# EnnaDelfen/SUHMO

Hardware: AMD Instinct MI355X
Metric: multigrid V-cycles/s (FAS head solve) + GSRB cell-updates/s; achieved HBM GB/s vs peak (higher is better)
Workload: dtype f64; 1 GPU; SHMIP-A head solve, 4096x4096 cells per GPU (square cells of 24.4 m), single AMR level, 64x64 boxes, 6 MG depths, 4+4 GSRB sweeps per depth, 16 bottom (BASELINE north_star: 4096^2 single-level); partition=none

## Files before the change

### suhmo_amd/csrc/suhmo_amr.hip

```cpp
#include "suhmo_common.h"

namespace {
struct Pair { suhmo_level *C, *F; };

int check_pair(suhmo_level *C, suhmo_level *F)
{
    ARG(C && F);
    const DV &c = C->d[0].v, &f = F->d[0].v;
    if (f.nxg != 2 * c.nxg || f.nyg != 2 * c.nyg || (f.i0 & 1) || (f.j0 & 1) || (f.nx & 1) || (f.ny & 1)) {
        suhmo_set_error("amr: the fine level must be a coarse-aligned patch of the domain refined by 2"); return -1; }
    {
        const int lo[2] = {f.i0 / 2, f.j0 / 2}, hi[2] = {(f.i0 + f.nx) / 2 - 1, (f.j0 + f.ny) / 2 - 1};
        const int clo[2] = {c.i0, c.j0}, chi[2] = {c.i0 + c.nx - 1, c.j0 + c.ny - 1}, dom[2] = {c.nxg, c.nyg};
        for (int d = 0; d < 2; d++) {
            bool ok_lo = (clo[d] == 0) ? lo[d] >= 0 : lo[d] - clo[d] >= 2;
            bool ok_hi = (chi[d] == dom[d] - 1) ? hi[d] <= chi[d] : chi[d] - hi[d] >= 2;
            if (d == 1) {
                if (f.rk[0]) ok_lo = lo[1] == clo[1] && c.rk[0]; else if (c.rk[0]) ok_lo = lo[1] - clo[1] >= 1;
                if (f.rk[1]) ok_hi = hi[1] == chi[1] && c.rk[1]; else if (c.rk[1]) ok_hi = chi[1] - hi[1] >= 1;
            }
            if (!ok_lo || !ok_hi) { suhmo_set_error("amr: the fine patch is not properly nested in its coarse level (2 cells)"); return -1; }
        }
    }
    if (C->device != F->device) { suhmo_set_error("amr2: both levels on one device"); return -1; }
// ... 155 lines not shown
    const int co = cidx(vc, I + vf.i0 / 2 - vc.i0, J + vf.j0 / 2 - vc.j0), fo = cidx(vf, 2 * I, 2 * J);
    if (J < ncy) { double sm = 0.0; sm = sm + bxf[fo]; sm = sm + bxf[fo + vf.P]; bxc[co] = sm / 2.0; }
    if (I < ncx) { double sm = 0.0; sm = sm + byf[fo]; sm = sm + byf[fo + 1]; byc[co] = sm / 2.0; }
}
}

int suhmo_grad_cc(suhmo_level *L, int depth, hipStream_t st);
int suhmo_re_bcoef_unfused(suhmo_level *L, int depth, hipStream_t st);

extern "C" int suhmo_amr2_cf_interp(suhmo_level_t *C, suhmo_level_t *F, int field_f, int field_c, suhmo_stream_t s)
{
    int rc = check_pair(C, F); if (rc) return rc;
    ARG(field_f >= 0 && field_f < SUHMO_F_COUNT && field_c >= 0 && field_c < SUHMO_F_COUNT);
    HIPCHK(hipSetDevice(F->device));
    const DV &vf = F->d[0].v, &vc = C->d[0].v;
    double *pf = suhmo_field(F, 0, field_f), *pc = suhmo_field(C, 0, field_c);
    if (!pf || !pc) { suhmo_set_error("field allocation failed"); return -2; }
    if (field_c == SUHMO_F_PHI && (rc = suhmo_ensure_phi_halo(C, 0, 1, (hipStream_t)s))) return rc;
    int n = 2 * vf.ny + 2 * vf.nx;
    hipLaunchKernelGGL(k_cf_interp, dim3((n + 255) / 256), dim3(256), 0, (hipStream_t)s, vf, pf, vc, pc);
    HIPCHK(hipGetLastError());
    return 0;
}

extern "C" int suhmo_amr2_average(suhmo_level_t *C, suhmo_level_t *F, int field_f, int field_c, suhmo_stream_t s)
{
    int rc = check_pair(C, F); if (rc) return rc;
    ARG(field_f >= 0 && field_f < SUHMO_F_COUNT && field_c >= 0 && field_c < SUHMO_F_COUNT);
    HIPCHK(hipSetDevice(F->device));
    const DV &vf = F->d[0].v, &vc = C->d[0].v;
    double *pf = suhmo_field(F, 0, field_f), *pc = suhmo_field(C, 0, field_c);
    if (!pf || !pc) { suhmo_set_error("field allocation failed"); return -2; }
    if (field_c == SUHMO_F_PHI) C->d[0].phi_fresh = 0;
    hipLaunchKernelGGL(k_amr_average, dim3((vf.nx / 2 + 63) / 64, (vf.ny / 2 + 3) / 4), dim3(64, 4), 0, (hipStream_t)s, vf, pf, vc, pc);
    HIPCHK(hipGetLastError());
    return 0;
}

extern "C" int suhmo_amr2_fine_update_operator(suhmo_level_t *C, suhmo_level_t *F, suhmo_stream_t s)
{
    int rc = check_pair(C, F); if (rc) return rc;
    HIPCHK(hipSetDevice(F->device));
    hipStream_t st = (hipStream_t)s;
    if ((rc = suhmo_grad_cc(F, 0, st))) return rc;
    if ((rc = suhmo_grad_cc(C, 0, st))) return rc;
    if ((rc = suhmo_amr2_cf_interp(C, F, SUHMO_F_GRADX, SUHMO_F_GRADX, s))) return rc;
    if ((rc = suhmo_amr2_cf_interp(C, F, SUHMO_F_GRADY, SUHMO_F_GRADY, s))) return rc;
    return suhmo_re_bcoef_unfused(F, 0, st);
}

extern "C" int suhmo_amr2_reflux(suhmo_level_t *C, suhmo_level_t *F, int field_c, suhmo_stream_t s)
{
    int rc = check_pair(C, F); if (rc) return rc;
    ARG(field_c >= 0 && field_c < SUHMO_F_COUNT && field_c != SUHMO_F_PHI && field_c != SUHMO_F_BX && field_c != SUHMO_F_BY);
    HIPCHK(hipSetDevice(F->device));
    const DV &vf = F->d[0].v, &vc = C->d[0].v;
    double *p = suhmo_field(C, 0, field_c);
    if (!p) { suhmo_set_error("field allocation failed"); return -2; }
    if ((rc = suhmo_amr2_cf_interp(C, F, SUHMO_F_PHI, SUHMO_F_PHI, s))) return rc;
    int n = vf.ny + vf.nx;
    hipLaunchKernelGGL(k_amr_reflux, dim3((n + 255) / 256), dim3(256), 0, (hipStream_t)s, vf, F->d[0].fp, vc, C->d[0].fp, p);
    HIPCHK(hipGetLastError());
    return 0;
}
extern "C" int suhmo_amr2_pwl_fill(suhmo_level_t *C, suhmo_level_t *F, int field_f, int field_c, suhmo_stream_t s)
{
    int rc = check_pair(C, F); if (rc) return rc;
    ARG(field_f >= 0 && field_f < SUHMO_F_COUNT && field_c >= 0 && field_c < SUHMO_F_COUNT);
    ARG(field_f != SUHMO_F_BX && field_f != SUHMO_F_BY && field_f != SUHMO_F_QWX && field_f != SUHMO_F_QWY && field_f != SUHMO_F_DCX && field_f != SUHMO_F_DCY);
    HIPCHK(hipSetDevice(F->device));
    const DV &vf = F->d[0].v, &vc = C->d[0].v;
    double *pf = suhmo_field(F, 0, field_f), *pc = suhmo_field(C, 0, field_c);
    if (!pf || !pc) { suhmo_set_error("field allocation failed"); return -2; }
    if (field_f == SUHMO_F_PHI) F->d[0].phi_fresh = 0;
    int n = 2 * (vf.nx + 2) + 2 * vf.ny;
    hipLaunchKernelGGL(k_pwl_fill, dim3((n + 255) / 256), dim3(256), 0, (hipStream_t)s, vf, pf, vc, pc);
    HIPCHK(hipGetLastError());
    return 0;
}
extern "C" int suhmo_amr2_prolong_pc(suhmo_level_t *C, suhmo_level_t *F, int field_c, suhmo_stream_t s)
{
    int rc = check_pair(C, F); if (rc) return rc;
    ARG(field_c >= 0 && field_c < SUHMO_F_COUNT && field_c != SUHMO_F_BX && field_c != SUHMO_F_BY);
    HIPCHK(hipSetDevice(F->device));
    Depth &DC = C->d[0], &DF = F->d[0];
    double *corr = suhmo_field(C, 0, field_c);
    if (!corr) { suhmo_set_error("field allocation failed"); return -2; }
    DF.phi_fresh = 0;
    hipLaunchKernelGGL(k_amr_prolong_pc, dim3((DF.v.nx + 63) / 64, (DF.v.ny + 3) / 4), dim3(64, 4), 0, (hipStream_t)s, DF.v, DF.fp.f[SUHMO_F_PHI], DC.v, corr);
    HIPCHK(hipGetLastError());
    return 0;
}
extern "C" int suhmo_amr2_finer_operator_changed(suhmo_level_t *C, suhmo_level_t *F, suhmo_stream_t s)
{
    int rc = check_pair(C, F); if (rc) return rc;
    HIPCHK(hipSetDevice(F->device));
    for (int f : {SUHMO_F_ACOEF, SUHMO_F_B, SUHMO_F_PI, SUHMO_F_ZB, SUHMO_F_MASK})
        if ((rc = suhmo_amr2_average(C, F, f, f, s))) return rc;
    const DV &vf = F->d[0].v, &vc = C->d[0].v;
    hipLaunchKernelGGL(k_amr_average_faces, dim3((vf.nx / 2 + 1 + 63) / 64, (vf.ny / 2 + 1 + 3) / 4), dim3(64, 4), 0, (hipStream_t)s, vf,
                       F->d[0].fp.f[SUHMO_F_BX], F->d[0].fp.f[SUHMO_F_BY], vc, C->d[0].fp.f[SUHMO_F_BX], C->d[0].fp.f[SUHMO_F_BY]);
    HIPCHK(hipGetLastError());
    C->coarse_mask_ok = 0;
    suhmo_level_drop_graphs(C);
    return 0;
}

extern "C" int suhmo_amr2_prolong2(suhmo_level_t *C, suhmo_level_t *F, int field_c, suhmo_stream_t s)
{
    int rc = check_pair(C, F); if (rc) return rc;
    ARG(field_c >= 0 && field_c < SUHMO_F_COUNT && field_c != SUHMO_F_BX && field_c != SUHMO_F_BY);
    HIPCHK(hipSetDevice(F->device));
    Depth &DC = C->d[0], &DF = F->d[0];
    double *corr = suhmo_field(C, 0, field_c);
    if (!corr) { suhmo_set_error("field allocation failed"); return -2; }
    if ((rc = suhmo_level_exchange(C, 0, field_c, s))) return rc;
    if ((rc = suhmo_level_fill_ghosts(C, 0, field_c, 0, s))) return rc;
    DF.phi_fresh = 0;
    hipLaunchKernelGGL(k_amr_prolong2, dim3((DF.v.nx + 63) / 64, (DF.v.ny + 3) / 4), dim3(64, 4), 0, (hipStream_t)s, DF.v, DF.fp.f[SUHMO_F_PHI], DC.v, corr);
    HIPCHK(hipGetLastError());
    return 0;
}
extern "C" int suhmo_amr2_set_covered(suhmo_level_t *C, suhmo_level_t *F, int field_c, double value, suhmo_stream_t s)
{
    int rc = check_pair(C, F); if (rc) return rc;
    ARG(field_c >= 0 && field_c < SUHMO_F_COUNT);
    HIPCHK(hipSetDevice(F->device));
    const DV &vf = F->d[0].v, &vc = C->d[0].v;
    double *p = suhmo_field(C, 0, field_c);
    if (!p) { suhmo_set_error("field allocation failed"); return -2; }
    if (field_c == SUHMO_F_PHI) C->d[0].phi_fresh = 0;
    hipLaunchKernelGGL(k_amr_set_covered, dim3((vf.nx / 2 + 63) / 64, (vf.ny / 2 + 3) / 4), dim3(64, 4), 0, (hipStream_t)s, vf, vc, p, value);
    HIPCHK(hipGetLastError());
    return 0;
}

int suhmo_apply_and_residual(suhmo_level *L, int depth, hipStream_t st);
namespace {
int cf_phi(suhmo_level_t **lv, int l, suhmo_stream_t s)
{
    if (l == 0) return 0;
    if (lv[l]) return suhmo_amr2_cf_interp(lv[l - 1], lv[l], SUHMO_F_PHI, SUHMO_F_PHI, s);
    if (lv[l - 1]) return suhmo_ensure_phi_halo(lv[l - 1], 0, 1, (hipStream_t)s);
    return 0;
}
int composite_residual(suhmo_level_t **lv, int l, suhmo_stream_t s)
{
    suhmo_level *C = lv[l - 1], *F = lv[l];
    if (!C) return 0;
    hipStream_t st = (hipStream_t)s;
    int rc;
    if ((rc = cf_phi(lv, l - 1, s))) return rc;
    if ((rc = suhmo_apply_and_residual(C, 0, st))) return rc;
    double *res = suhmo_field(C, 0, SUHMO_F_RES);
    if ((rc = cf_phi(lv, l, s))) return rc;
    if (F) {
        const DV &vf = F->d[0].v, &vc = C->d[0].v;
        int n = vf.ny + vf.nx;
        hipLaunchKernelGGL(k_amr_reflux, dim3((n + 255) / 256), dim3(256), 0, st, vf, F->d[0].fp, vc, C->d[0].fp, res, 1);
        HIPCHK(hipGetLastError());
    }
    return 0;
}
int vcycle_amr(suhmo_level_t **lv, int l, const suhmo_solver_params_t *sp, suhmo_stream_t s)
// ... 131 lines not shown
```

### suhmo_amd/csrc/suhmo_bcoef.hip

```cpp
#include "suhmo_hier.h"
#include "suhmo_level_int.h"
#include "suhmo_batch.h"
#include <algorithm>
#include <cmath>
#include <initializer_list>
#include <type_traits>
__device__ __forceinline__ void d_gradcc_val(const DV &v, const FP &fp, int hasMask, int i, int j, double &gx, double &gy)
{
    const double *__restrict__ phi = fp.f[SUHMO_F_PHI];
    int idx = cidx(v, i, j);
    double c = phi[idx];
    double e = phiE(v, phi, idx, i, c, false), w = phiW(v, phi, idx, i, c, false);
    double n = phiN(v, phi, idx, j, c, false), s = phiS(v, phi, idx, j, c, false);
    double gW = v.fdx * (c - w), gE = v.fdx * (e - c), gS = v.fdy * (c - s), gN = v.fdy * (n - c);
    if (hasMask) {
        const double *__restrict__ m = fp.f[SUHMO_F_MASK];
        bool mc = m[idx] < 1e-6;
        if (mc || m[idx - 1] < 1e-6) gW = 0.0;
        if (mc || m[idx + 1] < 1e-6) gE = 0.0;
        if (mc || m[idx - v.P] < 1e-6) gS = 0.0;
        if (mc || m[idx + v.P] < 1e-6) gN = 0.0;
    }
    gx = 0.5 * (gW + gE);
    gy = 0.5 * (gS + gN);
// ... 122 lines not shown
    if (i > v.nx || j > v.ny) return;
    int idx = cidx(v, i, j);
    const double *__restrict__ Re = fp.f[SUHMO_F_RE], *__restrict__ B = fp.f[SUHMO_F_B], *__restrict__ m = fp.f[SUHMO_F_MASK];
    if (j < v.ny)
        fp.f[SUHMO_F_BX][idx] = bcoef_face(ph, Re[idx], Re[idx - 1], B[idx], B[idx - 1], m[idx], m[idx - 1], i + v.i0 == 0 || i + v.i0 == v.nxg);
    if (i < v.nx) {
        int jg = j + v.j0;
        fp.f[SUHMO_F_BY][idx] = bcoef_face(ph, Re[idx], Re[idx - v.P], B[idx], B[idx - v.P], m[idx], m[idx - v.P], jg == 0 || jg == v.nyg);
    }
}
template <class T> __global__ __launch_bounds__(256) void k_bcoef_faces(T t) { d_bcoef_faces(t.view(), t.fields(), t.phys()); }
__global__ __launch_bounds__(256) void k_re_bcoef(OnBoxes t)
{
    const DV &v = t.view();
    const FP &fp = t.fields();
    const suhmo_phys_t &ph = t.phys();
    const int i = (int)(blockIdx.x * blockDim.x + threadIdx.x) - 1, j = (int)(blockIdx.y * blockDim.y + threadIdx.y) - 1;
    if (i > v.nx || j > v.ny) return;
    const bool xo = (i < 0 || i >= v.nx), yo = (j < 0 || j >= v.ny);
    if (xo && yo) return;
    const int idx = cidx(v, i, j);
    const double Rc = d_re_val(fp, ph, idx);
    fp.f[SUHMO_F_RE][idx] = Rc;
    if (i < 0 || j < 0) return;
    const double *__restrict__ B = fp.f[SUHMO_F_B], *__restrict__ m = fp.f[SUHMO_F_MASK];
    if (j < v.ny)
        fp.f[SUHMO_F_BX][idx] = bcoef_face(ph, Rc, d_re_val(fp, ph, idx - 1), B[idx], B[idx - 1], m[idx], m[idx - 1], i + v.i0 == 0 || i + v.i0 == v.nxg);
    if (i < v.nx) {
        const int jg = j + v.j0;
        fp.f[SUHMO_F_BY][idx] = bcoef_face(ph, Rc, d_re_val(fp, ph, idx - v.P), B[idx], B[idx - v.P], m[idx], m[idx - v.P], jg == 0 || jg == v.nyg);
    }
}

template <bool INTERIOR, int BT_X, int BT_Y>
__device__ __forceinline__ void bcoef_tile(const DV &v, const FP &fp, const suhmo_phys_t &ph, int hasMask, double *sphi, double *sB, double *sM,
                                           unsigned *negflag, unsigned epoch)
{
    constexpr int PW = BT_X + 4, PH = BT_Y + 4;
    constexpr int RW = BT_X + 2, RH = BT_Y + 2;
    constexpr int TX = BT_X + 2, TY = 256 / TX;
    constexpr int NK = RH / TY;
    static_assert(TX * TY == 256 && RH % TY == 0, "tile shape");
    double *sre = sphi;
    const int i0 = blockIdx.x * BT_X, j0 = blockIdx.y * BT_Y;
    const int tx = threadIdx.x, ty = threadIdx.y;
    const double *__restrict__ phi = fp.f[SUHMO_F_PHI], *__restrict__ Bf = fp.f[SUHMO_F_B], *__restrict__ mk = fp.f[SUHMO_F_MASK];
    double *__restrict__ bxo = fp.f[SUHMO_F_BX], *__restrict__ byo = fp.f[SUHMO_F_BY];
    const bool halo_lo = v.ext[0], halo_hi = v.ext[1], selfper_y = v.per[1] && !halo_lo && !halo_hi;
    auto xin = [&](int i) { return INTERIOR || (i >= 0 && i < v.nx) || v.per[0]; };
    auto yin = [&](int j) { return INTERIOR || (j >= 0 && j < v.ny) || selfper_y || (j < 0 && halo_lo && j >= -v.gy) || (j >= v.ny && halo_hi && j < v.ny + v.gy); };
    auto wrapx = [&](int i) { return (!INTERIOR && v.per[0]) ? (i < 0 ? i + v.nx : (i >= v.nx ? i - v.nx : i)) : i; };
    auto wrapy = [&](int j) { return (!INTERIOR && selfper_y) ? (j < 0 ? j + v.ny : (j >= v.ny ? j - v.ny : j)) : j; };

    for (int lj = ty; lj < PH; lj += TY) {
        const int j = j0 - 2 + lj;
        const bool yi = yin(j);
        for (int li = tx; li < PW; li += TX) {
            const int i = i0 - 2 + li;
            const bool xi = xin(i);
            double val = 0.0;
            if (xi && yi) val = phi[cidx(v, wrapx(i), wrapy(j))];
            else if (yi && (i == -1 || i == v.nx)) {
                int ic = i < 0 ? 0 : v.nx - 1, idx = cidx(v, ic, wrapy(j));
                double c = phi[idx];
                val = i < 0 ? phiW(v, phi, idx, ic, c, false) : phiE(v, phi, idx, ic, c, false);
            } else if (xi && (j == -1 || j == v.ny)) {
                int jc = j < 0 ? 0 : v.ny - 1, idx = cidx(v, wrapx(i), jc);
                double c = phi[idx];
                val = j < 0 ? phiS(v, phi, idx, jc, c, false) : phiN(v, phi, idx, jc, c, false);
            }
            sphi[lj * PW + li] = val;
        }
    }
    const int i = i0 - 1 + tx;
    const bool xi = xin(i);
    double Br[NK];
    bool hasB[NK];
    bool neg = false;
#pragma unroll
    for (int k = 0; k < NK; k++) {
        const int lj = ty + TY * k, j = j0 - 1 + lj;
        hasB[k] = INTERIOR || (i >= -1 && i <= v.nx && j >= -v.gy && j <= v.ny + v.gy - 1 && !((i < 0 || i >= v.nx) && (j < 0 || j >= v.ny)));
        double b = 0.0, m = 0.0;
        if (hasB[k]) { int idx = cidx(v, i, j); b = Bf[idx]; m = mk[idx]; }
        neg = neg || (m < 0.0 && i >= 0 && i < v.nx && j >= 0 && j < v.ny);
        Br[k] = b;
        sB[lj * RW + tx] = b; sM[lj * RW + tx] = m;
    }
    if (negflag && neg) *negflag = epoch;
    __syncthreads();
    auto gradcc = [&](int p, int gi, int gj, double &gx, double &gy) {
        double c = sphi[p], w = sphi[p - 1], e = sphi[p + 1], s = sphi[p - PW], n = sphi[p + PW];
        double gW = v.fdx * (c - w), gE = v.fdx * (e - c), gS = v.fdy * (c - s), gN = v.fdy * (n - c);
        if (hasMask) {
            int idx = cidx(v, wrapx(gi), wrapy(gj));
            bool mc = mk[idx] < 1e-6;
            if (mc || mk[idx - 1] < 1e-6) gW = 0.0;
            if (mc || mk[idx + 1] < 1e-6) gE = 0.0;
            if (mc || mk[idx - v.P] < 1e-6) gS = 0.0;
            if (mc || mk[idx + v.P] < 1e-6) gN = 0.0;
        }
        gx = 0.5 * (gW + gE); gy = 0.5 * (gS + gN);
    };
    double rer[NK];
#pragma unroll
    for (int k = 0; k < NK; k++) {
        const int lj = ty + TY * k, j = j0 - 1 + lj;
        const bool yi = yin(j);
        const int p = (lj + 1) * PW + (tx + 1);
        double gx = 0.0, gy = 0.0;
        if (xi && yi) {
            gradcc(p, i, j, gx, gy);
        } else if (xi != yi) {
            int d = 0, di = 0, dj = 0;
            if (!xi && (i == -1 || i == v.nx)) { di = i < 0 ? 1 : -1; d = di; }
            else if (!yi && (j == -1 || j == v.ny)) { dj = j < 0 ? 1 : -1; d = dj * PW; }
            if (d != 0) {
                double g1x, g1y, g2x, g2y;
                gradcc(p + d, i + di, j + dj, g1x, g1y);
                gradcc(p + 2 * d, i + 2 * di, j + 2 * dj, g2x, g2y);
                gx = 2.0 * g1x - g2x; gy = 2.0 * g1y - g2y;
            }
        }
        double re = 0.0;
        if (hasB[k]) {
            double B = Br[k];
            double sg = sqrt(gx * gx + gy * gy);
            double discr = 1.0 + 4.0 * ph.omega * (B * B * B * ph.grav * sg) / (12.0 * ph.nu * ph.nu);
            re = (-1.0 + sqrt(discr)) / (2.0 * ph.omega);
        }
        rer[k] = re;
    }
    __syncthreads();
#pragma unroll
    for (int k = 0; k < NK; k++) sre[(ty + TY * k) * RW + tx] = rer[k];
    __syncthreads();
    const int nxt = (!INTERIOR && i0 + BT_X >= v.nx) ? v.nx - i0 + 1 : BT_X, nyt = (!INTERIOR && j0 + BT_Y >= v.ny) ? v.ny - j0 + 1 : BT_Y;
    const int fx = tx - 1;
    if (fx >= 0 && fx < nxt) {
        for (int fy = ty; fy < nyt; fy += TY) {
            const int j = j0 + fy, idx = cidx(v, i, j), r = (fy + 1) * RW + tx;
            if (INTERIOR || j < v.ny)
                bxo[idx] = bcoef_face(ph, sre[r], sre[r - 1], sB[r], sB[r - 1], sM[r], sM[r - 1], !INTERIOR && (i == 0 || i == v.nx));
            if (INTERIOR || i < v.nx) {
                int jg = j + v.j0;
                byo[idx] = bcoef_face(ph, sre[r], sre[r - RW], sB[r], sB[r - RW], sM[r], sM[r - RW], !INTERIOR && (jg == 0 || jg == v.nyg));
            }
        }
    }
}
struct MaskHalo { const double *m[SUHMO_MAXDEPTH]; int nx[SUHMO_MAXDEPTH], ny[SUHMO_MAXDEPTH], P[SUHMO_MAXDEPTH], gy[SUHMO_MAXDEPTH]; int nd, lo, hi; };
__global__ __launch_bounds__(256) void k_mask_halo_report(MaskHalo h, unsigned *negflag, unsigned epoch)
{
    const int d = blockIdx.z, i = blockIdx.x * blockDim.x + threadIdx.x;
    if (d >= h.nd || i >= h.nx[d]) return;
    const int g = h.gy[d];
    bool neg = false;
    for (int r = blockIdx.y; r < 2 * g; r += gridDim.y) {
        const bool top = r >= g;
        if (top ? !h.hi : !h.lo) continue;
        const int j = top ? h.ny[d] + (r - g) : -1 - r;
        neg = neg || h.m[d][(long)(j + g) * h.P[d] + SUHMO_XOFF + i] < 0.0;
    }
    if (neg) *negflag = epoch;
}
template <int BT_X, int BT_Y>
__device__ __forceinline__ void d_bcoef_fused(const DV &v, const FP &fp, const suhmo_phys_t &ph, int hasMask, unsigned *negflag, unsigned epoch)
{
    __shared__ double sphi[(BT_X + 4) * (BT_Y + 4)], sB[(BT_X + 2) * (BT_Y + 2)], sM[(BT_X + 2) * (BT_Y + 2)];
    const int i0 = blockIdx.x * BT_X, j0 = blockIdx.y * BT_Y;
    const bool interior = i0 - 2 >= 0 && i0 + BT_X + 1 <= v.nx - 1 && j0 - 2 >= 0 && j0 + BT_Y + 1 <= v.ny - 1;
    if (interior) bcoef_tile<true, BT_X, BT_Y>(v, fp, ph, hasMask, sphi, sB, sM, negflag, epoch);
    else bcoef_tile<false, BT_X, BT_Y>(v, fp, ph, hasMask, sphi, sB, sM, negflag, epoch);
}
template <class T, int BT_X, int BT_Y>
__global__ __launch_bounds__(256) void k_bcoef_fused(T t, unsigned *negflag, unsigned epoch)
{
    const suhmo_phys_t ph = t.phys();
    if (std::is_same<T, OnMembers>::value) { negflag = nullptr; epoch = 0u; }
    d_bcoef_fused<BT_X, BT_Y>(t.view(), t.fields(), ph, ph.use_mask_gradients, negflag, epoch);
}
template <class T> int launch_bcoef_fused(const T &t, bool wide, unsigned *flag, unsigned epoch, hipStream_t st)
{
    if constexpr (std::is_same<T, OnLevel>::value)
        if (wide) return launch_grid(k_bcoef_fused<T, 126, 14>, t, dim3((t.nx() + 125) / 126, (t.ny() + 13) / 14), dim3(128, 2), st, flag, epoch);
    return launch_grid(k_bcoef_fused<T, 62, 14>, t, dim3((t.nx() + 61) / 62, (t.ny() + 13) / 14), dim3(64, 4), st, flag, epoch);
}
template int launch_bcoef_fused(const OnMembers &, bool, unsigned *, unsigned, hipStream_t);
template <class T> int launch_re(const T &t, hipStream_t st) { return launch_over(k_re<T>, t, GHOSTED, st); }
template <class T> int launch_bcoef_faces(const T &t, hipStream_t st) { return launch_over(k_bcoef_faces<T>, t, FACES, st); }
template <class T> int launch_grad_cc(const T &t, hipStream_t st)
{
    int rc = launch_over(k_gradcc<T>, t, CELLS, st);
    return rc ? rc : launch_over(k_grad_ghosts<T>, t, PERIMETER, st);
}
template int launch_re(const OnLevel &, hipStream_t);
template int launch_re(const OnBoxes &, hipStream_t);
template int launch_re(const OnMembers &, hipStream_t);
template int launch_bcoef_faces(const OnLevel &, hipStream_t);
template int launch_bcoef_faces(const OnBoxes &, hipStream_t);
template int launch_bcoef_faces(const OnMembers &, hipStream_t);
template int launch_grad_cc(const OnMembers &, hipStream_t);

extern "C" int suhmo_level_update_operator(suhmo_level_t *L, int depth, suhmo_stream_t s)
{
    SUHMO_TIME("VCAMRNonLinearPoissonOp::UpdateOperator");
    ARG(L); ARG(depth >= 0 && depth < L->ndepth);
    HIPCHK(hipSetDevice(L->device));
    hipStream_t st = (hipStream_t)s;
    Depth &D = L->d[depth];
    bool fused = L->bcoef_fused && D.v.nx >= 4 && D.v.ny >= 4 && (!(D.v.ext[0] || D.v.ext[1]) || (D.v.gy >= 2 && D.v.ny >= 2))
                 && L->desc.nx_global == 0;
    int rc = suhmo_ensure_phi_halo(L, depth, fused ? 2 : 1, st); if (rc) return rc;
    if (fused) {
        const bool wide = L->bcoef_tile_x == 126 && D.v.nx >= 256;
        unsigned *flag = nullptr;
        if (depth == 0) { L->maskflag_epoch = 0; L->mask_reported = 0; }
        if (depth == 0 && L->skip_mask) {
            flag = (unsigned *)(L->scratch + L->scratch_elems - 1);
            if (++L->mask_epoch == 0) L->mask_epoch = 1;
            L->mask_reported = 1;
        }
        if ((rc = launch_bcoef_fused(on_level(L, depth), wide, flag, L->mask_epoch, st))) return rc;
        if (flag && (D.v.ext[0] || D.v.ext[1])) {
            MaskHalo h;
            h.nd = 0; h.lo = D.v.ext[0]; h.hi = D.v.ext[1];
            const int last = L->coarse_mask_ok ? (L->agg ? L->agg_depth : L->ndepth) : 1;
            int gmax = 1;
            for (int k = 0; k < last && k < SUHMO_MAXDEPTH; k++) {
                const Depth &Dk = L->d[k];
                h.m[k] = Dk.fp.f[SUHMO_F_MASK]; h.nx[k] = Dk.v.nx; h.ny[k] = Dk.v.ny; h.P[k] = Dk.v.P; h.gy[k] = Dk.v.gy;
                if (Dk.v.gy > gmax) gmax = Dk.v.gy;
                h.nd = k + 1;
            }
            hipLaunchKernelGGL(k_mask_halo_report, dim3((D.v.nx + 255) / 256, 2 * gmax, h.nd), dim3(256), 0, st, h, flag, L->mask_epoch);
        }
    } else {
        if (depth == 0) { L->maskflag_epoch = 0; L->mask_reported = 0; }
        if (!suhmo_field(L, depth, SUHMO_F_GRADX) || !suhmo_field(L, depth, SUHMO_F_GRADY) || !suhmo_field(L, depth, SUHMO_F_RE)) return -2;
        const OnLevel t = on_level(L, depth);
        if ((rc = launch_over(k_gradcc<OnLevel>, t, CELLS, st))) return rc;
        rc = suhmo_exchange_fields(L, depth, {SUHMO_F_GRADX, SUHMO_F_GRADY}, st); if (rc) return rc;
        if ((rc = launch_over(k_grad_ghosts<OnLevel>, t, PERIMETER, st)) || (rc = launch_re(t, st)) || (rc = launch_bcoef_faces(t, st))) return rc;
    }
    HIPCHK(hipGetLastError());
    if (depth == 0 && L->faces_deferred) return 0;
    rc = suhmo_exchange_fields(L, depth, {SUHMO_F_BX, SUHMO_F_BY}, st); if (rc) return rc;
    return 0;
}

int suhmo_grad_cc(suhmo_level *L, int depth, hipStream_t st)
{
    if (!suhmo_field(L, depth, SUHMO_F_GRADX) || !suhmo_field(L, depth, SUHMO_F_GRADY) || !suhmo_field(L, depth, SUHMO_F_RE)) return -2;
    int rc = suhmo_ensure_phi_halo(L, depth, 1, st); if (rc) return rc;
    if ((rc = launch_over(k_gradcc<OnLevel>, on_level(L, depth), CELLS, st))) return rc;
    rc = suhmo_exchange_fields(L, depth, {SUHMO_F_GRADX, SUHMO_F_GRADY}, st); if (rc) return rc;
    return launch_over(k_grad_ghosts<OnLevel>, on_level(L, depth), PERIMETER, st);
}
int suhmo_grad_cc_list(suhmo_level *L, int depth, const int2 *d_cells, int n, hipStream_t st)
{
    Depth &D = L->d[depth];
    if (!suhmo_field(L, depth, SUHMO_F_GRADX) || !suhmo_field(L, depth, SUHMO_F_GRADY) || !suhmo_field(L, depth, SUHMO_F_RE)) return -2;
    int rc = suhmo_ensure_phi_halo(L, depth, 1, st); if (rc) return rc;
    if (n) hipLaunchKernelGGL(k_gradcc_list, dim3((n + 255) / 256), dim3(256), 0, st, D.v, D.fp, L->ph.use_mask_gradients, d_cells, n);
    HIPCHK(hipGetLastError());
    return 0;
}
int suhmo_re_bcoef_unfused(suhmo_level *L, int depth, hipStream_t st)
{
// ... 260 lines not shown
{
    static const int fields[5] = {SUHMO_F_ACOEF, SUHMO_F_B, SUHMO_F_PI, SUHMO_F_ZB, SUHMO_F_MASK};
    int nblocks = 0;
    for (int q = 0; q < 5; q++) a.f[q] = L->d[0].fp.f[fields[q]];
    for (int dep = 1; dep < L->ndepth; dep++) {
        const Depth &C = L->d[dep];
        AvgDepth &o = a.d[dep - 1];
        o.nx = C.v.nx; o.ny = C.v.ny; o.P = C.v.P; o.gy = C.v.gy;
        for (int q = 0; q < 5; q++) o.c[q] = C.fp.f[fields[q]];
        o.boff = nblocks; o.nbx = (C.v.nx + 63) / 64;
        nblocks += 5 * o.nbx * ((C.v.ny + 3) / 4);
    }
    return nblocks;
}
template <class T, class A> static int launch_average_cells_all(const T &t, A av, int nblocks, const DV &v1, int nd, hipStream_t st)
{
    int rc = launch_grid(k_average_cells_all<T, A>, t, dim3(nblocks), BLK2D, st, av, nd);
    return rc ? rc : launch_grid(k_coef_ghosts_all<T, A>, t, dim3((2 * v1.ny + 2 * v1.nx + 255) / 256, 4 * (nd - 1)), dim3(256), st, av);
}
int suhmo_build_mg_coefficients(suhmo_level *L, bool with_faces, hipStream_t st)
{
    const int nd = L->ndepth;
    if (nd > 1) {
        AvgAll a;
        const int nblocks = fill_avg_all(L, a);
        int rc = launch_average_cells_all(on_level(L, 0), a, nblocks, L->d[1].v, nd, st); if (rc) return rc;
    }
    for (int dep = 1; dep < nd; dep++) {
        int rc;
        if (with_faces && (rc = suhmo_level_average_operator(L, dep, (suhmo_stream_t)st))) return rc;
        if (L->agg && dep >= L->agg_depth) continue;
        rc = suhmo_exchange_fields(L, dep, {SUHMO_F_ACOEF, SUHMO_F_B, SUHMO_F_PI, SUHMO_F_ZB, SUHMO_F_MASK}, st); if (rc) return rc;
    }
    L->coarse_mask_ok = 1;
    return suhmo_agg_gather_static(L, with_faces, st);
}
extern "C" int suhmo_level_build_mg_coefficients(suhmo_level_t *L, suhmo_stream_t s)
{
    ARG(L);
    HIPCHK(hipSetDevice(L->device));
    return suhmo_build_mg_coefficients(L, true, (hipStream_t)s);
}

int suhmo_multi_grad_cc(const suhmo_multi &m, hipStream_t st)
{
    return m.merged ? launch_over(k_gradcc_ghosts, m.on(), CELLS, st) : launch_grad_cc(m.on(), st);
}

int suhmo_levels_grad_cc(const suhmo_lvboxes &lv, int hasMask, hipStream_t st)
{
    int nz = 0;
    for (int q = 0; q < lv.n; q++) nz += lv.nbox[q];
    if (nz <= 0) return 0;
    hipLaunchKernelGGL(k_gradcc_ghosts_lv, dim3((lv.maxnx + 63) / 64, (lv.maxny + 3) / 4, nz), BLK2D, 0, st, lv, hasMask);
    HIPCHK(hipGetLastError());
    return 0;
}

int suhmo_multi_re_bcoef(const suhmo_multi &m, hipStream_t st)
{
    const OnBoxes t = m.on();
    if (m.merged) return launch_over(k_re_bcoef, t, GHOSTED, st);
    int rc = launch_re(t, st);
    return rc ? rc : launch_bcoef_faces(t, st);
}

// ... 37 lines not shown
```

### suhmo_amd/csrc/suhmo_common.h

```cpp
#pragma once
#include <hip/hip_runtime.h>
#include <cstdio>
#include <cstdlib>
#include <cstring>
#include <utility>
#include <string>
#include <vector>
#include "../../include/suhmo_hip.h"

#define SUHMO_XOFF 16
#define SUHMO_MAXDEPTH 16

struct DV {
    int nx, ny;
    int P;
    int gy;
    int rows;
    int j0, nyg;
    double dx, dy;
    double rdx, rdy;
    double fdx, fdy;
    double alpha, beta;
    int bct[2][2];
    double two_v[2][2];
// ... 64 lines not shown
{
    return aterm * c
           - v.beta * (bxE * (e - c) * v.rdx - bxW * (c - w) * v.rdx
                       + byN * (n - c) * v.rdy - byS * (c - s) * v.rdy)
           + nl;
}

__device__ __forceinline__ double lambda_cell(const DV &v, double aterm, double bxE, double bxW,
                                              double byN, double byS)
{
    double lam = aterm;
    lam = lam + v.rdx * v.beta * (bxE + bxW);
    lam = lam + v.rdy * v.beta * (byN + byS);
    return lam;
}

struct Depth {
    DV v;
    FP fp;
    size_t elems;
    int nbox;
    int prolong_pending;
    int rhs_pending;
    double *phi_alt;
    int phi_fresh;
};

struct VGraph {
    int key[4]; hipGraphExec_t exec;
    double *p0[SUHMO_MAXDEPTH], *a0[SUHMO_MAXDEPTH];
    double *p1[SUHMO_MAXDEPTH], *a1[SUHMO_MAXDEPTH];
    double *rhs;
    int rout_req, rout_done, rout_np; const double *rout_rhs;
};
struct ProfEv { hipEvent_t a, b; long cells; int restricts; };

struct suhmo_level {
    int ndepth;
    int batch_owned;
    int stub;
    Depth d[SUHMO_MAXDEPTH];
    suhmo_level_desc_t desc;
    std::vector<int> boxes;
    suhmo_phys_t ph;
    int device;
    double *scratch;
    double *hscratch;
    double *hscratch_dev;
    unsigned long long hseq;
    int poll_readback;
    size_t scratch_elems;
    suhmo_exchange_fn ex;
    suhmo_allreduce_max_fn ar;
    suhmo_allreduce_fn ar2;
    int (*ard)(void *user, double *dev_values, int n, int op, suhmo_stream_t s);
    void *user;
    int (*ex_begin)(void *user);
    int (*ex_end)(void *user, suhmo_level *L, suhmo_stream_t s);
    long graph_max_cells;
    std::vector<VGraph> vgraphs; int vgraph_seen[4]; hipStream_t gstream;
    long vgraph_replays;
    suhmo_level *gap; double gap_dt;
    void *rccl;
    int faces_deferred;
    void *ipc; int ipc_owner;
    long agg_min_cells;
    int agg_depth, agg_world, agg_rank;
    suhmo_level *agg;
    int agg_static_stale;
    suhmo_allgather_fn ag; void *ag_user;
    double *agg_send, *agg_recv; size_t agg_cap; long agg_gathers;
    int resout_req, resout_armed, resout_done; const double *resout_rhs; long resout_count;
    int resout_np;
    long frhs_stream, frhs_tile;
    int prof_on;
    std::vector<ProfEv> prof;
    int gsrb_variant;
    long fused_min_cells;
    int bcoef_fused;
    int bcoef_tile_x;
    int fused_nt;
    int fused_restrict;
    int fused_hc;
    int fas_rhs_fused;
    int strips_rhs_local;
    int skip_mask;
    int mask_reported;
    int coarse_mask_ok;
    unsigned mask_epoch, maskflag_epoch;
    int overlap_halo;
    hipStream_t xstream; hipEvent_t xev[2]; long overlapped;
    int tile_strips;
    int tile_chunks;
    int resid_in_relax;
    int fas_rhs_in_relax;
    long tile_max_cells;
    int tile_restrict;
    int tile_order;
    int bottom_solver; long bottom_one_launch_max_cells;
    unsigned long long *bottom_ctr; long bottom_host_iters, bottom_host_solves;
    int gsrb_tile, tile_t, tile_s;
};

void suhmo_set_error(const char *fmt, ...);
struct SuhmoTimer { const char *name; double t0; int mode; explicit SuhmoTimer(const char *n); ~SuhmoTimer(); };
#define SUHMO_TIME(label) SuhmoTimer suhmo_tm_(label)
#define HIPCHK(x) do { hipError_t e_ = (x); if (e_ != hipSuccess) { \
    suhmo_set_error("%s:%d %s -> %s", __FILE__, __LINE__, #x, hipGetErrorString(e_)); return -2; } } while (0)
#define ARG(cond) do { if (!(cond)) { suhmo_set_error("%s:%d bad argument: %s", __FILE__, __LINE__, #cond); return -1; } } while (0)

double *suhmo_field(suhmo_level *L, int depth, int field);
int suhmo_level_create_(suhmo_level_t **out, const suhmo_level_desc_t *desc, bool stub);
void suhmo_level_share_transport(suhmo_level *dst, const suhmo_level *src);
int suhmo_level_materialize_(suhmo_level *L);
void suhmo_fp_changed();
unsigned long suhmo_fp_epoch();
struct SwapGuard {
    double **a, **b; bool armed;
    SwapGuard() : a(nullptr), b(nullptr), armed(false) {}
    void arm(double **a_, double **b_) { a = a_; b = b_; std::swap(*a, *b); armed = true; suhmo_fp_changed(); }
    void back() { if (armed) { std::swap(*a, *b); armed = false; suhmo_fp_changed(); } }
    ~SwapGuard() { back(); }
};
int suhmo_average_operator_all(suhmo_level *L, int nd, hipStream_t st);
int suhmo_restrict_both(suhmo_level *L, int depth, hipStream_t st);
bool suhmo_gsrb_can_fuse_prolong(suhmo_level *L, int depth, int sweeps);
int suhmo_level_residual_and_norm(suhmo_level *L, double *out, hipStream_t st);
int suhmo_level_norm_from_partials(suhmo_level *L, int np, double *out, hipStream_t st);
bool suhmo_gsrb_can_fuse_rhs(suhmo_level *L, int depth, int sweeps, bool rhs_local = false);
int suhmo_launch_gsrb(suhmo_level *L, int depth, int sweeps, int tail, hipStream_t st, int *restricted = nullptr);
void suhmo_level_drop_graphs(suhmo_level *L);
int suhmo_ensure_phi_halo(suhmo_level *L, int depth, int need, hipStream_t st);
int suhmo_fas_coarse_rhs(suhmo_level *L, int depth, hipStream_t st, int hcomp = 0);
struct HostSlot { double *val; unsigned long long *flag; unsigned long long seq; };
HostSlot suhmo_host_slot(suhmo_level *L);
int suhmo_readback(suhmo_level *L, hipStream_t st, double *out, double *out2 = nullptr);
// ... 53 lines not shown
```

### suhmo_amd/csrc/suhmo_fas.hip

```cpp
#include "suhmo_common.h"
#include <cstdlib>

static int eff_depths(const suhmo_level *L, const suhmo_solver_params_t *sp)
{
    int nd = L->ndepth;
    if (sp->max_depth >= 0 && sp->max_depth + 1 < nd) nd = sp->max_depth + 1;
    return nd;
}

static int relax(suhmo_level *L, int dep, int sweeps, int tail, suhmo_stream_t s, bool observable = false, int *restricted = nullptr)
{
    L->resout_armed = observable && dep == 0 && L->resout_req && L->resid_in_relax;
    int rc = suhmo_launch_gsrb(L, dep, sweeps, tail, (hipStream_t)s, restricted);
    L->resout_armed = 0;
    if (rc) return rc;
    if (sweeps > 0 && observable) return suhmo_level_fill_ghosts(L, dep, SUHMO_F_PHI, 1, s);
    return 0;
}

static int rows_after_prolong(int dep, int num_smooth)
{
    int tail_post = 2;
    for (int d = 1; d <= dep; d++) tail_post = (2 * num_smooth + tail_post + 1) / 2;
    return 2 * num_smooth + tail_post;
// ... 52 lines not shown
    } else {
        if ((rc = suhmo_prolong_with_halo(L, dep, (hipStream_t)s))) return rc;
    }
    return relax(L, dep, S, tail_post, s, dep == 0);
}

static int vcycle_body(suhmo_level *L, const suhmo_solver_params_t *sp, int nd, suhmo_stream_t s)
{
    int rc;
    if (sp->bcoeff_otf) {
        L->faces_deferred = 1;
        rc = suhmo_level_update_operator(L, 0, s);
        if (rc) { L->faces_deferred = 0; return rc; }
        if (L->mask_reported) L->maskflag_epoch = L->mask_epoch;
        if ((rc = suhmo_average_operator_all(L, nd, (hipStream_t)s))) return rc;
    } else L->maskflag_epoch = 0;
    rc = fas_cycle(L, 0, sp, nd, s);
    L->maskflag_epoch = 0;
    return rc;
}

void suhmo_level_drop_graphs(suhmo_level *L)
{
    if (getenv("SUHMO_GRAPH_DEBUG")) { int ok = 0; for (VGraph &g : L->vgraphs) ok += g.exec != nullptr; fprintf(stderr,
        "[suhmo] level %dx%d: %zu V-cycle graphs, %d executable\n", L->d[0].v.nx, L->d[0].v.ny, L->vgraphs.size(), ok); }
    for (VGraph &g : L->vgraphs) if (g.exec) (void)hipGraphExecDestroy(g.exec);
    L->vgraphs.clear();
    if (L->gstream) { (void)hipStreamDestroy(L->gstream); L->gstream = nullptr; }
}
static int vcycle_graph(suhmo_level *L, const suhmo_solver_params_t *sp, int nd, suhmo_stream_t s, bool &done)
{
    done = false;
    const int key[4] = {sp->num_smooth, sp->num_bottom, sp->bcoeff_otf, nd};
    auto at_start = [&](const VGraph &g) {
        if (memcmp(g.key, key, sizeof(key))) return false;
        for (int d = 0; d < L->ndepth; d++) if (L->d[d].fp.f[SUHMO_F_PHI] != g.p0[d] || L->d[d].phi_alt != g.a0[d]) return false;
        if (g.rout_req != (L->resid_in_relax ? L->resout_req : 0) || g.rout_rhs != L->resout_rhs) return false;
        return L->d[0].fp.f[SUHMO_F_RHS] == g.rhs;
    };
    for (const VGraph &g : L->vgraphs)
        if (at_start(g)) {
            if (!g.exec) return 0;
            HIPCHK(hipGraphLaunch(g.exec, (hipStream_t)s)); L->vgraph_replays++;
            for (int d = 0; d < L->ndepth; d++) { L->d[d].fp.f[SUHMO_F_PHI] = g.p1[d]; L->d[d].phi_alt = g.a1[d]; } suhmo_fp_changed();
            if (g.rout_done) { L->resout_done = 1; L->resout_count++; L->resout_np = g.rout_np; }
            done = true;
            return 0;
        }
    for (int k = 0; k < 4; k++) if (L->vgraph_seen[k] != key[k]) { memcpy(L->vgraph_seen, key, sizeof(key)); return 0; }
    if (L->vgraphs.size() >= 16) return 0;
    if (!L->gstream) HIPCHK(hipStreamCreateWithFlags(&L->gstream, hipStreamNonBlocking));
    VGraph g; memcpy(g.key, key, sizeof(key)); g.exec = nullptr;
    for (int d = 0; d < SUHMO_MAXDEPTH; d++) { g.p0[d] = g.a0[d] = g.p1[d] = g.a1[d] = nullptr; }
    for (int d = 0; d < L->ndepth; d++) { g.p0[d] = L->d[d].fp.f[SUHMO_F_PHI]; g.a0[d] = L->d[d].phi_alt; }
    g.rhs = L->d[0].fp.f[SUHMO_F_RHS];
    g.rout_req = L->resid_in_relax ? L->resout_req : 0; g.rout_rhs = L->resout_rhs; g.rout_done = 0;
    const int rout_before = L->resout_done; const long rout_count = L->resout_count;
    HIPCHK(hipStreamSynchronize((hipStream_t)s));
    hipGraph_t graph = nullptr;
    hipError_t e = hipStreamBeginCapture(L->gstream, hipStreamCaptureModeThreadLocal);
    int rc = 0;
    if (e == hipSuccess) {
        rc = vcycle_body(L, sp, nd, (suhmo_stream_t)L->gstream);
        e = hipStreamEndCapture(L->gstream, &graph);
    }
    g.rout_done = L->resout_count != rout_count;
    g.rout_np = L->resout_np;
    L->resout_done = rout_before; L->resout_count = rout_count;
    bool clean = true;
    for (int d = 0; d < L->ndepth; d++) {
        clean = clean && !L->d[d].prolong_pending && !L->d[d].rhs_pending;
        g.p1[d] = L->d[d].fp.f[SUHMO_F_PHI]; g.a1[d] = L->d[d].phi_alt;
        L->d[d].prolong_pending = 0; L->d[d].rhs_pending = 0;
        L->d[d].fp.f[SUHMO_F_PHI] = g.p0[d]; L->d[d].phi_alt = g.a0[d];
    }
    if (e == hipSuccess && rc == 0 && clean && graph && hipGraphInstantiate(&g.exec, graph, nullptr, nullptr, 0) != hipSuccess) g.exec = nullptr;
    if (!(e == hipSuccess && rc == 0 && clean)) g.exec = nullptr;
    if (graph) (void)hipGraphDestroy(graph);
    (void)hipGetLastError();
    L->vgraphs.push_back(g);
    if (!g.exec) return 0;
    HIPCHK(hipGraphLaunch(g.exec, (hipStream_t)s)); L->vgraph_replays++;
    for (int d = 0; d < L->ndepth; d++) { L->d[d].fp.f[SUHMO_F_PHI] = g.p1[d]; L->d[d].phi_alt = g.a1[d]; } suhmo_fp_changed();
    if (g.rout_done) { L->resout_done = 1; L->resout_count++; L->resout_np = g.rout_np; }
    done = true;
    return 0;
}

extern "C" int suhmo_level_vcycle(suhmo_level_t *L, const suhmo_solver_params_t *sp, suhmo_stream_t s)
{
    SUHMO_TIME("AMRFASMultiGrid::VCycle");
    ARG(L && sp);
    HIPCHK(hipSetDevice(L->device));
    int nd = eff_depths(L, sp);
    const Depth &D = L->d[0];
    const bool ext = D.v.ext[0] || D.v.ext[1];
    const bool host_bottom = L->bottom_solver && !suhmo_bottom_one_launch(L, nd - 1);
    if (L->graph_max_cells > 0 && !L->ex && !ext && !L->prof_on && !host_bottom && (long)D.v.nx * D.v.ny <= L->graph_max_cells) {
        bool done = false;
        int rc = vcycle_graph(L, sp, nd, s, done);
        if (rc || done) return rc;
    }
    return vcycle_body(L, sp, nd, s);
}

extern "C" int suhmo_level_solve(suhmo_level_t *L, const suhmo_solver_params_t *sp, int *iters, double *hist, suhmo_stream_t s)
{
    SUHMO_TIME("AMRFASMultiGrid::solve");
    ARG(L && sp);
    HIPCHK(hipSetDevice(L->device));
    bool have_res = false;
    int np = 0;
    auto residual = [&](double *rnorm) {
        if (!have_res) return suhmo_level_residual_and_norm(L, rnorm, (hipStream_t)s);
        if (np > 0) return suhmo_level_norm_from_partials(L, np, rnorm, (hipStream_t)s);
        return suhmo_level_norm(L, 0, SUHMO_F_RES, 0, rnorm, s);
    };
    auto cycle = [&] {
        L->resout_req = 1 | 4; L->resout_rhs = nullptr; L->resout_done = 0; L->resout_np = 0;
        int rc = suhmo_level_vcycle(L, sp, s);
        have_res = L->resout_done != 0;
        np = have_res ? L->resout_np : 0;
        L->resout_req = 0; L->resout_done = 0; L->resout_np = 0;
        return rc;
    };
    int rc = suhmo_solve_no_init(sp, iters, hist, residual, cycle);
    if (rc) return rc;
    return suhmo_level_fill_ghosts(L, 0, SUHMO_F_PHI, 0, s);
}
```

### suhmo_amd/csrc/suhmo_gsrb.hip

```cpp
#include "suhmo_hier.h"
#include "suhmo_batch.h"
#include <type_traits>

template <bool HAS_ALPHA>
__device__ __forceinline__ void d_gsrb_pass_simple(const DV &v, const FP &fp, suhmo_phys_t ph, int pass, int jlo, int jhi,
                                                   const FP *__restrict__ ft = nullptr, const int2 *__restrict__ push = nullptr)
{
    int j = jlo + (int)(blockIdx.y * blockDim.y + threadIdx.y);
    int t = blockIdx.x * blockDim.x + threadIdx.x;
    if (j > jhi) return;
    int i = 2 * t + ((j + v.j0 + pass) & 1);
    if (i >= v.nx) return;
    double *__restrict__ phi = fp.f[SUHMO_F_PHI];
    int idx = cidx(v, i, j);
    double c = phi[idx];
    double e = phiE(v, phi, idx, i, c, false), w = phiW(v, phi, idx, i, c, false);
    double n = phiN(v, phi, idx, j, c, false), s = phiS(v, phi, idx, j, c, false);
    double bxW = fp.f[SUHMO_F_BX][idx], bxE = fp.f[SUHMO_F_BX][idx + 1];
    double byS = fp.f[SUHMO_F_BY][idx], byN = fp.f[SUHMO_F_BY][idx + v.P];
    double nl, dnl;
    nl_terms(ph, c, fp.f[SUHMO_F_B][idx], fp.f[SUHMO_F_PI][idx], fp.f[SUHMO_F_ZB][idx],
             fp.f[SUHMO_F_MASK][idx], nl, dnl);
    double aterm = HAS_ALPHA ? v.alpha * fp.f[SUHMO_F_ACOEF][idx] : v.alpha;
    double lofphi = lofphi_cell(v, aterm, c, e, w, n, s, bxE, bxW, byN, byS, nl);
// ... 187 lines not shown
template <int G, int T, int S>
static void launch_box(const suhmo_multi &m, const suhmo_phys_t &ph, bool has_alpha, const void *halo, const int *hbase, int fsrc, int fdst, int npass, int bc_ghosts, hipStream_t st)
{
    const dim3 grd(((m.maxnx + T - 1) / T) * ((m.maxny + T - 1) / T), m.nbox);
    if (has_alpha) hipLaunchKernelGGL((k_gsrb_box_m<true, G, T, S>), grd, dim3(BoxGeom<G, T, S>::NT), 0, st, m.dv, m.fp, (const int2 *)halo, hbase, ph, fsrc, fdst, npass, bc_ghosts);
    else hipLaunchKernelGGL((k_gsrb_box_m<false, G, T, S>), grd, dim3(BoxGeom<G, T, S>::NT), 0, st, m.dv, m.fp, (const int2 *)halo, hbase, ph, fsrc, fdst, npass, bc_ghosts);
}
int suhmo_multi_gsrb_box(const suhmo_multi &m, const suhmo_phys_t &ph, bool has_alpha, const void *halo, const int *hbase, int fsrc, int fdst, int npass, int bc_ghosts, hipStream_t st)
{
    if (m.nbox <= 0) return 0;
    if (npass < 1 || npass > 2 * SUHMO_BOX_HALO) { suhmo_set_error("internal: %d colour passes in one box launch", npass); return -4; }
    if (npass > 4) launch_box<8, 16, 1>(m, ph, has_alpha, halo, hbase, fsrc, fdst, npass, bc_ghosts, st);
    else launch_box<4, 16, 1>(m, ph, has_alpha, halo, hbase, fsrc, fdst, npass, bc_ghosts, st);
    HIPCHK(hipGetLastError());
    return 0;
}

struct FusedGeom {
    int W;
    int Hc;
    int nstrips, nchunks, ntiles;
    int ylo, yhi;
    int jbeg, jend;
    int wrap_y;
    const unsigned *negflag; unsigned mask_epoch;
    int nchl, chunk0, chunk1, edges;
    const double *pc, *pco; int Pc, gyc;
    double *rres, *rphi; int rP, rgy;
    const double *fres; double *frhs, *flphi, *fphiold;
    const double *ortrue; double *ores, *olphi;
    double *onorm;
};

struct RowCoef {
    double rhs[2], B[2], Pi[2], zb[2], mask[2], a[2], byS[2], byN[2];
    double bx0, bx1, bx2;
};
#define CP2(d, s, f) d.f[0] = s.f[0]; d.f[1] = s.f[1]
template <bool HAS_ALPHA>
__device__ __forceinline__ void copy_coef(RowCoef &d, const RowCoef &s)
{
    CP2(d, s, rhs); CP2(d, s, B); CP2(d, s, Pi); CP2(d, s, zb); CP2(d, s, mask);
    if (HAS_ALPHA) { CP2(d, s, a); }
    CP2(d, s, byS); CP2(d, s, byN);
    d.bx0 = s.bx0; d.bx1 = s.bx1; d.bx2 = s.bx2;
}

template <int K, bool HAS_ALPHA, int NT, int RM = 0, bool FRHS = false>
__global__ __launch_bounds__(NT) void k_gsrb_fused(DV v, FP fp, const double *__restrict__ pin,
                                                   double *__restrict__ pout, suhmo_phys_t ph, FusedGeom g)
{
    constexpr bool ROUT = RM == 2, RR = RM != 0;
    static_assert(!(FRHS && (RR || HAS_ALPHA)), "the right-hand side is formed in the plain launch of an alpha = 0 operator");
    constexpr int LW = 2 * NT, R = 2 * K + 3 + (RR ? 1 : 0);
    constexpr int HX = 2 * K + (RR ? 2 : 0), EY = RR ? 1 : 0;
    __shared__ double lds[R * LW];

    int b = blockIdx.x, q = g.ntiles / 8, rem = g.ntiles % 8, xcd = b % 8;
    int tile = xcd * q + (xcd < rem ? xcd : rem) + b / 8;
    int strip = tile / g.nchl, chunk = tile % g.nchl;
    chunk = g.edges ? (chunk < g.chunk0 ? chunk : g.chunk1 + (chunk - g.chunk0)) : g.chunk0 + chunk;

    const int t = threadIdx.x;
    const int c0 = strip * g.W;
    const int xl = 2 * t;
    const int i0 = c0 - HX + xl;
    const bool in_row = xl < g.W + 2 * HX;
    int im = i0;
    if (v.per[0]) { if (im < 0) im += v.nx; else if (im >= v.nx) im -= v.nx; }
    const bool cval = in_row && im >= 0 && im < v.nx;
    const int cend = (c0 + g.W < v.nx) ? c0 + g.W : v.nx;
    const bool own = cval && i0 >= c0 && i0 < cend;

    const int jA = g.jbeg + chunk * g.Hc;
    const int jB = (jA + g.Hc < g.jend) ? jA + g.Hc : g.jend;
    const int jmin = (jA - EY - 2 * K > g.ylo) ? jA - EY - 2 * K : g.ylo;
    const int jmax = (jB - 1 + EY + 2 * K < g.yhi) ? jB - 1 + EY + 2 * K : g.yhi;

    const double *__restrict__ f_rhs = fp.f[SUHMO_F_RHS], *__restrict__ f_B = fp.f[SUHMO_F_B];
    const double *__restrict__ f_Pi = fp.f[SUHMO_F_PI], *__restrict__ f_zb = fp.f[SUHMO_F_ZB];
    const double *__restrict__ f_mask = fp.f[SUHMO_F_MASK], *__restrict__ f_a = fp.f[SUHMO_F_ACOEF];
    const double *__restrict__ f_bx = fp.f[SUHMO_F_BX], *__restrict__ f_by = fp.f[SUHMO_F_BY];

    auto wrapj = [&](int j) { if (g.wrap_y) { if (j < 0) j += v.ny; else if (j >= v.ny) j -= v.ny; } return j; };
    auto ld2 = [&](const double *__restrict__ p, int idx) { return *reinterpret_cast<const double2 *>(p + idx); };

    RowCoef cf0, cf1, cf2, cf3, cf4, cf5;
    double racc = 0.0, raccp = 0.0;
    double nmax = 0.0;
    const bool xbc = !v.per[0] && (c0 - HX <= 0 || c0 + g.W + HX >= v.nx);
    const bool ybc = !v.per[1] && (jmin <= 0 || jmax >= v.ny - 1);
    double2 pnext = make_double2(0.0, 0.0);
    double2 pprev = make_double2(0.0, 0.0);
    const bool usemask = !g.negflag || *g.negflag == g.mask_epoch;

    int sr = 0;
    auto ring = [](int x) { return x < 0 ? x + R : x; };
    for (int r = jmin - 1; r <= jB - 1 + 2 * K + EY; r++) {
        bool lphi = cval && (r + 1 >= jmin) && (r + 1 <= jmax);
        if (lphi) {
            const int jr = wrapj(r + 1);
            pnext = ld2(pin, cidx(v, im, jr));
            if (g.pc) {
                const int ic = ((jr >> 1) + g.gyc) * g.Pc + SUHMO_XOFF + (im >> 1);
                const double corr = 1.0 * g.pc[ic] + (-1.0) * g.pco[ic];
                pnext.x = pnext.x + corr; pnext.y = pnext.y + corr;
            }
        }
        bool lcf = cval && (r >= jmin) && (r <= jmax);
        if (lcf) {
            int idx = cidx(v, im, wrapj(r));
#define LD2(dst, p, ix) { double2 t_ = ld2(p, ix); dst[0] = t_.x; dst[1] = t_.y; }
            LD2(cf0.rhs, (FRHS ? g.fres : f_rhs), idx); LD2(cf0.B, f_B, idx); LD2(cf0.Pi, f_Pi, idx);
            LD2(cf0.zb, f_zb, idx);
            if (usemask) { LD2(cf0.mask, f_mask, idx); } else { cf0.mask[0] = 1.0; cf0.mask[1] = 1.0; }
            if (HAS_ALPHA) LD2(cf0.a, f_a, idx);
            LD2(cf0.byS, f_by, idx); LD2(cf0.byN, f_by, idx + v.P);
            double2 bxp = ld2(f_bx, idx);
            cf0.bx0 = bxp.x; cf0.bx1 = bxp.y; cf0.bx2 = f_bx[idx + 2];
        }
        __syncthreads();

        if constexpr (FRHS) {
            const int jf = r - 1;
            if (cval && jf >= jmin && jf <= jmax) {
                const int s0 = ring(sr - 1), sN = sr;
                const double *row = lds + s0 * LW;
                double lo[2], cc[2];
#pragma unroll
                for (int a = 0; a < 2; a++) {
                    const int x = xl + a, i = im + a;
                    double c = row[x];
                    double w = row[(a == 0 && xl == 0) ? 0 : x - 1], e = row[(a == 1 && xl == LW - 2) ? LW - 1 : x + 1];
                    double n = lds[sN * LW + x], s = a ? pprev.y : pprev.x;
                    if (xbc) {
                        if (i == 0) w = (v.bct[0][0] == 0) ? v.two_v[0][0] - c : c + v.neu[0][0];
                        if (i == v.nx - 1) e = (v.bct[0][1] == 0) ? v.two_v[0][1] - c : c + v.neu[0][1];
                    }
                    if (ybc) {
                        if (jf == 0 && !v.ext[0]) s = (v.bct[1][0] == 0) ? v.two_v[1][0] - c : c + v.neu[1][0];
                        if (jf == v.ny - 1 && !v.ext[1]) n = (v.bct[1][1] == 0) ? v.two_v[1][1] - c : c + v.neu[1][1];
                    }
                    double nl, dnl;
                    nl_terms(ph, c, cf1.B[a], cf1.Pi[a], cf1.zb[a], cf1.mask[a], nl, dnl);
                    const double bxW = a ? cf1.bx1 : cf1.bx0, bxE = a ? cf1.bx2 : cf1.bx1;
                    lo[a] = lofphi_cell(v, v.alpha, c, e, w, n, s, bxE, bxW, cf1.byN[a], cf1.byS[a], nl);
                    cc[a] = c;
                }
                cf1.rhs[0] = 1.0 * cf1.rhs[0] + 1.0 * lo[0]; cf1.rhs[1] = 1.0 * cf1.rhs[1] + 1.0 * lo[1];
                const bool lo_end = v.ext[0] && chunk == 0, hi_end = v.ext[1] && chunk == g.nchunks - 1;
                const int jP0 = lo_end ? jmin : jA, jP1 = hi_end ? jmax + 1 : jB;
                const int jR0 = lo_end ? jmin + 1 : jA, jR1 = hi_end ? jmax : jB;
                if (own && jf >= jP0 && jf < jP1) {
                    const int idx = cidx(v, i0, jf);
                    if (jf >= jR0 && jf < jR1) {
                        *reinterpret_cast<double2 *>(g.flphi + idx) = make_double2(lo[0], lo[1]);
                        *reinterpret_cast<double2 *>(g.frhs + idx) = make_double2(cf1.rhs[0], cf1.rhs[1]);
                    }
                    *reinterpret_cast<double2 *>(g.fphiold + idx) = make_double2(cc[0], cc[1]);
                }
                pprev = make_double2(cc[0], cc[1]);
            }
            __syncthreads();
        }

        auto advance_a = [&](const int m, const RowCoef &q, auto a_tag) {
            constexpr int a = decltype(a_tag)::value;
            const int j = r - m;
            const int x = xl + a, i = im + a;
            const int s0 = ring(sr - m), sN = ring(sr - m + 1), sS = ring(sr - m - 1);
            const double *row = lds + s0 * LW;
            double c = row[x];
            double w = row[(a == 0 && xl == 0) ? 0 : x - 1], e = row[(a == 1 && xl == LW - 2) ? LW - 1 : x + 1];
            double n = lds[sN * LW + x], s = lds[sS * LW + x];
            if (xbc) {
                if (i == 0) w = (v.bct[0][0] == 0) ? v.two_v[0][0] - c : c + v.neu[0][0];
                if (i == v.nx - 1) e = (v.bct[0][1] == 0) ? v.two_v[0][1] - c : c + v.neu[0][1];
            }
            if (ybc) {
                if (j == 0 && !v.ext[0]) s = (v.bct[1][0] == 0) ? v.two_v[1][0] - c : c + v.neu[1][0];
                if (j == v.ny - 1 && !v.ext[1]) n = (v.bct[1][1] == 0) ? v.two_v[1][1] - c : c + v.neu[1][1];
            }
            double nl, dnl;
            nl_terms(ph, c, q.B[a], q.Pi[a], q.zb[a], q.mask[a], nl, dnl);
            const double bxW = a ? q.bx1 : q.bx0, bxE = a ? q.bx2 : q.bx1;
            double aterm = HAS_ALPHA ? v.alpha * q.a[a] : v.alpha;
            double lofphi = lofphi_cell(v, aterm, c, e, w, n, s, bxE, bxW, q.byN[a], q.byS[a], nl);
            double lam = lambda_cell(v, aterm, bxE, bxW, q.byN[a], q.byS[a]);
            double denom = 1.0e-16 + lam + dnl;
            lds[s0 * LW + x] = c + (q.rhs[a] - lofphi) / denom;
        };
        auto advance = [&](const int m, const RowCoef &q) {
            const int j = r - m;
            if (j >= jmin && j <= jmax) {
                const int a = (j + v.j0 + ((m - 1) & 1)) & 1;
                if (a) { if (cval) advance_a(m, q, std::integral_constant<int, 1>()); }
                else   { if (cval) advance_a(m, q, std::integral_constant<int, 0>()); }
            }
        };
        advance(1, cf1);
        __syncthreads();
        advance(2, cf2);
        if constexpr (K >= 2) {
            __syncthreads();
            advance(3, cf3);
            __syncthreads();
            advance(4, cf4);
        }

        if constexpr (RR) {
            const int jr = r - 2 * K - 1;
            if (own && jr >= jA && jr < jB && jr >= 0 && jr < v.ny) {
                const RowCoef &q = (K >= 2) ? cf5 : cf3;
                const int s0 = ring(sr - (2 * K + 1)), sN = ring(sr - 2 * K), sS = ring(sr - (2 * K + 2));
                const double *row = lds + s0 * LW;
                double acc = (jr & 1) ? racc : 0.0, accp = (jr & 1) ? raccp : 0.0;
                double lo2[2] = {0.0, 0.0};
#pragma unroll
                for (int a = 0; a < 2; a++) {
                    const int x = xl + a, i = im + a;
                    double c = row[x], w = row[x - 1], e = row[x + 1];
                    double n = lds[sN * LW + x], s = lds[sS * LW + x];
                    if (xbc) {
                        if (i == 0) w = (v.bct[0][0] == 0) ? v.two_v[0][0] - c : c + v.neu[0][0];
                        if (i == v.nx - 1) e = (v.bct[0][1] == 0) ? v.two_v[0][1] - c : c + v.neu[0][1];
                    }
                    if (ybc) {
                        if (jr == 0 && !v.ext[0]) s = (v.bct[1][0] == 0) ? v.two_v[1][0] - c : c + v.neu[1][0];
                        if (jr == v.ny - 1 && !v.ext[1]) n = (v.bct[1][1] == 0) ? v.two_v[1][1] - c : c + v.neu[1][1];
                    }
                    double nl, dnl;
                    nl_terms(ph, c, q.B[a], q.Pi[a], q.zb[a], q.mask[a], nl, dnl);
                    const double bxW = a ? q.bx1 : q.bx0, bxE = a ? q.bx2 : q.bx1;
                    double aterm = HAS_ALPHA ? v.alpha * q.a[a] : v.alpha;
                    double lofphi = lofphi_cell(v, aterm, c, e, w, n, s, bxE, bxW, q.byN[a], q.byS[a], nl);
                    if constexpr (ROUT) lo2[a] = lofphi;
                    else {
                        acc = acc + (q.rhs[a] - lofphi) / 4.0;
                        accp = accp + c / 4.0;
                    }
                }
                if constexpr (ROUT) {
                    const int idx = cidx(v, i0, jr);
                    const double2 rt = *reinterpret_cast<const double2 *>(g.ortrue + idx);
                    const double r0 = -1.0 * lo2[0] + 1.0 * rt.x, r1 = -1.0 * lo2[1] + 1.0 * rt.y;
                    *reinterpret_cast<double2 *>(g.ores + idx) = make_double2(r0, r1);
                    if (g.olphi) *reinterpret_cast<double2 *>(g.olphi + idx) = make_double2(lo2[0], lo2[1]);
                    nmax = fmax(nmax, fmax(fabs(r0), fabs(r1)));
                } else if (jr & 1) {
                    const int ic = ((jr >> 1) + g.rgy) * g.rP + SUHMO_XOFF + (i0 >> 1);
                    g.rres[ic] = acc; g.rphi[ic] = accp;
                } else { racc = acc; raccp = accp; }
            }
        }
        {
            const int jo = r - 2 * K;
            if (own && jo >= jA && jo < jB) {
                const int so = ring(sr - 2 * K);
                double2 o = make_double2(lds[so * LW + xl], lds[so * LW + xl + 1]);
                *reinterpret_cast<double2 *>(pout + cidx(v, i0, jo)) = o;
            }
        }
        sr = sr + 1 == R ? 0 : sr + 1;
        if (in_row) { lds[sr * LW + xl] = pnext.x; lds[sr * LW + xl + 1] = pnext.y; }
        if constexpr (RR && K >= 2) copy_coef<HAS_ALPHA>(cf5, cf4);
        if constexpr (K >= 2) { copy_coef<HAS_ALPHA>(cf4, cf3); copy_coef<HAS_ALPHA>(cf3, cf2); }
        else if constexpr (RR) copy_coef<HAS_ALPHA>(cf3, cf2);
        copy_coef<HAS_ALPHA>(cf2, cf1);
        copy_coef<HAS_ALPHA>(cf1, cf0);
    }
    if constexpr (ROUT) {
        if (g.onorm) {
            static_assert(!ROUT || NT == 64, "one wave per workgroup");
#pragma unroll
            for (int o = 32; o > 0; o >>= 1) nmax = fmax(nmax, __shfl_xor(nmax, o));
            if (t == 0) g.onorm[strip * g.nchunks + chunk] = nmax;
        }
    }
}

static bool fused_ok(const suhmo_level *L, const Depth &D, int K)
{
    const DV &v = D.v;
    if (v.nx % 2 || v.nx < 64 || v.ny < 4 * K + 4) return false;
    if (v.cfx[0] || v.cfx[1] || L->desc.nx_global > 0) return false;
    if ((v.ext[0] || v.ext[1]) && (v.gy < 2 * K || v.ny < 2 * K)) return false;
    if (v.per[1] && !(v.ext[0] || v.ext[1]) && v.ny < 4 * K) return false;
    return true;
}

template <int K, int NT, int RM = 0>
static int launch_fused(suhmo_level *L, int depth, int ext_rows, hipStream_t st, int part = 0)
{
    constexpr bool RST = RM == 1, RR = RM != 0;
    Depth &D = L->d[depth];
    const DV &v = D.v;
    if (!D.phi_alt) {
        HIPCHK(hipMalloc(&D.phi_alt, D.elems * sizeof(double)));
        HIPCHK(hipMemsetAsync(D.phi_alt, 0, D.elems * sizeof(double), st));
    }
    FusedGeom g;
    constexpr int HX = 2 * K + (RR ? 2 : 0), EY = RR ? 1 : 0;
    const int maxW = 2 * NT - 2 * HX;
    g.nstrips = (v.nx + maxW - 1) / maxW;
    g.W = 2 * ((v.nx + 2 * g.nstrips - 1) / (2 * g.nstrips));
    g.nstrips = (v.nx + g.W - 1) / g.W;
    {
        static int slots_k[3] = {0, 0, 0};
        if (!slots_k[K]) {
            int nb = 0, ncu = 0, dev = 0;
            HIPCHK(hipGetDevice(&dev));
            HIPCHK(hipDeviceGetAttribute(&ncu, hipDeviceAttributeMultiprocessorCount, dev));
            HIPCHK(hipOccupancyMaxActiveBlocksPerMultiprocessor(&nb, (k_gsrb_fused<K, false, NT, RM>), NT, 0));
            slots_k[K] = (nb > 0 ? nb : 1) * (ncu > 0 ? ncu : 256);
        }
        g.jbeg = v.ext[0] ? -ext_rows : 0;
        g.jend = v.ny + (v.ext[1] ? ext_rows : 0);
        const int nrows = g.jend - g.jbeg;
        int nch = slots_k[K] / g.nstrips;
        if (nch < 1) nch = 1;
        g.Hc = (nrows + nch - 1) / nch;
        if (g.Hc < 8 * K) g.Hc = 8 * K;
        if ((long)v.nx * v.ny < 2000000L) g.Hc = 6;
        if (L->fused_hc > 0) g.Hc = L->fused_hc;
        if (RST) g.Hc += g.Hc & 1;
        if (g.Hc > nrows) g.Hc = nrows;
        g.nchunks = (nrows + g.Hc - 1) / g.Hc;
    }
    g.nchl = g.nchunks; g.chunk0 = 0; g.chunk1 = g.nchunks; g.edges = 0;
    if (part) {
        int c0 = 0, c1 = g.nchunks;
        if (v.ext[0]) while (c0 < g.nchunks && g.jbeg + c0 * g.Hc - 2 * K - EY < 0) c0++;
        if (v.ext[1]) while (c1 > c0 && std::min(g.jbeg + c1 * g.Hc, g.jend) - 1 + 2 * K + EY > v.ny - 1) c1--;
        const bool ok = c1 > c0 && c1 - c0 < g.nchunks;
        if (!ok) { if (part == 1) return 1; }
        else if (part == 1) { g.chunk0 = c0; g.chunk1 = c1; g.nchl = c1 - c0; }
        else { g.edges = 1; g.chunk0 = c0; g.chunk1 = c1; g.nchl = g.nchunks - (c1 - c0); }
    }
    g.ntiles = g.nstrips * g.nchl;
    bool selfper = v.per[1] && !(v.ext[0] || v.ext[1]);
    g.wrap_y = selfper;
    g.ylo = v.ext[0] ? g.jbeg - 2 * K - EY : (selfper ? -2 * K - EY : 0);
    g.yhi = v.ext[1] ? g.jend - 1 + 2 * K + EY : (selfper ? v.ny - 1 + 2 * K + EY : v.ny - 1);
    const double *pin = D.fp.f[SUHMO_F_PHI];
    g.pc = g.pco = nullptr; g.Pc = g.gyc = 0;
    if (D.prolong_pending) {
        Depth &C = L->d[depth + 1];
        g.pc = C.fp.f[SUHMO_F_PHI]; g.pco = C.fp.f[SUHMO_F_PHIOLD]; g.Pc = C.v.P; g.gyc = C.v.gy;
        if (part != 1) D.prolong_pending = 0;
    }
    g.negflag = nullptr; g.mask_epoch = 0;
    if (L->skip_mask && L->maskflag_epoch && L->maskflag_epoch == L->mask_epoch && (depth == 0 || L->coarse_mask_ok)
        && (L->desc.nx_global == 0)) {
        g.negflag = (const unsigned *)(L->scratch + L->scratch_elems - 1); g.mask_epoch = L->mask_epoch;
    }
    g.rres = g.rphi = nullptr; g.rP = g.rgy = 0;
    if (RST) {
        Depth &C = L->d[depth + 1];
        g.rres = C.fp.f[SUHMO_F_RES]; g.rphi = C.fp.f[SUHMO_F_PHI]; g.rP = C.v.P; g.rgy = C.v.gy;
        C.phi_fresh = 0;
    }
    g.fres = nullptr; g.frhs = g.flphi = g.fphiold = nullptr;
    g.ortrue = nullptr; g.ores = g.olphi = nullptr;
    if (RM == 2) {
        if (v.alpha != 0.0) { suhmo_set_error("internal: residual output on a launch that cannot form it"); return -4; }
        g.ortrue = L->resout_rhs ? L->resout_rhs : D.fp.f[SUHMO_F_RHS];
        g.ores = D.fp.f[SUHMO_F_RES];
        if (L->resout_req & 2) { g.olphi = suhmo_field(L, depth, SUHMO_F_LPHI); if (!g.olphi) return -2; }
        g.onorm = nullptr;
        if ((L->resout_req & 4) && (size_t)g.nstrips * g.nchunks + 4 < L->scratch_elems) { g.onorm = L->scratch + 2; L->resout_np = g.nstrips * g.nchunks; }
        else L->resout_np = 0;
    }
    if (D.rhs_pending) {
        if constexpr (K == 2 && NT == 64 && !RR) {
            if (part || v.alpha != 0.0) { suhmo_set_error("internal: rhs_pending on a launch that cannot form it"); return -4; }
            g.fres = D.fp.f[SUHMO_F_RES]; g.frhs = D.fp.f[SUHMO_F_RHS]; g.flphi = suhmo_field(L, depth, SUHMO_F_LPHI); g.fphiold = suhmo_field(L, depth, SUHMO_F_PHIOLD);
            if (!g.flphi || !g.fphiold) return -2;
            D.rhs_pending = 0; L->frhs_stream++;
            hipLaunchKernelGGL((k_gsrb_fused<2, false, 64, false, true>), dim3(g.ntiles), dim3(NT), 0, st, v, D.fp, pin, D.phi_alt, L->ph, g);
            { std::swap(D.fp.f[SUHMO_F_PHI], D.phi_alt); suhmo_fp_changed(); }
            return 0;
        } else { suhmo_set_error("internal: rhs_pending on a launch that cannot form it"); return -4; }
    }
    if (v.alpha != 0.0)
        hipLaunchKernelGGL((k_gsrb_fused<K, true, NT, false>), dim3(g.ntiles), dim3(NT), 0, st, v, D.fp, pin, D.phi_alt, L->ph, g);
    else
        hipLaunchKernelGGL((k_gsrb_fused<K, false, NT, RM>), dim3(g.ntiles), dim3(NT), 0, st, v, D.fp, pin, D.phi_alt, L->ph, g);
    if (part != 1) { std::swap(D.fp.f[SUHMO_F_PHI], D.phi_alt); suhmo_fp_changed(); }
    return 0;
}

struct TileGeom {
    int ntx, nty;
    const double *pc, *pco; int Pc, gyc;
    double *rres, *rphi; int rP, rgy;
    int frhs;
    int jbeg, jend;
    int chunks;
    int order;
};
struct PairCoef { double rhs0, rhs1, B0, B1, Pi0, Pi1, zb0, zb1, a0, a1, byS0, byS1, byN0, byN1, bx0, bx1, bx2; int mneg; };

template <int T, bool RST> struct TileShape { static constexpr int TX = T, TY = (RST && T == 32) ? 28 : T; };
template <int S, int T, bool RST> struct TileThreads { static constexpr int NT = 256; };
template <int S, int T, bool HAS_ALPHA, bool RST = false, bool CHUNKED = false>
__device__ __forceinline__ void d_gsrb_tile(const DV &v, const FP &fp, const double *__restrict__ pin, double *__restrict__ pout,
                                            const suhmo_phys_t &ph, const TileGeom &g)
{
    constexpr int TX = TileShape<T, RST>::TX, TY = TileShape<T, RST>::TY;
    constexpr int HX = 2 * S + (RST ? 2 : 0), HY = 2 * S + (RST ? 1 : 0);
    constexpr int LX = TX + 2 * HX, LY = TY + 2 * HY, NP = LX / 2, NPAIR = NP * LY;
    constexpr int NT = TileThreads<S, T, RST>::NT, NK = (NPAIR + NT - 1) / NT;
    constexpr int PAD = LX + 2;
    __shared__ double lds_raw[LY * LX + 2 * PAD];
    double *const lds = lds_raw + PAD;
    __shared__ double lq[RST ? TY * TX : 1];
    int tl = blockIdx.x;
    if (g.order) {
        const int nt = g.ntx * g.nty, q8 = nt / 8, rem = nt % 8, xcd = tl % 8;
// ... 619 lines not shown
```

### suhmo_amd/csrc/suhmo_hier.h

```cpp
#pragma once
#include "suhmo_target.h"
constexpr int SUHMO_BOX_HALO = 8;
struct suhmo_multi { const DV *dv; const FP *fp; int nbox, maxnx, maxny; double *red;
                     int merged;
                     const void *push; const int *pbase;
                     suhmo_phys_t ph;
                     OnBoxes on() const { return OnBoxes{dv, fp, ph, nbox, maxnx, maxny}; } };
template <class T> int launch_colour_pass(const T &t, bool has_alpha, int pass, int lo, int hi, const void *push, const int *pbase, hipStream_t st);
int suhmo_multi_gsrb_box(const suhmo_multi &m, const suhmo_phys_t &ph, bool has_alpha, const void *halo, const int *hbase, int fsrc, int fdst, int npass,
    int bc_ghosts, hipStream_t st);
template <class T> int launch_fill_ghosts(const T &t, int field, int homog, hipStream_t st);
template <class T> int launch_axby(const T &t, int fd, int fx, int fy, double a, double b, hipStream_t st);
template <class T> int launch_restrict(const T &f, const T &c, bool also_phi, bool has_alpha, hipStream_t st);
template <class T> int launch_prolong(const T &f, const T &c, int lo, int hi, int lo_c, int hi_c, hipStream_t st);
int launch_apply_boxes(const OnBoxes &t, bool has_alpha, int mode, hipStream_t st);
int suhmo_apply_and_residual(suhmo_level *L, int depth, hipStream_t st);
int launch_fas_enter(const OnBoxes &t, hipStream_t st);
int launch_fas_leave(const OnBoxes &t, hipStream_t st);
int launch_copy(const OnBoxes &t, int fd, int fs, hipStream_t st);
int launch_copy_between(const OnBoxes &dst, const OnBoxes &src, const int *fd, const int *fs, int n, hipStream_t st);
template <class T> int launch_grad_cc(const T &t, hipStream_t st);
template <class T> int launch_re(const T &t, hipStream_t st);
template <class T> int launch_bcoef_faces(const T &t, hipStream_t st);
template <class T> int launch_coef_ghosts(const T &t, int field, hipStream_t st);
template <class T> int launch_bcoef_fused(const T &t, bool wide, unsigned *flag, unsigned epoch, hipStream_t st);
int suhmo_multi_grad_cc(const suhmo_multi &m, hipStream_t st);
int suhmo_multi_re_bcoef(const suhmo_multi &m, hipStream_t st);
int suhmo_multi_norm_max(const suhmo_multi &m, suhmo_level *slot, int field, double *out, hipStream_t st);
int suhmo_level_norm_max_partials(suhmo_level *L, int field, const double **partials, int *np, hipStream_t st);
int suhmo_multi_norm_max_partials(const suhmo_multi &m, int field, const double **partials, int *np, hipStream_t st);
int suhmo_norm_max_of_lists(suhmo_level *slot, const double *const *partials, const int *np, int cnt, double *out, hipStream_t st);
constexpr int SUHMO_LVMAX = 7;
struct suhmo_lvboxes { const DV *dv[SUHMO_LVMAX]; const FP *fp[SUHMO_LVMAX]; int nbox[SUHMO_LVMAX], mode[SUHMO_LVMAX]; int n, maxnx, maxny; };
int suhmo_levels_apply(const suhmo_lvboxes &lv, const suhmo_phys_t &ph, bool has_alpha, hipStream_t st);
int suhmo_levels_norm_max_cover_partials(const suhmo_lvboxes &lv, int field, double *partial, int *np, hipStream_t st);
int suhmo_level_norm_max_cover_partials(suhmo_level *L, int field, const double **partials, int *np, hipStream_t st);
int suhmo_levels_grad_cc(const suhmo_lvboxes &lv, int hasMask, hipStream_t st);
```

### suhmo_amd/csrc/suhmo_hier.hip

```cpp
#include "suhmo_hier_int.h"
#include <string>

int suhmo_grad_cc(suhmo_level *L, int depth, hipStream_t st);
int suhmo_apply_and_residual_rects(suhmo_level *L, int depth, const int4 *d_rects, int n, int maxw, int maxh, hipStream_t st);
int suhmo_grad_cc_list(suhmo_level *L, int depth, const int2 *d_cells, int n, hipStream_t st);

using namespace hier;
namespace {
inline const suhmo_phys_t &phys_of(suhmo_hier *H, int l) { return H->lev[l].box[0]->ph; }
inline bool has_alpha(suhmo_hier *H, int l) { return H->lev[l].box[0]->d[0].v.alpha != 0.0; }
int hier_gsrb(suhmo_hier *H, int l, int sweeps, suhmo_stream_t s, bool may_swap = false)
{
    SUHMO_TIME("AMRNonLinearPoissonOp::relaxNF");
    if (l == 0) { H->phi_shadow_fresh = false; H->phi_ver[0]++; H->base_full_ver++; return suhmo_level_gsrb(base_of(H), 0, sweeps, s); }
    int rc;
    suhmo_multi m;
    if ((rc = multi_of(H, l, HST(s), m))) return rc;
    HLev &Vf = H->lev[l];
    if (sweeps > 0 && H->fused_relax && Vf.halo_ok && !Vf.part) {
        if ((rc = ensure_field(H, l, SUHMO_F_PHI2)) || (rc = multi_of(H, l, HST(s), m))) return rc;
        if (Vf.self_wrap < 0) {
            Vf.self_wrap = 0;
            for (suhmo_level *L : Vf.box) { const DV &v = L->d[0].v; if ((v.per[0] && !v.cfx[0]) || (v.per[1] && !v.ext[0])) Vf.self_wrap = 1; }
        }
// ... 19 lines not shown
    const bool push = H->push_ghosts && !V.part;
    for (int it = 0; it < sweeps; it++)
        for (int pass = 0; pass < 2; pass++) {
            if ((rc = launch_colour_pass(m.on(), has_alpha(H, l), pass, 0, 0, push ? m.push : nullptr, m.pbase, HST(s)))) return rc;
            H->phi_ver[l]++;
            if (!push && (rc = hier_ff(H, l, SUHMO_F_PHI, -1, false, HST(s), V.part ? pass : -1))) return rc;
        }
    if (sweeps > 0 && (rc = launch_fill_ghosts(m.on(), SUHMO_F_PHI, 1, HST(s)))) return rc;
    if (sweeps > 0 && push) H->ff_seen[l] = H->phi_ver[l];
    return 0;
}
int hier_level_residual(suhmo_hier *H, int l, suhmo_stream_t s)
{
    if (l == 0) return suhmo_level_residual(base_of(H), 0, s);
    int rc;
    suhmo_multi m;
    if ((rc = hier_ff(H, l, SUHMO_F_PHI, -1, false, HST(s))) || (rc = multi_of(H, l, HST(s), m))) return rc;
    return launch_apply_boxes(m.on(), has_alpha(H, l), 1, HST(s));
}
int hier_axby(suhmo_hier *H, int l, int dst, int x, int y, double a, double b, suhmo_stream_t s)
{
    if (l == 0) return suhmo_level_axby(base_of(H), 0, dst, x, y, a, b, s);
    int rc;
    suhmo_multi m;
    if ((rc = ensure_field(H, l, dst)) || (rc = ensure_field(H, l, x)) || (rc = ensure_field(H, l, y)) || (rc = multi_of(H, l, HST(s), m))) return rc;
    return launch_axby(m.on(), dst, x, y, a, b, HST(s));
}
int hier_copy(suhmo_hier *H, int l, int dst, int src, suhmo_stream_t s)
{
    int rc;
    if ((rc = ensure_field(H, l, dst)) || (rc = ensure_field(H, l, src))) return rc;
    if (dst == SUHMO_F_PHI) { for (suhmo_level *L : H->lev[l].box) L->d[0].phi_fresh = 0; H->phi_ver[l]++; }
    if (dst == SUHMO_F_PHI && l == 0) H->phi_shadow_fresh = false;
    if (l == 0) H->base_full_ver++;
    if (l == 0) {
        suhmo_level *L = base_of(H);
        HIPCHK(hipMemcpyAsync(L->d[0].fp.f[dst], L->d[0].fp.f[src], L->d[0].elems * sizeof(double), hipMemcpyDeviceToDevice, HST(s)));
        return 0;
    }
    suhmo_multi m;
    if ((rc = multi_of(H, l, HST(s), m))) return rc;
    return launch_copy(m.on(), dst, src, HST(s));
}
int cf_phi(suhmo_hier *H, int l, suhmo_stream_t s)
{
    if (l == 0) return 0;
    if (H->cf_seen[l][0] == H->phi_ver[l] && H->cf_seen[l][1] == H->phi_ver[l - 1]) return 0;
    if (H->merged_launches && !H->lev[l].part && H->ff_seen[l] != H->phi_ver[l]) {
        int rc = hier_cf_ff(H, l, SUHMO_F_PHI, SUHMO_F_PHI, -1, -1, false, HST(s));
        if (!rc) { H->cf_seen[l][0] = H->phi_ver[l]; H->cf_seen[l][1] = H->phi_ver[l - 1]; H->ff_seen[l] = H->phi_ver[l]; }
        return rc;
    }
    int rc = hier_cf(H, l, SUHMO_F_PHI, SUHMO_F_PHI, HST(s));
    if (!rc) { H->cf_seen[l][0] = H->phi_ver[l]; H->cf_seen[l][1] = H->phi_ver[l - 1]; }
    return rc;
}

inline bool levels_mergeable(const suhmo_hier *H) { return H->merged_launches && !H->part && !dist_base(H) && H->nlev <= SUHMO_LVMAX + 1; }
int levels_boxes(suhmo_hier *H, int llo, int lhi, int mode_top, int mode_rest, suhmo_stream_t s, suhmo_lvboxes &lv)
{
    memset(&lv, 0, sizeof(lv));
    int rc;
    for (int l = lhi; l >= std::max(1, llo); l--) {
        suhmo_multi m;
        if ((rc = multi_of(H, l, HST(s), m))) return rc;
        const int q = lv.n++;
// ... 442 lines not shown
    ARG(H);
    H->ag = fn; H->ag_user = user;
    if (H->gap) { H->gap->ag = fn; H->gap->ag_user = user; }
    return 0;
}
int suhmo_rccl_allgather_hook(void *user, const double *send, long count, double *recv, suhmo_stream_t s);
extern "C" int suhmo_hier_attach_rccl(suhmo_hier_t *H)
{
    ARG(H);
    suhmo_level *B = base_of(H);
    if (!B->rccl) { suhmo_set_error("hier: attach the base strip first (suhmo_level_attach_rccl on suhmo_hier_box(H, 0, 0))"); return -1; }
    return suhmo_hier_set_allgather(H, suhmo_rccl_allgather_hook, B->rccl);
}
extern "C" long suhmo_hier_gathers(const suhmo_hier_t *H) { return H ? H->gathers + (H->gap ? H->gap->gathers : 0) : -1; }
extern "C" int suhmo_hier_num_levels(const suhmo_hier_t *H) { return H ? H->nlev : -1; }
extern "C" int suhmo_hier_num_boxes(const suhmo_hier_t *H, int l) { return (H && l >= 0 && l < H->nlev) ? (int)H->lev[l].box.size() : -1; }
extern "C" suhmo_level_t *suhmo_hier_box(suhmo_hier_t *H, int l, int k)
{
    if (!H || l < 0 || l >= H->nlev || k < 0 || k >= (int)H->lev[l].box.size()) return nullptr;
    return H->lev[l].box[k];
}
extern "C" int suhmo_hier_box_owner(const suhmo_hier_t *H, int l, int k, int *held)
{
    if (!H || l < 0 || l >= H->nlev || k < 0 || k >= (int)H->lev[l].box.size()) return -2;
    const HLev &V = H->lev[l];
    if (held) *held = V.part ? (int)V.held[k] : 1;
    return V.part ? V.owner[k] : -1;
}
extern "C" int suhmo_hier_exchange(suhmo_hier_t *H, int l, int field, int corners, suhmo_stream_t s)
{
    int rc = check_hier(H); if (rc) return rc;
    ARG(l >= 0 && l < H->nlev && field >= 0 && field < SUHMO_F_COUNT);
    HIPCHK(hipSetDevice(H->device));
    return hier_ff(H, l, field, -1, corners != 0, HST(s));
}
extern "C" int suhmo_hier_cf_interp(suhmo_hier_t *H, int l, int field_f, int field_c, suhmo_stream_t s)
{
    int rc = check_hier(H); if (rc) return rc;
    ARG(l >= 1 && l < H->nlev && field_f >= 0 && field_f < SUHMO_F_COUNT && field_c >= 0 && field_c < SUHMO_F_COUNT);
    HIPCHK(hipSetDevice(H->device));
    return hier_cf(H, l, field_f, field_c, HST(s));
}
extern "C" int suhmo_hier_pwl_fill(suhmo_hier_t *H, int l, int field_f, int field_c, suhmo_stream_t s)
{
    int rc = check_hier(H); if (rc) return rc;
    ARG(l >= 1 && l < H->nlev && field_f >= 0 && field_f < SUHMO_F_COUNT && field_c >= 0 && field_c < SUHMO_F_COUNT);
    HIPCHK(hipSetDevice(H->device));
    return hier_pwl(H, l, field_f, field_c, HST(s));
}
extern "C" int suhmo_hier_average(suhmo_hier_t *H, int l, int field_f, int field_c, suhmo_stream_t s)
{
    int rc = check_hier(H); if (rc) return rc;
    ARG(l >= 1 && l < H->nlev && field_f >= 0 && field_f < SUHMO_F_COUNT && field_c >= 0 && field_c < SUHMO_F_COUNT);
    HIPCHK(hipSetDevice(H->device));
    return hier_avg(H, l, field_f, field_c, 0, 0.0, HST(s));
}
extern "C" int suhmo_hier_gsrb(suhmo_hier_t *H, int l, int sweeps, suhmo_stream_t s)
{
    int rc = check_hier(H); if (rc) return rc;
    ARG(l >= 0 && l < H->nlev && sweeps >= 0);
    HIPCHK(hipSetDevice(H->device));
    return hier_gsrb(H, l, sweeps, s);
}
extern "C" int suhmo_hier_update_operator(suhmo_hier_t *H, int l, suhmo_stream_t s)
{
    int rc = check_hier(H); if (rc) return rc;
// ... 90 lines not shown
```

### suhmo_amd/csrc/suhmo_hier_fill.hip

```cpp
#include "suhmo_hier_int.h"

using namespace hier;
namespace {
__device__ __forceinline__ double *fptr(const FP *tab, const FP &base, int use_base, int b, int field)
{
    return use_base ? base.f[field] : tab[b].f[field];
}
__device__ __forceinline__ void d_ff(const CopyEnt &c, const FP *__restrict__ tab, int f0, int f1)
{
    tab[c.d.b].f[f0][c.d.off] = tab[c.s.b].f[f0][c.s.off];
    if (f1 >= 0) tab[c.d.b].f[f1][c.d.off] = tab[c.s.b].f[f1][c.s.off];
}
__global__ void k_ff(const CopyEnt *__restrict__ e, int n, const FP *__restrict__ tab, int f0, int f1)
{
    int t = blockIdx.x * blockDim.x + threadIdx.x;
    if (t >= n) return;
    d_ff(e[t], tab, f0, f1);
}
__device__ __forceinline__ void d_cf(const CfEnt &q, const FP *__restrict__ ftab, int ff0, const FP *__restrict__ ctab, const FP &cbase,
                                     int use_base, int fc0, int ff1, int fc1)
{
    const double c_s = 8.0 / 15.0, c_b = 2.0 / 3.0, c_a = -0.2;
    const double xt = q.xsign ? 0.25 : -0.25;
  for (int pass = 0; pass < (ff1 >= 0 ? 2 : 1); pass++) {
// ... 516 lines not shown
    if (ff1 >= 0 && ((rc = ensure_field(H, l, ff1)) || (rc = ensure_field(H, l - 1, fc1)) || (rc = refresh_tables(H, l, st)))) return rc;
    { const int fl[2] = {fc, fc1};
      if (l == 1 && (rc = refresh_base(H, fl, ff1 >= 0 ? 2 : 1, st))) return rc; }
    if ((rc = coarse_args(H, l - 1, st, ca))) return rc;
    const DevVec<CopyEnt> &list = corners ? V.ff_all : V.ff_side;
    const int nbcf = (int)g1(V.cf.n).x, nbff = (int)g1(list.n).x;
    if (nbcf + nbff > 0)
        hipLaunchKernelGGL(k_cf_ff, dim3(nbcf + nbff), dim3(256), 0, st, V.cf.d, (int)V.cf.n, nbcf, list.d, (int)list.n, V.d_fp, ff, ca.tab, ca.base, ca.use_base, fc, ff1, fc1);
    HIPCHK(hipGetLastError());
    return 0;
}
int hier_pwl(suhmo_hier *H, int l, int ff, int fc, hipStream_t st)
{
    if (l == 0) return 0;
    HLev &V = H->lev[l];
    int rc;
    CoarseArgs ca;
    if ((rc = ensure_field(H, l, ff)) || (rc = ensure_field(H, l - 1, fc)) || (rc = refresh_tables(H, l, st))) return rc;
    if (l == 1 && (rc = refresh_base1(H, fc, st))) return rc;
    if (l > 1 && V.part && (rc = sync1(H, l - 1, V.sy_cread, fc, st))) return rc;
    if ((rc = coarse_args(H, l - 1, st, ca))) return rc;
    if (V.pwl.n) hipLaunchKernelGGL(k_pwl, g1(V.pwl.n), dim3(256), 0, st, V.pwl.d, (int)V.pwl.n, V.d_fp, ff, ca.tab, ca.base, ca.use_base, fc);
    HIPCHK(hipGetLastError());
    return 0;
}
int hier_avg(suhmo_hier *H, int l, int ff, int fc, int mode, double val, hipStream_t st)
{
    HLev &V = H->lev[l];
    int rc;
    CoarseArgs ca;
    if ((rc = ensure_field(H, l, ff)) || (rc = ensure_field(H, l - 1, fc)) || (rc = refresh_tables(H, l, st)) || (rc = coarse_args(H, l - 1, st, ca))) return rc;
    if (fc == SUHMO_F_PHI) { for (suhmo_level *L : H->lev[l - 1].box) L->d[0].phi_fresh = 0; H->phi_ver[l - 1]++; }
    if (fc == SUHMO_F_PHI && l == 1) H->phi_shadow_fresh = false;
    if (mode == 1) {
        if (V.avg_cov.n) {
            dim3 grd((V.cov_w + 63) / 64, (V.cov_h + 3) / 4, (unsigned)V.avg_cov.n);
            hipLaunchKernelGGL(k_avg, grd, dim3(64, 4), 0, st, V.avg_cov.d, V.d_fp, V.d_dv, ff, ca.tab, ca.dv, ca.dst, ca.ddv, ca.use_base, fc, mode, val);
        }
        HIPCHK(hipGetLastError());
        return 0;
    }
    if (V.avg.n) {
        dim3 grd((V.avg_w + 63) / 64, (V.avg_h + 3) / 4, (unsigned)V.avg.n);
        hipLaunchKernelGGL(k_avg, grd, dim3(64, 4), 0, st, V.avg.d, V.d_fp, V.d_dv, ff, ca.tab, ca.dv, ca.dst, ca.ddv, ca.use_base, fc, mode, val);
    }
    HIPCHK(hipGetLastError());
    if (V.part && V.put_stride) {
        SUHMO_TIME("hier: averages onto coarse cells other ranks hold");
        if (!H->ag) { suhmo_set_error("hier: level %d is partitioned over the ranks and no all-gather is attached", l); return -1; }
        if ((rc = part_staging(H, (size_t)V.put_stride, st))) return rc;
        if (V.avg_put.n) {
            dim3 grd((V.put_w + 63) / 64, (V.put_h + 3) / 4, (unsigned)V.avg_put.n);
            hipLaunchKernelGGL(k_avg_put, grd, dim3(64, 4), 0, st, V.avg_put.d, V.d_fp, V.d_dv, ff, H->ps);
        }
        HIPCHK(hipGetLastError());
        if ((rc = H->ag(H->ag_user, H->ps, V.put_stride, H->pr, (suhmo_stream_t)st))) return rc;
        H->part_gathers++;
        H->part_bytes += 8L * V.put_mine;
        if (V.avg_get.n) {
            dim3 grd((V.get_w + 63) / 64, (V.get_h + 3) / 4, (unsigned)V.avg_get.n);
            hipLaunchKernelGGL(k_put_unpack, grd, dim3(64, 4), 0, st, V.avg_get.d, ca.tab, ca.dv, ca.dst, ca.ddv, ca.use_base, fc, H->pr, V.put_stride);
        }
        HIPCHK(hipGetLastError());
    }
    return 0;
}
// ... 40 lines not shown
        if ((rc = multi_of(H, l - 1, st, mc))) return rc;
        const int cgx = (mc.maxnx + 2 + 63) / 64, cgy = (mc.maxny + 2 + 3) / 4;
        hipLaunchKernelGGL(k_prolong2_fused, dim3(nk + cgx * cgy * mc.nbox), dim3(256), (size_t)V.win_max * sizeof(double), st, V.wing.d, V.wstart.d, V.d_win, k0,
                           ca.tab, ca.dv, ca.base, ca.bdv, ca.use_base, (int)SUHMO_F_PHI, (const double *)nullptr, V.d_fp, V.d_dv, (int)SUHMO_F_PHIOLD, nk, cgx, cgy);
        HIPCHK(hipGetLastError());
        return 0;
    }
    if (H->fused_prolong && V.win_max <= 6144) {
        hipLaunchKernelGGL(k_prolong2_fused, dim3(nk), dim3(256), (size_t)V.win_max * sizeof(double), st, V.wing.d, V.wstart.d, V.d_win, k0,
                           ca.tab, ca.dv, ca.base, ca.bdv, ca.use_base, field_c, minus_saved ? V.winold : nullptr, V.d_fp, V.d_dv, -1, nk, 1, 1);
        HIPCHK(hipGetLastError());
        return 0;
    }
    if (V.wing.n) {
        dim3 grd((V.wing_w + 63) / 64, (V.wing_h + 3) / 4, (unsigned)V.wing.n);
        hipLaunchKernelGGL(k_win_gather, grd, dim3(64, 4), 0, st, V.wing.d, V.winbuf, ca.tab, ca.dv, ca.base, ca.bdv, ca.use_base, field_c, V.d_win, V.d_wing_box,
                           minus_saved ? V.winold : nullptr);
    }
    int maxp = 0, maxx = 0, maxy = 0;
    for (const Win &w : V.win) maxp = std::max(maxp, 2 * (w.nx - 2) + 2 * (w.ny - 2));
    for (suhmo_level *L : V.box) { maxx = std::max(maxx, L->d[0].v.nx); maxy = std::max(maxy, L->d[0].v.ny); }
    hipLaunchKernelGGL(k_win_bc, dim3((maxp + 255) / 256, nk), dim3(256), 0, st, V.d_win + k0, nk, V.winbuf, ca.bdv);
    hipLaunchKernelGGL(k_prolong2_win, dim3((maxx + 63) / 64, (maxy + 3) / 4, nk), dim3(64, 4), 0, st, V.d_win + k0, V.winbuf, V.d_fp + k0, V.d_dv + k0);
    HIPCHK(hipGetLastError());
    return 0;
}
int hier_reflux(suhmo_hier *H, int l, int field_c, hipStream_t st, int residual)
{
    SUHMO_TIME("VCAMRNonLinearPoissonOp::reflux");
    HLev &V = H->lev[l];
    int rc;
    CoarseArgs ca;
    if ((rc = ensure_field(H, l - 1, field_c)) || (rc = refresh_tables(H, l, st))) return rc;
    { const int fl[3] = {SUHMO_F_PHI, SUHMO_F_BX, SUHMO_F_BY};
      if (l == 1) { if ((rc = refresh_base(H, fl, 3, st))) return rc; }
      else if (V.part && (rc = sync_run(H, l - 1, V.sy_cread, fl, 3, st))) return rc;
      if (V.part && (rc = sync_run(H, l, V.sy_fface, fl, 3, st))) return rc; }
    if ((rc = coarse_args(H, l - 1, st, ca))) return rc;
    const DV &vc = H->lev[l - 1].box[0]->d[0].v;
    if (V.targets.n)
        hipLaunchKernelGGL(k_reflux, g1(V.targets.n), dim3(256), 0, st, V.targets.d, (int)V.targets.n, V.faces.d, V.d_fp, V.d_dv, ca.tab, ca.base, ca.dst,
                           ca.use_base, field_c, vc.dx, vc.dy, vc.beta, residual);
    HIPCHK(hipGetLastError());
    return 0;
}

int ghosts_levels(suhmo_hier *H, int llo, int lhi, suhmo_stream_t s)
{
    LvGhosts g;
    memset(&g, 0, sizeof(g));
    int rc, nb = 0;
    for (int l = std::max(1, llo); l <= lhi; l++) {
        HLev &V = H->lev[l];
        const bool cf_ok = H->cf_seen[l][0] == H->phi_ver[l] && H->cf_seen[l][1] == H->phi_ver[l - 1], ff_ok = H->ff_seen[l] == H->phi_ver[l];
        if (cf_ok && ff_ok) continue;
        if ((rc = ensure_field(H, l, SUHMO_F_PHI)) || (rc = ensure_field(H, l - 1, SUHMO_F_PHI)) || (rc = refresh_tables(H, l, HST(s)))) return rc;
        if (l - 1 >= 1 && (rc = refresh_tables(H, l - 1, HST(s)))) return rc;
        const int q = g.n++;
        g.cf[q] = V.cf.d; g.ncf[q] = (int)V.cf.n; g.nbcf[q] = (int)g1(V.cf.n).x;
        g.ff[q] = V.ff_side.d; g.nff[q] = (int)V.ff_side.n;
        g.nb[q] = g.nbcf[q] + (int)g1(V.ff_side.n).x;
        g.ftab[q] = V.d_fp; g.ctab[q] = l - 1 >= 1 ? H->lev[l - 1].d_fp : nullptr; g.use_base[q] = l - 1 == 0;
        nb += g.nb[q];
        H->cf_seen[l][0] = H->phi_ver[l]; H->cf_seen[l][1] = H->phi_ver[l - 1]; H->ff_seen[l] = H->phi_ver[l];
    }
    if (nb > 0) {
// ... 60 lines not shown
```

### suhmo_amd/csrc/suhmo_level.hip

```cpp
#include "suhmo_hier.h"
#include "suhmo_level_int.h"
#include <algorithm>
#include <cstdarg>
#include <cmath>
#include <initializer_list>

static thread_local char g_err[512] = "";
void suhmo_set_error(const char *fmt, ...)
{
    va_list ap; va_start(ap, fmt); vsnprintf(g_err, sizeof(g_err), fmt, ap); va_end(ap);
}
extern "C" const char *suhmo_last_error(void) { return g_err; }
#include <atomic>
#include <chrono>
#include <map>
#include <mutex>
namespace {
std::atomic<int> g_timer_mode{-1};
std::mutex g_timer_mu;
struct TimerRec { long count = 0; double total = 0.0; };
std::map<std::string, TimerRec> g_timers;
inline double now_s() { return std::chrono::duration<double>(std::chrono::steady_clock::now().time_since_epoch()).count(); }
inline int timer_mode()
{
// ... 112 lines not shown
    ARG(desc->i0 >= 0 && (desc->nx_global == 0 ? desc->i0 == 0 : desc->i0 + desc->nx <= desc->nx_global));
    ARG(desc->i0 % 2 == 0);
    ARG(desc->patch_ny == 0 || (desc->nx_global > 0 && desc->patch_j0 <= desc->j0 && desc->j0 + desc->ny <= desc->patch_j0 + desc->patch_ny));
    ARG((long)(desc->nx + 64) * (long)(desc->ny + 2 * (desc->halo_rows < 1 ? 1 : desc->halo_rows)) < (1L << 31));
    int ndev = 0;
    HIPCHK(hipGetDeviceCount(&ndev));
    if (ndev <= 0) { suhmo_set_error("no HIP device: the product path has no CPU fallback"); return -3; }
    ARG(desc->device >= 0 && desc->device < ndev);
    HIPCHK(hipSetDevice(desc->device));
    suhmo_level *L = new suhmo_level();
    L->desc = *desc; L->ph = desc->phys; L->device = desc->device; L->batch_owned = 0;
    L->ex = nullptr; L->ar = nullptr; L->ar2 = nullptr; L->ard = nullptr; L->user = nullptr; L->ex_begin = nullptr; L->ex_end = nullptr; L->rccl = nullptr;
        L->ipc = nullptr; L->ipc_owner = 0; L->faces_deferred = 0; L->gap = nullptr; L->gap_dt = 0.0; L->prof_on = 0; L->gsrb_variant = -1; L->fused_hc = 0;
    L->bcoef_fused = 1;
    L->bcoef_tile_x = 62;
    L->fused_nt = 64;
    L->fused_restrict = 1;
    L->gsrb_tile = 1; L->tile_t = 0; L->tile_s = 4;
    L->tile_max_cells = 3000000;
    L->fas_rhs_in_relax = 3;
    L->tile_chunks = 1;
    L->tile_order = 2; L->tile_restrict = 0;
    L->tile_strips = 1;
    L->overlap_halo = 1; L->xstream = nullptr; L->xev[0] = L->xev[1] = nullptr; L->overlapped = 0;
    L->strips_rhs_local = 1;
    L->fas_rhs_fused = 1;
    L->agg_min_cells = 100000; L->agg_depth = 0; L->agg_world = 1; L->agg_rank = 0; L->agg = nullptr; L->ag = nullptr; L->ag_user = nullptr;
    L->agg_send = L->agg_recv = nullptr; L->agg_cap = 0; L->agg_gathers = 0; L->agg_static_stale = 0;
    L->frhs_stream = L->frhs_tile = 0;
    L->resout_np = 0;
    L->resout_req = L->resout_armed = L->resout_done = 0; L->resout_rhs = nullptr; L->resout_count = 0; L->resid_in_relax = 1;
    L->graph_max_cells = 1500000; L->gstream = nullptr; L->vgraph_replays = 0; memset(L->vgraph_seen, 0, sizeof(L->vgraph_seen));
    L->fused_min_cells = 1000000;
    L->skip_mask = 1; L->poll_readback = 1;
    L->bottom_solver = 0; L->bottom_one_launch_max_cells = 16384;
    L->bottom_ctr = nullptr; L->bottom_host_iters = L->bottom_host_solves = 0;
    {
        struct IntKnob { const char *env; int suhmo_level::*field; };
        struct LongKnob { const char *env; long suhmo_level::*field; };
        static const IntKnob ints[] = {
            {"SUHMO_GSRB_VARIANT", &suhmo_level::gsrb_variant}, {"SUHMO_FUSED_HC", &suhmo_level::fused_hc}, {"SUHMO_BCOEF_FUSED", &suhmo_level::bcoef_fused},
            {"SUHMO_BCOEF_TILE_X", &suhmo_level::bcoef_tile_x}, {"SUHMO_FUSED_NT", &suhmo_level::fused_nt}, {"SUHMO_OVERLAP_HALO", &suhmo_level::overlap_halo},
            {"SUHMO_STRIPS_RHS_LOCAL", &suhmo_level::strips_rhs_local}, {"SUHMO_FAS_RHS_FUSED", &suhmo_level::fas_rhs_fused},
            {"SUHMO_RESID_IN_RELAX", &suhmo_level::resid_in_relax}, {"SUHMO_TILE_STRIPS", &suhmo_level::tile_strips}, {"SUHMO_TILE_CHUNKS", &suhmo_level::tile_chunks},
            {"SUHMO_TILE_RESTRICT", &suhmo_level::tile_restrict}, {"SUHMO_TILE_ORDER", &suhmo_level::tile_order}, {"SUHMO_FAS_RHS_IN_RELAX", &suhmo_level::fas_rhs_in_relax},
            {"SUHMO_TILE_S", &suhmo_level::tile_s}, {"SUHMO_GSRB_TILE", &suhmo_level::gsrb_tile}, {"SUHMO_TILE_T", &suhmo_level::tile_t},
            {"SUHMO_FUSED_RESTRICT", &suhmo_level::fused_restrict}, {"SUHMO_SKIP_MASK", &suhmo_level::skip_mask}, {"SUHMO_POLL_READBACK", &suhmo_level::poll_readback}};
        static const LongKnob longs[] = {
            {"SUHMO_AGG_MIN_CELLS", &suhmo_level::agg_min_cells}, {"SUHMO_TILE_MAX_CELLS", &suhmo_level::tile_max_cells},
            {"SUHMO_GRAPH_MAX_CELLS", &suhmo_level::graph_max_cells}, {"SUHMO_FUSED_MIN_CELLS", &suhmo_level::fused_min_cells},
            {"SUHMO_BOTTOM_ONE_LAUNCH_MAX_CELLS", &suhmo_level::bottom_one_launch_max_cells}};
        for (const IntKnob &k : ints) if (const char *e = getenv(k.env)) L->*(k.field) = atoi(e);
        for (const LongKnob &k : longs) if (const char *e = getenv(k.env)) L->*(k.field) = atol(e);
        L->fas_rhs_fused = L->fas_rhs_fused != 0;
        if (L->tile_order < 0 || L->tile_order > 2) L->tile_order = 0;
        if (L->tile_t != 16 && L->tile_t != 32) L->tile_t = 0;
    }
    if (desc->boxes && desc->nbox > 0) {
        L->boxes.assign(desc->boxes, desc->boxes + 4 * (size_t)desc->nbox);
    } else {
        int mb = desc->max_box > 0 ? desc->max_box : 64;
        for (int bj = 0; bj * mb < desc->ny; bj++)
            for (int bi = 0; bi * mb < desc->nx; bi++) {
                int lo0 = desc->i0 + bi * mb, lo1 = desc->j0 + bj * mb;
                int hi0 = std::min(lo0 + mb, desc->i0 + desc->nx) - 1, hi1 = std::min(lo1 + mb, desc->j0 + desc->ny) - 1;
                int b[4] = {lo0, lo1, hi0, hi1};
                L->boxes.insert(L->boxes.end(), b, b + 4);
            }
    }
    L->desc.boxes = nullptr;
    L->desc.nbox = (int)(L->boxes.size() / 4);
    {
        long cells = 0;
        for (size_t k = 0; k < L->boxes.size(); k += 4) {
            const int *b = &L->boxes[k];
            if (b[0] < desc->i0 || b[2] >= desc->i0 + desc->nx || b[1] < desc->j0 || b[3] >= desc->j0 + desc->ny || b[0] > b[2] || b[1] > b[3]) {
                suhmo_set_error("box %zu outside the strip", k / 4); delete L; return -1;
            }
            cells += (long)(b[2] - b[0] + 1) * (b[3] - b[1] + 1);
        }
        if (cells != (long)desc->nx * desc->ny) { suhmo_set_error("boxes do not tile the level"); delete L; return -1; }
    }
    L->ndepth = 1;
    for (int dep = 1; dep < SUHMO_MAXDEPTH; dep++) {
        if (!boxes_coarsenable(L->boxes, (1 << dep) * 2)) break;
        if ((desc->j0 % (1 << dep)) || (desc->ny_global % (1 << dep))) break;
        if ((desc->i0 % (2 << dep)) || (desc->nx_global % (1 << dep))) break;
        L->ndepth = dep + 1;
    }
    for (int dep = 0; dep < L->ndepth; dep++) {
        Depth &D = L->d[dep];
        make_dv(D.v, L->desc, dep);
        D.elems = (size_t)D.v.P * (size_t)(D.v.rows + 1);
        D.nbox = L->desc.nbox;
        memset(&D.fp, 0, sizeof(D.fp));
        D.phi_alt = nullptr; D.prolong_pending = 0; D.rhs_pending = 0; D.phi_fresh = 0;
    }
    L->scratch = nullptr; L->scratch_elems = 0; L->hscratch = nullptr; L->hscratch_dev = nullptr; L->hseq = 0;
    L->mask_epoch = 0; L->maskflag_epoch = 0; L->mask_reported = 0; L->coarse_mask_ok = 0;
    L->stub = 1;
    if (!stub) { int rc = level_storage(L); if (rc) { suhmo_level_destroy(L); return rc; } }
    *out = L;
    return 0;
}
static int level_storage(suhmo_level *L)
{
    static const int eager[] = {SUHMO_F_PHI, SUHMO_F_RHS, SUHMO_F_ACOEF, SUHMO_F_B, SUHMO_F_PI, SUHMO_F_ZB,
                                SUHMO_F_MASK, SUHMO_F_BX, SUHMO_F_BY, SUHMO_F_RES, SUHMO_F_LPHI};
    HIPCHK(hipSetDevice(L->device));
    L->stub = 0;
    for (int dep = 0; dep < L->ndepth; dep++) {
        for (int f : eager) {
            if (dep == 0 && f == SUHMO_F_LPHI) continue;
            if (!suhmo_field(L, dep, f)) { suhmo_set_error("hipMalloc failed (depth %d field %d)", dep, f); return -2; }
        }
        if (dep > 0) { suhmo_field(L, dep, SUHMO_F_PHIOLD); suhmo_field(L, dep, SUHMO_F_CORR); }
    }
    L->scratch_elems = 16384;
    HIPCHK(hipMalloc(&L->scratch, L->scratch_elems * sizeof(double)));
    HIPCHK(hipMemset(L->scratch, 0, L->scratch_elems * sizeof(double)));
    HIPCHK(hipHostMalloc(&L->hscratch, 64 * sizeof(double), hipHostMallocMapped | hipHostMallocCoherent));
    memset(L->hscratch, 0, 64 * sizeof(double));
    if (L->poll_readback && hipHostGetDevicePointer((void **)&L->hscratch_dev, L->hscratch, 0) != hipSuccess) { L->hscratch_dev = nullptr; L->poll_readback = 0; (void)hipGetLastError(); }
    return 0;
}

extern "C" int suhmo_level_destroy(suhmo_level_t *L)
{
    if (!L) return 0;
    if (L->batch_owned) { suhmo_set_error("this level is a member of a batch: suhmo_batch_destroy frees it"); return -1; }
    (void)hipSetDevice(L->device);
    (void)hipDeviceSynchronize();
    if (L->rccl) (void)suhmo_level_detach_rccl(L);
    if (L->gap) { (void)suhmo_level_destroy(L->gap); L->gap = nullptr; }
    suhmo_ipc_release(L);
    suhmo_agg_release(L);
    suhmo_level_drop_graphs(L);
    for (int dep = 0; dep < L->ndepth; dep++)
        for (int f = 0; f < SUHMO_F_COUNT; f++)
            if (L->d[dep].fp.f[f]) (void)hipFree(L->d[dep].fp.f[f]);
    for (int dep = 0; dep < L->ndepth; dep++)
        if (L->d[dep].phi_alt) (void)hipFree(L->d[dep].phi_alt);
    for (auto &pe : L->prof) { (void)hipEventDestroy(pe.a); (void)hipEventDestroy(pe.b); }
    if (L->xstream) { (void)hipStreamDestroy(L->xstream); (void)hipEventDestroy(L->xev[0]); (void)hipEventDestroy(L->xev[1]); }
    if (L->scratch) (void)hipFree(L->scratch);
    if (L->bottom_ctr) (void)hipFree(L->bottom_ctr);
    if (L->hscratch) (void)hipHostFree(L->hscratch);
    delete L;
    return 0;
}

static int remake_views(suhmo_level *L)
{
    for (int dep = 0; dep < L->ndepth; dep++) make_dv(L->d[dep].v, L->desc, dep);
    suhmo_level_drop_graphs(L);
    return 0;
}
extern "C" int suhmo_level_set_alpha_beta(suhmo_level_t *L, double alpha, double beta)
{
    ARG(L);
    L->desc.alpha = alpha; L->desc.beta = beta;
    if (L->agg) { int rc = suhmo_level_set_alpha_beta(L->agg, alpha, beta); if (rc) return rc; }
    return remake_views(L);
}
extern "C" int suhmo_level_set_bc(suhmo_level_t *L, const suhmo_bc_t *bc)
{
    ARG(L && bc);
    for (int d = 0; d < 2; d++)
        if ((bc->periodic[d] != 0) != (L->desc.bc.periodic[d] != 0)) { suhmo_set_error("setBC cannot change the periodicity of the domain"); return -1; }
    for (int d = 0; d < 2; d++) for (int s = 0; s < 2; s++) ARG(bc->type[d][s] == 0 || bc->type[d][s] == 1);
    L->desc.bc = *bc;
    if (L->agg) { int rc = suhmo_level_set_bc(L->agg, bc); if (rc) return rc; }
    return remake_views(L);
}

static long *option_slot_long(suhmo_level *L, const char *key)
{
    if (!strcmp(key, "fused_min_cells")) return &L->fused_min_cells;
    if (!strcmp(key, "tile_max_cells")) return &L->tile_max_cells;
    if (!strcmp(key, "graph_max_cells")) return &L->graph_max_cells;
    if (!strcmp(key, "agg_min_cells")) return &L->agg_min_cells;
    return nullptr;
}
static int *option_slot_int(suhmo_level *L, const char *key)
{
    static const struct { const char *k; int suhmo_level::*m; } tab[] = {
        {"gsrb_variant", &suhmo_level::gsrb_variant}, {"fused_hc", &suhmo_level::fused_hc}, {"bcoef_fused", &suhmo_level::bcoef_fused}, {"bcoef_tile_x", &suhmo_level::bcoef_tile_x},
        {"fused_nt", &suhmo_level::fused_nt}, {"fused_restrict", &suhmo_level::fused_restrict}, {"strips_rhs_local", &suhmo_level::strips_rhs_local},
        {"tile_strips", &suhmo_level::tile_strips}, {"overlap_halo", &suhmo_level::overlap_halo}, {"skip_mask", &suhmo_level::skip_mask}, {"tile_chunks",
            &suhmo_level::tile_chunks}, {"tile_order", &suhmo_level::tile_order}, {"tile_restrict", &suhmo_level::tile_restrict}, {"fas_rhs_in_relax",
            &suhmo_level::fas_rhs_in_relax}, {"resid_in_relax", &suhmo_level::resid_in_relax}, {"fas_rhs_fused", &suhmo_level::fas_rhs_fused},
        {"tile_s", &suhmo_level::tile_s}, {"gsrb_tile", &suhmo_level::gsrb_tile}, {"tile_t", &suhmo_level::tile_t}, {"poll_readback", &suhmo_level::poll_readback}};
    for (const auto &e : tab) if (!strcmp(key, e.k)) return &(L->*(e.m));
    return nullptr;
}
extern "C" int suhmo_level_set_option(suhmo_level_t *L, const char *key, long value)
{
    ARG(L && key);
    if (!strcmp(key, "bottom_solver")) {
        if (value != 0 && value != 1) { suhmo_set_error("bottom_solver: 0 (bottom relaxes only) or 1 (RelaxSolver)"); return -1; }
        return suhmo_bottom_configure(L, (int)value, L->bottom_one_launch_max_cells);
    }
    if (!strcmp(key, "bottom_one_launch_max_cells")) {
        if (value < 0) { suhmo_set_error("bottom_one_launch_max_cells: >= 0"); return -1; }
        return suhmo_bottom_configure(L, L->bottom_solver, value);
    }
    if (long *p = option_slot_long(L, key)) {
        *p = value; suhmo_level_drop_graphs(L);
        if (!strcmp(key, "agg_min_cells")) return suhmo_agg_setup(L);
        return 0;
    }
    if (int *p = option_slot_int(L, key)) {
        if (!strcmp(key, "tile_t") && value != 0 && value != 16 && value != 32) { suhmo_set_error("tile_t: 0 (by size), 16 or 32"); return -1; }
        if (!strcmp(key, "fused_nt") && value != 64 && value != 256) { suhmo_set_error("fused_nt: 64 or 256"); return -1; }
        if (!strcmp(key, "poll_readback") && value && !L->hscratch_dev) { suhmo_set_error("poll_readback: no device address of the host slot"); return -1; }
        *p = (int)value; suhmo_level_drop_graphs(L); return 0;
    }
    suhmo_set_error("unknown option '%s'", key);
    return -1;
}
extern "C" int suhmo_level_get_option(const suhmo_level_t *L, const char *key, long *value)
{
    ARG(L && key && value);
    if (long *p = option_slot_long(const_cast<suhmo_level *>(L), key)) { *value = *p; return 0; }
    if (int *p = option_slot_int(const_cast<suhmo_level *>(L), key)) { *value = *p; return 0; }
    if (!strcmp(key, "overlapped_launches")) { *value = L->overlapped; return 0; }
    if (!strcmp(key, "agg_gathers")) { *value = L->agg_gathers; return 0; }
    if (!strcmp(key, "rhs_in_streaming_launches")) { *value = L->frhs_stream; return 0; }
    if (!strcmp(key, "rhs_in_tile_launches")) { *value = L->frhs_tile; return 0; }
    if (!strcmp(key, "residual_in_relax_launches")) { *value = L->resout_count; return 0; }
    if (!strcmp(key, "vcycle_graph_replays")) { *value = L->vgraph_replays; return 0; }
    if (!strcmp(key, "bottom_solver")) { *value = L->bottom_solver; return 0; }
    if (!strcmp(key, "bottom_one_launch_max_cells")) { *value = L->bottom_one_launch_max_cells; return 0; }
    if (!strcmp(key, "bottom_solver_iterations")) { *value = suhmo_bottom_counter(L, 0); return 0; }
    if (!strcmp(key, "bottom_solves_one_launch")) { *value = suhmo_bottom_counter(L, 1); return 0; }
    if (!strcmp(key, "bottom_solves_host_loop")) { *value = suhmo_bottom_counter(L, 2); return 0; }
    suhmo_set_error("unknown option '%s'", key);
    return -1;
}

extern "C" int suhmo_level_num_depths(const suhmo_level_t *L) { return L ? L->ndepth : -1; }
extern "C" int suhmo_level_synchronize(suhmo_level_t *L, suhmo_stream_t s)
{
    ARG(L);
    HIPCHK(hipStreamSynchronize((hipStream_t)s));
    return 0;
}
extern "C" int suhmo_level_set_hooks(suhmo_level_t *L, suhmo_exchange_fn ex, suhmo_allreduce_max_fn ar, void *user)
{
    ARG(L);
    L->ex = ex; L->ar = ar; L->ar2 = nullptr; L->ard = nullptr; L->user = user; L->ex_begin = nullptr; L->ex_end = nullptr;
    return 0;
}
void suhmo_level_share_transport(suhmo_level *dst, const suhmo_level *src)
{
    dst->ex = src->ex; dst->ar = src->ar; dst->ar2 = src->ar2; dst->ard = src->ard; dst->user = src->user;
    dst->ex_begin = src->ex_begin; dst->ex_end = src->ex_end; dst->ipc = src->ipc;
}
extern "C" int suhmo_level_set_allgather(suhmo_level_t *L, suhmo_allgather_fn fn, void *user)
{
    ARG(L);
    HIPCHK(hipSetDevice(L->device));
    L->ag = fn; L->ag_user = user;
    return suhmo_agg_setup(L);
}
extern "C" int suhmo_level_agglomerated_depth(const suhmo_level_t *L) { return L ? L->agg_depth : -1; }
extern "C" int suhmo_level_set_reduce_hook(suhmo_level_t *L, suhmo_allreduce_fn fn)
{
    ARG(L);
    L->ar2 = fn;
    return 0;
}

extern "C" int suhmo_level_exchange(suhmo_level_t *L, int depth, int field, suhmo_stream_t s)
{
    ARG(L); ARG(depth >= 0 && depth < L->ndepth); ARG(field >= 0 && field < SUHMO_F_COUNT);
    const DV &v = L->d[depth].v;
    if (L->ex && (v.ext[0] || v.ext[1])) {
        if (!suhmo_field(L, depth, field)) return -2;
        int rc = L->ex(L->user, L, depth, &field, 1, s);
        if (!rc && field == SUHMO_F_PHI) L->d[depth].phi_fresh = suhmo_halo_rows(v);
        return rc;
    }
    return 0;
}
extern "C" int suhmo_level_halo_info(const suhmo_level_t *L, int depth, int *halo_rows, int *ext_lo, int *ext_hi, int *nx, int *ny)
{
    ARG(L); ARG(depth >= 0 && depth < L->ndepth);
    const DV &v = L->d[depth].v;
    if (halo_rows) *halo_rows = v.gy;
    if (ext_lo) *ext_lo = v.ext[0];
    if (ext_hi) *ext_hi = v.ext[1];
    if (nx) *nx = v.nx;
    if (ny) *ny = v.ny;
    return 0;
}


extern "C" int suhmo_level_field_view(suhmo_level_t *L, int depth, int field, double **base, long *pitch, long *origin)
{
    CHECK_DF(L, depth, field);
    double *p = suhmo_field(L, depth, field);
    if (!p) { suhmo_set_error("field allocation failed"); return -2; }
    if (base) *base = p;
    if (pitch) *pitch = L->d[depth].v.P;
    if (origin) *origin = cidx(L->d[depth].v, 0, 0);
    return 0;
}

static int copy2d(suhmo_level *L, int depth, int field, double *host, long hpitch, int i0, int j0, int ni, int nj,
                  bool to_canvas, bool on_device, hipStream_t st)
{
    if (ni <= 0 || nj <= 0) return 0;
    double *p = suhmo_field(L, depth, field);
    if (!p) { suhmo_set_error("field allocation failed"); return -2; }
    const DV &v = L->d[depth].v;
    double *c = p + cidx(v, i0, j0);
    hipMemcpyKind kind = to_canvas ? (on_device ? hipMemcpyDeviceToDevice : hipMemcpyHostToDevice)
                                   : (on_device ? hipMemcpyDeviceToDevice : hipMemcpyDeviceToHost);
    if (to_canvas)
        HIPCHK(hipMemcpy2DAsync(c, (size_t)v.P * 8, host, (size_t)hpitch * 8, (size_t)ni * 8, nj, kind, st));
    else
        HIPCHK(hipMemcpy2DAsync(host, (size_t)hpitch * 8, c, (size_t)v.P * 8, (size_t)ni * 8, nj, kind, st));
    return 0;
}

static int field_io(suhmo_level *L, int depth, int field, double *buf, int ghosted, int on_device, bool set, hipStream_t st)
{
    const DV &v = L->d[depth].v;
    int rc;
    if (is_xface(field)) rc = copy2d(L, depth, field, buf, v.nx + 1, 0, 0, v.nx + 1, v.ny, set, on_device, st);
    else if (is_yface(field)) rc = copy2d(L, depth, field, buf, v.nx, 0, 0, v.nx, v.ny + 1, set, on_device, st);
    else if (ghosted) rc = copy2d(L, depth, field, buf, v.nx + 2, -1, -1, v.nx + 2, v.ny + 2, set, on_device, st);
    else rc = copy2d(L, depth, field, buf, v.nx, 0, 0, v.nx, v.ny, set, on_device, st);
    if (rc) return rc;
    if (!on_device) HIPCHK(hipStreamSynchronize(st));
    return 0;
}

extern "C" int suhmo_level_set_field(suhmo_level_t *L, int depth, int field, const double *src, int ghosted,
                                     int on_device, suhmo_stream_t s)
{
    CHECK_DF(L, depth, field); ARG(src);
    HIPCHK(hipSetDevice(L->device));
    if (field == SUHMO_F_PHI) phi_changed(L, depth);
    if (field == SUHMO_F_MASK) { L->coarse_mask_ok = 0; L->maskflag_epoch = 0; }
    return field_io(L, depth, field, (double *)src, ghosted, on_device, true, (hipStream_t)s);
}
extern "C" int suhmo_level_get_field(suhmo_level_t *L, int depth, int field, double *dst, int ghosted,
                                     int on_device, suhmo_stream_t s)
{
    CHECK_DF(L, depth, field); ARG(dst);
    HIPCHK(hipSetDevice(L->device));
    return field_io(L, depth, field, dst, ghosted, on_device, false, (hipStream_t)s);
}

static void box_region(const suhmo_level *L, int depth, int field, int ibox, int r[4])
{
    const int *b = &L->boxes[4 * (size_t)ibox];
    int c = 1 << depth;
    r[0] = b[0] / c - L->d[depth].v.i0; r[1] = b[1] / c - L->d[depth].v.j0;
    r[2] = (b[2] + 1) / c - 1 - L->d[depth].v.i0; r[3] = (b[3] + 1) / c - 1 - L->d[depth].v.j0;
    if (is_xface(field)) r[2] += 1;
    if (is_yface(field)) r[3] += 1;
}

extern "C" int suhmo_level_put_box(suhmo_level_t *L, int depth, int field, int ibox, const double *fab,
                                   int flo0, int flo1, int fhi0, int fhi1, int with_domain_ghosts, suhmo_stream_t s)
{
    CHECK_DF(L, depth, field); ARG(fab); ARG(ibox >= 0 && ibox < L->desc.nbox);
    HIPCHK(hipSetDevice(L->device));
    hipStream_t st = (hipStream_t)s;
    const DV &v = L->d[depth].v;
    if (field == SUHMO_F_PHI) phi_changed(L, depth);
    if (field == SUHMO_F_MASK) { L->coarse_mask_ok = 0; L->maskflag_epoch = 0; }
    int r[4]; box_region(L, depth, field, ibox, r);
    int j0 = v.j0;
    flo0 -= v.i0; fhi0 -= v.i0;
    const bool patch = L->desc.nx_global > 0;
    long fp = fhi0 - flo0 + 1;
    ARG(flo0 <= r[0] && fhi0 >= r[2] && flo1 - j0 <= r[1] && fhi1 - j0 >= r[3]);
    double *h = (double *)fab;
    int rc = copy2d(L, depth, field, h + (long)(r[1] + j0 - flo1) * fp + (r[0] - flo0), fp, r[0], r[1],
                    r[2] - r[0] + 1, r[3] - r[1] + 1, true, false, st);
    if (rc) return rc;
    if (with_domain_ghosts && !is_face(field)) {
        if (r[0] == 0 && flo0 <= -1)
            rc |= copy2d(L, depth, field, h + (long)(r[1] + j0 - flo1) * fp + (-1 - flo0), fp, -1, r[1], 1, r[3] - r[1] + 1, true, false, st);
        if (r[2] == v.nx - 1 && fhi0 >= v.nx)
            rc |= copy2d(L, depth, field, h + (long)(r[1] + j0 - flo1) * fp + (v.nx - flo0), fp, v.nx, r[1], 1, r[3] - r[1] + 1, true, false, st);
        if (r[1] + j0 == 0 && flo1 <= -1)
            rc |= copy2d(L, depth, field, h + (long)(-1 - flo1) * fp + (r[0] - flo0), fp, r[0], -1 - j0, r[2] - r[0] + 1, 1, true, false, st);
        else if (patch && r[1] == 0 && flo1 <= j0 - 1)
            rc |= copy2d(L, depth, field, h + (long)(j0 - 1 - flo1) * fp + (r[0] - flo0), fp, r[0], -1, r[2] - r[0] + 1, 1, true, false, st);
        if (r[3] + j0 == v.nyg - 1 && fhi1 >= v.nyg)
            rc |= copy2d(L, depth, field, h + (long)(v.nyg - flo1) * fp + (r[0] - flo0), fp, r[0], v.nyg - j0, r[2] - r[0] + 1, 1, true, false, st);
        else if (patch && r[3] == v.ny - 1 && fhi1 >= j0 + v.ny)
            rc |= copy2d(L, depth, field, h + (long)(j0 + v.ny - flo1) * fp + (r[0] - flo0), fp, r[0], v.ny, r[2] - r[0] + 1, 1, true, false, st);
        if (rc) return rc;
    }
    HIPCHK(hipStreamSynchronize(st));
    return 0;
}

extern "C" int suhmo_level_get_box(suhmo_level_t *L, int depth, int field, int ibox, double *fab,
                                   int flo0, int flo1, int fhi0, int fhi1, suhmo_stream_t s)
{
    CHECK_DF(L, depth, field); ARG(fab); ARG(ibox >= 0 && ibox < L->desc.nbox);
// ... 12 lines not shown
    return 0;
}

__global__ void k_pack_rows(DV v, const double *__restrict__ p, int jstart, int rows, double *__restrict__ buf)
{
    int i = blockIdx.x * blockDim.x + threadIdx.x, r = blockIdx.y * blockDim.y + threadIdx.y;
    if (i > v.nx || r >= rows) return;
    buf[(size_t)r * (v.nx + 1) + i] = p[cidx(v, i, jstart + r)];
}
__global__ void k_unpack_rows(DV v, double *__restrict__ p, int jstart, int rows, const double *__restrict__ buf)
{
    int i = blockIdx.x * blockDim.x + threadIdx.x, r = blockIdx.y * blockDim.y + threadIdx.y;
    if (i > v.nx || r >= rows) return;
    p[cidx(v, i, jstart + r)] = buf[(size_t)r * (v.nx + 1) + i];
}
extern "C" int suhmo_level_pack_rows(suhmo_level_t *L, int depth, int field, int side, int rows, double *dev_buf, suhmo_stream_t s)
{
    CHECK_DF(L, depth, field); ARG(dev_buf); ARG(side == 0 || side == 1);
    const DV &v = L->d[depth].v;
    ARG(rows >= 1 && rows <= v.gy && rows <= v.ny);
    HIPCHK(hipSetDevice(L->device));
    int jstart = side == 0 ? 0 : v.ny - rows;
    if (field == SUHMO_F_BY && side == 0) jstart = 1;
    hipLaunchKernelGGL(k_pack_rows, grid2d(v.nx + 1, rows), BLK2D, 0, (hipStream_t)s, v, suhmo_field(L, depth, field), jstart, rows, dev_buf);
    HIPCHK(hipGetLastError());
    return 0;
}
extern "C" int suhmo_level_unpack_rows(suhmo_level_t *L, int depth, int field, int side, int rows, const double *dev_buf, suhmo_stream_t s)
{
    CHECK_DF(L, depth, field); ARG(dev_buf); ARG(side == 0 || side == 1);
    const DV &v = L->d[depth].v;
    ARG(rows >= 1 && rows <= v.gy);
    HIPCHK(hipSetDevice(L->device));
    int jstart = side == 0 ? -rows : v.ny;
    if (field == SUHMO_F_BY && side == 1) jstart = v.ny + 1;
    hipLaunchKernelGGL(k_unpack_rows, grid2d(v.nx + 1, rows), BLK2D, 0, (hipStream_t)s, v, suhmo_field(L, depth, field), jstart, rows, dev_buf);
    HIPCHK(hipGetLastError());
    return 0;
}

extern "C" int suhmo_level_profile_enable(suhmo_level_t *L, int on) { ARG(L); L->prof_on = on; return 0; }
extern "C" int suhmo_level_profile_reset(suhmo_level_t *L)
{
    ARG(L);
    for (auto &pe : L->prof) { (void)hipEventDestroy(pe.a); (void)hipEventDestroy(pe.b); }
    L->prof.clear();
    return 0;
}
static int profile_read_kind(suhmo_level_t *L, suhmo_stream_t s, int kind, double *ms_total, long *launches, long *cells);
extern "C" int suhmo_level_profile_read(suhmo_level_t *L, suhmo_stream_t s, double *ms_total, long *launches, long *cells)
{ return profile_read_kind(L, s, 0, ms_total, launches, cells); }
extern "C" int suhmo_level_profile_read_restricting(suhmo_level_t *L, suhmo_stream_t s, double *ms_total, long *launches, long *cells)
{ return profile_read_kind(L, s, 1, ms_total, launches, cells); }
static int profile_read_kind(suhmo_level_t *L, suhmo_stream_t s, int kind, double *ms_total, long *launches, long *cells)
{
    ARG(L);
    HIPCHK(hipStreamSynchronize((hipStream_t)s));
    double tot = 0.0; long n = 0, c = 0;
    for (auto &pe : L->prof) {
        if (pe.restricts != kind) continue;
        float ms = 0.f;
        HIPCHK(hipEventElapsedTime(&ms, pe.a, pe.b));
        tot += ms; n++; c += pe.cells;
    }
    if (ms_total) *ms_total = tot;
    if (launches) *launches = n;
// ... 5 lines not shown
```

### suhmo_amd/csrc/suhmo_ops.hip

```cpp
#include "suhmo_hier.h"
#include "suhmo_level_int.h"
#include "suhmo_batch.h"
#include <algorithm>
#include <cmath>
#include <initializer_list>

__device__ __forceinline__ void d_fill_ghosts(const DV &v, double *__restrict__ p, int homog)
{
    int t = blockIdx.x * blockDim.x + threadIdx.x;
    if (t < 2 * v.ny) {
        int side = t / v.ny, j = t % v.ny;
        if (v.cfx[side]) return;
        int i = side ? v.nx - 1 : 0;
        int idx = cidx(v, i, j);
        double c = p[idx];
        if (side) p[idx + 1] = phiE(v, p, idx, i, c, homog); else p[idx - 1] = phiW(v, p, idx, i, c, homog);
        return;
    }
    t -= 2 * v.ny;
    if (t < 2 * v.nx) {
        int side = t / v.nx, i = t % v.nx;
        if (v.ext[side]) return;
        int j = side ? v.ny - 1 : 0;
        int idx = cidx(v, i, j);
        double c = p[idx];
        if (side) p[idx + v.P] = phiN(v, p, idx, j, c, homog); else p[idx - v.P] = phiS(v, p, idx, j, c, homog);
    }
}
template <class T> __global__ void k_fill_ghosts(T t, int field, int homog) { d_fill_ghosts(t.view(), t.field(field), homog); }
template <class T> int launch_fill_ghosts(const T &t, int field, int homog, hipStream_t st) { return launch_over(k_fill_ghosts<T>, t, PERIMETER, st, field, homog); }
template int launch_fill_ghosts(const OnBoxes &, int, int, hipStream_t);
template int launch_fill_ghosts(const OnMembers &, int, int, hipStream_t);

extern "C" int suhmo_level_fill_ghosts(suhmo_level_t *L, int depth, int field, int homogeneous, suhmo_stream_t s)
{
    CHECK_DF(L, depth, field); ARG(!is_face(field));
    HIPCHK(hipSetDevice(L->device));
    if (!suhmo_field(L, depth, field)) return -2;
    return launch_fill_ghosts(on_level(L, depth), field, homogeneous, (hipStream_t)s);
}

template <bool HAS_ALPHA, int MODE>
__device__ __forceinline__ double d_apply_at(const DV &v, const FP &fp, suhmo_phys_t ph, int homog, int halo, int hcomp, int i, int j)
{
    if (i >= v.nx || j >= v.ny + halo) return 0.0;
    const double *__restrict__ phi = fp.f[SUHMO_F_PHI];
    int idx = cidx(v, i, j);
    if (MODE == 2 && (j < 0 || j >= v.ny)) {
        const bool comp = (j < 0 && v.rk[0] && j >= -hcomp) || (j >= v.ny && v.rk[1] && j < v.ny + hcomp);
        if (!comp) { fp.f[SUHMO_F_PHIOLD][idx] = phi[idx]; return 0.0; }
    }
    double c = phi[idx];
    double e = phiE(v, phi, idx, i, c, homog), w = phiW(v, phi, idx, i, c, homog);
    double n = phiN(v, phi, idx, j, c, homog), s = phiS(v, phi, idx, j, c, homog);
    double bxW = fp.f[SUHMO_F_BX][idx], bxE = fp.f[SUHMO_F_BX][idx + 1];
    double byS = fp.f[SUHMO_F_BY][idx], byN = fp.f[SUHMO_F_BY][idx + v.P];
    double nl, dnl;
    nl_terms(ph, c, fp.f[SUHMO_F_B][idx], fp.f[SUHMO_F_PI][idx], fp.f[SUHMO_F_ZB][idx], fp.f[SUHMO_F_MASK][idx], nl, dnl);
    double aterm = HAS_ALPHA ? v.alpha * fp.f[SUHMO_F_ACOEF][idx] : v.alpha;
    double lofphi = lofphi_cell(v, aterm, c, e, w, n, s, bxE, bxW, byN, byS, nl);
    double res = 0.0;
    if (MODE == 0) fp.f[SUHMO_F_LPHI][idx] = lofphi;
    else if (MODE == 1) fp.f[SUHMO_F_RES][idx] = res = fp.f[SUHMO_F_RHS][idx] - lofphi;
    else if (MODE == 3) { fp.f[SUHMO_F_LPHI][idx] = lofphi; fp.f[SUHMO_F_RES][idx] = res = -1.0 * lofphi + 1.0 * fp.f[SUHMO_F_RHS][idx]; }
    else {
        fp.f[SUHMO_F_LPHI][idx] = lofphi;
        fp.f[SUHMO_F_RHS][idx] = 1.0 * fp.f[SUHMO_F_RES][idx] + 1.0 * lofphi;
        fp.f[SUHMO_F_PHIOLD][idx] = c;
    }
    return res;
}
// ... 55 lines not shown
        if (t < lv.n && q < 0) { if (z < lv.nbox[t]) { q = t; k = z; } else z -= lv.nbox[t]; }
    return q >= 0;
}
#define LV_PICK(lv, q, member, out) do { _Pragma("unroll") for (int t_ = 0; t_ < SUHMO_LVMAX; t_++) if (t_ == (q)) (out) = (lv).member[t_]; } while (0)
template <bool HAS_ALPHA>
__global__ __launch_bounds__(256) void k_apply_lv(suhmo_lvboxes lv, suhmo_phys_t ph)
{
    int q, k;
    if (!lv_find(lv, q, k)) return;
    const DV *dv = nullptr; const FP *fp = nullptr; int mode = 1;
    LV_PICK(lv, q, dv, dv); LV_PICK(lv, q, fp, fp); LV_PICK(lv, q, mode, mode);
    if (mode == 1) d_apply<HAS_ALPHA, 1>(dv[k], fp[k], ph, 0, 0, 0);
    else d_apply<HAS_ALPHA, 3>(dv[k], fp[k], ph, 0, 0, 0);
}
int suhmo_levels_apply(const suhmo_lvboxes &lv, const suhmo_phys_t &ph, bool has_alpha, hipStream_t st)
{
    int nz = 0;
    for (int q = 0; q < lv.n; q++) nz += lv.nbox[q];
    if (nz <= 0) return 0;
    const dim3 grd((lv.maxnx + 63) / 64, (lv.maxny + 3) / 4, nz);
    if (has_alpha) hipLaunchKernelGGL(k_apply_lv<true>, grd, BLK2D, 0, st, lv, ph);
    else hipLaunchKernelGGL(k_apply_lv<false>, grd, BLK2D, 0, st, lv, ph);
    HIPCHK(hipGetLastError());
    return 0;
}

int suhmo_exchange_fields(suhmo_level *L, int depth, std::initializer_list<int> fields, hipStream_t st)
{
    const DV &v = L->d[depth].v;
    if (!(L->ex && (v.ext[0] || v.ext[1]))) return 0;
    for (int f : fields) if (!suhmo_field(L, depth, f)) return -2;
    int rc = L->ex(L->user, L, depth, fields.begin(), (int)fields.size(), (suhmo_stream_t)st);
    if (!rc) for (int f : fields) if (f == SUHMO_F_PHI) L->d[depth].phi_fresh = suhmo_halo_rows(v);
    return rc;
}
int suhmo_exchange_list(suhmo_level *L, int depth, const int *fields, int n, hipStream_t st)
{
    const DV &v = L->d[depth].v;
    if (!(L->ex && (v.ext[0] || v.ext[1]))) return 0;
    for (int k = 0; k < n; k++) if (!suhmo_field(L, depth, fields[k])) return -2;
    int rc = L->ex(L->user, L, depth, fields, n, (suhmo_stream_t)st);
    if (!rc) for (int k = 0; k < n; k++) if (fields[k] == SUHMO_F_PHI) L->d[depth].phi_fresh = suhmo_halo_rows(v);
    return rc;
}
int suhmo_ensure_phi_halo(suhmo_level *L, int depth, int need, hipStream_t st)
{
    Depth &D = L->d[depth];
    if (!(L->ex && (D.v.ext[0] || D.v.ext[1]))) return 0;
    if (D.phi_fresh >= need) return 0;
    return suhmo_exchange_fields(L, depth, {SUHMO_F_PHI}, st);
}

extern "C" int suhmo_level_apply_op(suhmo_level_t *L, int depth, int homogeneous, suhmo_stream_t s)
{
    SUHMO_TIME("VCAMRNonLinearPoissonOp::applyOpI");
    ARG(L); ARG(depth >= 0 && depth < L->ndepth);
    HIPCHK(hipSetDevice(L->device));
    Depth &D = L->d[depth];
    if (!suhmo_field(L, depth, SUHMO_F_LPHI)) return -2;
    int rc = suhmo_ensure_phi_halo(L, depth, 1, (hipStream_t)s); if (rc) return rc;
    return launch_apply<0>(on_level(L, depth), D.v.alpha != 0.0, homogeneous, (hipStream_t)s);
}

int suhmo_apply_and_residual(suhmo_level *L, int depth, hipStream_t st)
{
    SUHMO_TIME("VCAMRNonLinearPoissonOp::applyOpI");
    Depth &D = L->d[depth];
    if (!suhmo_field(L, depth, SUHMO_F_LPHI) || !suhmo_field(L, depth, SUHMO_F_RES)) return -2;
    int rc = suhmo_ensure_phi_halo(L, depth, 1, st); if (rc) return rc;
    return launch_apply<3>(on_level(L, depth), D.v.alpha != 0.0, 0, st);
}

int suhmo_apply_and_residual_rects(suhmo_level *L, int depth, const int4 *d_rects, int n, int maxw, int maxh, hipStream_t st)
{
    SUHMO_TIME("VCAMRNonLinearPoissonOp::applyOpI");
// ... 247 lines not shown
    int idx = cidx(v, i, j), cc = cidx(vc, ic, jc);
    double p = phi[idx];
    p = p + fx2 * c[cc] + f0 * c[cc + o1 + o2 * vc.P];
    p = p + fx1 * (c[cc + o1] + c[cc + o2 * vc.P]);
    phi[idx] = p;
}
extern "C" int suhmo_level_prolong_bilinear(suhmo_level_t *L, int depth, suhmo_stream_t s)
{
    ARG(L); ARG(depth >= 0 && depth + 1 < L->ndepth);
    HIPCHK(hipSetDevice(L->device));
    Depth &D = L->d[depth], &C = L->d[depth + 1];
    phi_changed(L, depth);
    hipLaunchKernelGGL(k_prolong2, grid2d(D.v.nx, D.v.ny), BLK2D, 0, (hipStream_t)s, D.v, D.fp.f[SUHMO_F_PHI], C.v, C.fp.f[SUHMO_F_CORR]);
    HIPCHK(hipGetLastError());
    return 0;
}

__global__ void k_divergence(DV v, const double *__restrict__ ux, const double *__restrict__ uy, double *__restrict__ div)
{
    int i = blockIdx.x * blockDim.x + threadIdx.x, j = blockIdx.y * blockDim.y + threadIdx.y;
    if (i >= v.nx || j >= v.ny) return;
    int idx = cidx(v, i, j);
    double d = div[idx];
    d = d + v.fdx * (ux[idx + 1] - ux[idx]);
    d = d + v.fdy * (uy[idx + v.P] - uy[idx]);
    div[idx] = d;
}
extern "C" int suhmo_level_divergence(suhmo_level_t *L, int depth, int dst_field, suhmo_stream_t s)
{
    CHECK_DF(L, depth, dst_field); ARG(!is_face(dst_field));
    HIPCHK(hipSetDevice(L->device));
    Depth &D = L->d[depth];
    double *dst = suhmo_field(L, depth, dst_field);
    hipLaunchKernelGGL(k_divergence, grid2d(D.v.nx, D.v.ny), BLK2D, 0, (hipStream_t)s, D.v, D.fp.f[SUHMO_F_BX], D.fp.f[SUHMO_F_BY], dst);
    HIPCHK(hipGetLastError());
    return 0;
}

__global__ void k_getflux(DV v, FP fp, int dir, double scale, double *__restrict__ out)
{
    int i = blockIdx.x * blockDim.x + threadIdx.x, j = blockIdx.y * blockDim.y + threadIdx.y;
    int nxf = dir == 0 ? v.nx + 1 : v.nx, nyf = dir == 0 ? v.ny : v.ny + 1;
    if (i >= nxf || j >= nyf) return;
    const double *__restrict__ phi = fp.f[SUHMO_F_PHI];
    int idx = cidx(v, i, j);
    double phihi = phi[idx], philo = dir == 0 ? phi[idx - 1] : phi[idx - v.P];
    double gradphi = (phihi - philo) * scale;
    out[(size_t)j * nxf + i] = -fp.f[dir == 0 ? SUHMO_F_BX : SUHMO_F_BY][idx] * gradphi;
}
extern "C" int suhmo_level_get_flux(suhmo_level_t *L, int depth, int dir, int ref, double *flux_host, suhmo_stream_t s)
{
    ARG(L); ARG(depth >= 0 && depth < L->ndepth); ARG(dir == 0 || dir == 1); ARG(flux_host);
    HIPCHK(hipSetDevice(L->device));
    hipStream_t st = (hipStream_t)s;
    Depth &D = L->d[depth];
    int rc = suhmo_level_fill_ghosts(L, depth, SUHMO_F_PHI, 0, s); if (rc) return rc;
    int nxf = dir == 0 ? D.v.nx + 1 : D.v.nx, nyf = dir == 0 ? D.v.ny : D.v.ny + 1;
    double *tmp = nullptr;
    HIPCHK(hipMalloc(&tmp, (size_t)nxf * nyf * 8));
    double scale = D.v.beta * ref / (dir == 0 ? D.v.dx : D.v.dy);
    hipLaunchKernelGGL(k_getflux, grid2d(nxf, nyf), BLK2D, 0, st, D.v, D.fp, dir, scale, tmp);
    HIPCHK(hipMemcpyAsync(flux_host, tmp, (size_t)nxf * nyf * 8, hipMemcpyDeviceToHost, st));
    HIPCHK(hipStreamSynchronize(st));
    HIPCHK(hipFree(tmp));
    return 0;
}

__device__ __forceinline__ void d_axby(const DV &v, double *__restrict__ dst, const double *__restrict__ x, const double *__restrict__ y, double a, double b)
{
    int i = blockIdx.x * blockDim.x + threadIdx.x, j = blockIdx.y * blockDim.y + threadIdx.y;
    if (i >= v.nx || j >= v.ny) return;
    int idx = cidx(v, i, j);
    dst[idx] = a * x[idx] + b * y[idx];
}
template <class T> __global__ void k_axby(T t, int fd, int fx, int fy, double a, double b)
{
    d_axby(t.view(), t.field(fd), t.field(fx), t.field(fy), a, b);
}
template <class T> int launch_axby(const T &t, int fd, int fx, int fy, double a, double b, hipStream_t st) { return launch_over(k_axby<T>, t, CELLS, st, fd, fx, fy, a, b); }
template int launch_axby(const OnBoxes &, int, int, int, double, double, hipStream_t);
__global__ void k_setval(DV v, double *__restrict__ dst, double val)
{
    int i = blockIdx.x * blockDim.x + threadIdx.x, j = blockIdx.y * blockDim.y + threadIdx.y;
    if (i >= v.nx || j >= v.ny) return;
    dst[cidx(v, i, j)] = val;
}
extern "C" int suhmo_level_axby(suhmo_level_t *L, int depth, int dst, int x, int y, double a, double b, suhmo_stream_t s)
{
    CHECK_DF(L, depth, dst); CHECK_DF(L, depth, x); CHECK_DF(L, depth, y);
    HIPCHK(hipSetDevice(L->device));
    if (!suhmo_field(L, depth, dst) || !suhmo_field(L, depth, x) || !suhmo_field(L, depth, y)) return -2;
    if (dst == SUHMO_F_PHI) phi_changed(L, depth);
    if (dst == SUHMO_F_MASK) { L->coarse_mask_ok = 0; L->maskflag_epoch = 0; }
    return launch_axby(on_level(L, depth), dst, x, y, a, b, (hipStream_t)s);
}
extern "C" int suhmo_level_set_value(suhmo_level_t *L, int depth, int field, double val, suhmo_stream_t s)
{
    CHECK_DF(L, depth, field);
    HIPCHK(hipSetDevice(L->device));
    Depth &D = L->d[depth];
    if (field == SUHMO_F_PHI) phi_changed(L, depth);
    if (field == SUHMO_F_MASK) { L->coarse_mask_ok = 0; L->maskflag_epoch = 0; }
    hipLaunchKernelGGL(k_setval, grid2d(D.v.nx, D.v.ny), BLK2D, 0, (hipStream_t)s, D.v, suhmo_field(L, depth, field), val);
    HIPCHK(hipGetLastError());
    return 0;
}

__global__ __launch_bounds__(256) void k_norm_partial(DV v, const double *__restrict__ x, int ord, double *__restrict__ partial)
{
    __shared__ double sm[256];
    int tid = threadIdx.y * blockDim.x + threadIdx.x;
    double acc = 0.0;
    for (int j = blockIdx.y * blockDim.y + threadIdx.y; j < v.ny; j += gridDim.y * blockDim.y)
        for (int i = blockIdx.x * blockDim.x + threadIdx.x; i < v.nx; i += gridDim.x * blockDim.x) {
            double val = x[cidx(v, i, j)];
            if (ord == 0) acc = fmax(acc, fabs(val)); else acc += val * val;
        }
    sm[tid] = acc;
    __syncthreads();
    for (int s = 128; s > 0; s >>= 1) {
        if (tid < s) sm[tid] = ord == 0 ? fmax(sm[tid], sm[tid + s]) : sm[tid] + sm[tid + s];
        __syncthreads();
    }
    if (tid == 0) partial[blockIdx.y * gridDim.x + blockIdx.x] = sm[0];
}
__global__ void k_norm_final(const double *__restrict__ partial, int n, int ord, double *__restrict__ out, HostSlot hs)
{
    __shared__ double sm[256];
    int tid = threadIdx.x;
    double acc = 0.0;
    for (int k = tid; k < n; k += 256) acc = ord == 0 ? fmax(acc, partial[k]) : acc + partial[k];
    sm[tid] = acc;
    __syncthreads();
    for (int s = 128; s > 0; s >>= 1) {
        if (tid < s) sm[tid] = ord == 0 ? fmax(sm[tid], sm[tid + s]) : sm[tid] + sm[tid + s];
// ... 336 lines not shown
```

Before: 480.1 V-cycles/s.

## Track ice-mask cleanliness and use unmasked bcoef/relax kernels when mask is trivial

Adds a mask version/state tracker that is invalidated on every mask write. The fused bcoef kernel asynchronously scans the mask for small or negative values and reads the result back through an event. Once the mask is known to be clean, depth-0 bcoef launches a template variant that skips mask loads, shared-memory staging and flag reporting, which cuts memory traffic. This is gated by a new 'mask_known' knob and adds state-tracking complexity, so a missed invalidation would give wrong coefficients.

```diff
diff --git a/suhmo_amd/csrc/suhmo_amr.hip b/suhmo_amd/csrc/suhmo_amr.hip
--- a/suhmo_amd/csrc/suhmo_amr.hip
+++ b/suhmo_amd/csrc/suhmo_amr.hip
@@ -211,6 +211,7 @@
     double *pf = suhmo_field(F, 0, field_f), *pc = suhmo_field(C, 0, field_c);
     if (!pf || !pc) { suhmo_set_error("field allocation failed"); return -2; }
     if (field_c == SUHMO_F_PHI) C->d[0].phi_fresh = 0;
+    if (field_c == SUHMO_F_MASK) suhmo_mask_written(C);
     hipLaunchKernelGGL(k_amr_average, dim3((vf.nx / 2 + 63) / 64, (vf.ny / 2 + 3) / 4), dim3(64, 4), 0, (hipStream_t)s, vf, pf, vc, pc);
     HIPCHK(hipGetLastError());
     return 0;
@@ -237,6 +238,7 @@
     double *p = suhmo_field(C, 0, field_c);
     if (!p) { suhmo_set_error("field allocation failed"); return -2; }
     if ((rc = suhmo_amr2_cf_interp(C, F, SUHMO_F_PHI, SUHMO_F_PHI, s))) return rc;
+    if (field_c == SUHMO_F_MASK) suhmo_mask_written(C);
     int n = vf.ny + vf.nx;
     hipLaunchKernelGGL(k_amr_reflux, dim3((n + 255) / 256), dim3(256), 0, (hipStream_t)s, vf, F->d[0].fp, vc, C->d[0].fp, p);
     HIPCHK(hipGetLastError());
@@ -280,7 +282,7 @@
     hipLaunchKernelGGL(k_amr_average_faces, dim3((vf.nx / 2 + 1 + 63) / 64, (vf.ny / 2 + 1 + 3) / 4), dim3(64, 4), 0, (hipStream_t)s, vf,
                        F->d[0].fp.f[SUHMO_F_BX], F->d[0].fp.f[SUHMO_F_BY], vc, C->d[0].fp.f[SUHMO_F_BX], C->d[0].fp.f[SUHMO_F_BY]);
     HIPCHK(hipGetLastError());
-    C->coarse_mask_ok = 0;
+    suhmo_mask_written(C);
     suhmo_level_drop_graphs(C);
     return 0;
 }
@@ -309,6 +311,7 @@
     double *p = suhmo_field(C, 0, field_c);
     if (!p) { suhmo_set_error("field allocation failed"); return -2; }
     if (field_c == SUHMO_F_PHI) C->d[0].phi_fresh = 0;
+    if (field_c == SUHMO_F_MASK) suhmo_mask_written(C);
     hipLaunchKernelGGL(k_amr_set_covered, dim3((vf.nx / 2 + 63) / 64, (vf.ny / 2 + 3) / 4), dim3(64, 4), 0, (hipStream_t)s, vf, vc, p, value);
     HIPCHK(hipGetLastError());
     return 0;
diff --git a/suhmo_amd/csrc/suhmo_bcoef.hip b/suhmo_amd/csrc/suhmo_bcoef.hip
--- a/suhmo_amd/csrc/suhmo_bcoef.hip
+++ b/suhmo_amd/csrc/suhmo_bcoef.hip
@@ -178,10 +178,11 @@
     }
 }
 
-template <bool INTERIOR, int BT_X, int BT_Y>
-__device__ __forceinline__ void bcoef_tile(const DV &v, const FP &fp, const suhmo_phys_t &ph, int hasMask, double *sphi, double *sB, double *sM,
-                                           unsigned *negflag, unsigned epoch)
-{
+template <bool INTERIOR, int BT_X, int BT_Y, bool MASKED>
+__device__ __forceinline__ void bcoef_tile(const DV &v, const FP &fp, const suhmo_phys_t &ph, int hasMask_, double *sphi, double *sB, double *sM,
+                                           unsigned *negflag, unsigned epoch, unsigned *smallflag)
+{
+    const int hasMask = MASKED ? hasMask_ : 0;
     constexpr int PW = BT_X + 4, PH = BT_Y + 4;
     constexpr int RW = BT_X + 2, RH = BT_Y + 2;
     constexpr int TX = BT_X + 2, TY = 256 / TX;
@@ -222,18 +223,23 @@
     const bool xi = xin(i);
     double Br[NK];
     bool hasB[NK];
-    bool neg = false;
+    bool neg = false, small = false;
 #pragma unroll
     for (int k = 0; k < NK; k++) {
         const int lj = ty + TY * k, j = j0 - 1 + lj;
         hasB[k] = INTERIOR || (i >= -1 && i <= v.nx && j >= -v.gy && j <= v.ny + v.gy - 1 && !((i < 0 || i >= v.nx) && (j < 0 || j >= v.ny)));
         double b = 0.0, m = 0.0;
-        if (hasB[k]) { int idx = cidx(v, i, j); b = Bf[idx]; m = mk[idx]; }
-        neg = neg || (m < 0.0 && i >= 0 && i < v.nx && j >= 0 && j < v.ny);
+        if (hasB[k]) { int idx = cidx(v, i, j); b = Bf[idx]; if (MASKED) m = mk[idx]; }
+        if (MASKED) {
+            neg = neg || (m < 0.0 && i >= 0 && i < v.nx && j >= 0 && j < v.ny);
+            small = small || (hasB[k] && m < 1e-6 && j >= -1 && j <= v.ny);
+        }
         Br[k] = b;
-        sB[lj * RW + tx] = b; sM[lj * RW + tx] = m;
-    }
-    if (negflag && neg) *negflag = epoch;
+        sB[lj * RW + tx] = b;
+        if (MASKED) sM[lj * RW + tx] = m;
+    }
+    if (MASKED && negflag && neg) *negflag = epoch;
+    if (MASKED && smallflag && small) *smallflag = 1u;
     __syncthreads();
     auto gradcc = [&](int p, int gi, int gj, double &gx, double &gy) {
         double c = sphi[p], w = sphi[p - 1], e = sphi[p + 1], s = sphi[p - PW], n = sphi[p + PW];
@@ -287,52 +293,85 @@
         for (int fy = ty; fy < nyt; fy += TY) {
             const int j = j0 + fy, idx = cidx(v, i, j), r = (fy + 1) * RW + tx;
             if (INTERIOR || j < v.ny)
-                bxo[idx] = bcoef_face(ph, sre[r], sre[r - 1], sB[r], sB[r - 1], sM[r], sM[r - 1], !INTERIOR && (i == 0 || i == v.nx));
+                bxo[idx] = bcoef_face(ph, sre[r], sre[r - 1], sB[r], sB[r - 1], MASKED ? sM[r] : 1.0, MASKED ? sM[r - 1] : 1.0, !INTERIOR && (i == 0 || i == v.nx));
             if (INTERIOR || i < v.nx) {
                 int jg = j + v.j0;
-                byo[idx] = bcoef_face(ph, sre[r], sre[r - RW], sB[r], sB[r - RW], sM[r], sM[r - RW], !INTERIOR && (jg == 0 || jg == v.nyg));
+                byo[idx] = bcoef_face(ph, sre[r], sre[r - RW], sB[r], sB[r - RW], MASKED ? sM[r] : 1.0, MASKED ? sM[r - RW] : 1.0, !INTERIOR && (jg == 0 || jg == v.nyg));
             }
         }
     }
 }
 struct MaskHalo { const double *m[SUHMO_MAXDEPTH]; int nx[SUHMO_MAXDEPTH], ny[SUHMO_MAXDEPTH], P[SUHMO_MAXDEPTH], gy[SUHMO_MAXDEPTH]; int nd, lo, hi; };
-__global__ __launch_bounds__(256) void k_mask_halo_report(MaskHalo h, unsigned *negflag, unsigned epoch)
+__global__ __launch_bounds__(256) void k_mask_halo_report(MaskHalo h, unsigned *negflag, unsigned epoch, unsigned *smallflag)
 {
     const int d = blockIdx.z, i = blockIdx.x * blockDim.x + threadIdx.x;
     if (d >= h.nd || i >= h.nx[d]) return;
     const int g = h.gy[d];
-    bool neg = false;
+    bool neg = false, small = false;
     for (int r = blockIdx.y; r < 2 * g; r += gridDim.y) {
         const bool top = r >= g;
         if (top ? !h.hi : !h.lo) continue;
         const int j = top ? h.ny[d] + (r - g) : -1 - r;
-        neg = neg || h.m[d][(long)(j + g) * h.P[d] + SUHMO_XOFF + i] < 0.0;
-    }
-    if (neg) *negflag = epoch;
-}
-template <int BT_X, int BT_Y>
-__device__ __forceinline__ void d_bcoef_fused(const DV &v, const FP &fp, const suhmo_phys_t &ph, int hasMask, unsigned *negflag, unsigned epoch)
-{
-    __shared__ double sphi[(BT_X + 4) * (BT_Y + 4)], sB[(BT_X + 2) * (BT_Y + 2)], sM[(BT_X + 2) * (BT_Y + 2)];
+        const double *__restrict__ row = h.m[d] + (long)(j + g) * h.P[d] + SUHMO_XOFF;
+        const double m = row[i];
+        neg = neg || m < 0.0;
+        const int dist = top ? r - g : r;
+        small = small || ((d == 0 && dist < 2) ? m < 1e-6 : m < 0.0);
+        if (smallflag && d == 0 && i == 0 && (j == -1 || j == h.ny[d])) small = small || row[-1] < 1e-6 || row[h.nx[d]] < 1e-6;
+    }
+    if (negflag && neg) *negflag = epoch;
+    if (smallflag && small) *smallflag = 1u;
+}
+template <int BT_X, int BT_Y, bool MASKED>
+__device__ __forceinline__ void d_bcoef_fused(const DV &v, const FP &fp, const suhmo_phys_t &ph, int hasMask, unsigned *negflag, unsigned epoch, unsigned *smallflag)
+{
+    __shared__ double sphi[(BT_X + 4) * (BT_Y + 4)], sB[(BT_X + 2) * (BT_Y + 2)], sM[MASKED ? (BT_X + 2) * (BT_Y + 2) : 1];
     const int i0 = blockIdx.x * BT_X, j0 = blockIdx.y * BT_Y;
     const bool interior = i0 - 2 >= 0 && i0 + BT_X + 1 <= v.nx - 1 && j0 - 2 >= 0 && j0 + BT_Y + 1 <= v.ny - 1;
-    if (interior) bcoef_tile<true, BT_X, BT_Y>(v, fp, ph, hasMask, sphi, sB, sM, negflag, epoch);
-    else bcoef_tile<false, BT_X, BT_Y>(v, fp, ph, hasMask, sphi, sB, sM, negflag, epoch);
-}
-template <class T, int BT_X, int BT_Y>
-__global__ __launch_bounds__(256) void k_bcoef_fused(T t, unsigned *negflag, unsigned epoch)
+    if (interior) bcoef_tile<true, BT_X, BT_Y, MASKED>(v, fp, ph, hasMask, sphi, sB, sM, negflag, epoch, smallflag);
+    else bcoef_tile<false, BT_X, BT_Y, MASKED>(v, fp, ph, hasMask, sphi, sB, sM, negflag, epoch, smallflag);
+}
+template <class T, int BT_X, int BT_Y, bool MASKED = true>
+__global__ __launch_bounds__(256) void k_bcoef_fused(T t, unsigned *negflag, unsigned epoch, unsigned *smallflag)
 {
     const suhmo_phys_t ph = t.phys();
-    if (std::is_same<T, OnMembers>::value) { negflag = nullptr; epoch = 0u; }
-    d_bcoef_fused<BT_X, BT_Y>(t.view(), t.fields(), ph, ph.use_mask_gradients, negflag, epoch);
-}
-template <class T> int launch_bcoef_fused(const T &t, bool wide, unsigned *flag, unsigned epoch, hipStream_t st)
-{
-    if constexpr (std::is_same<T, OnLevel>::value)
-        if (wide) return launch_grid(k_bcoef_fused<T, 126, 14>, t, dim3((t.nx() + 125) / 126, (t.ny() + 13) / 14), dim3(128, 2), st, flag, epoch);
-    return launch_grid(k_bcoef_fused<T, 62, 14>, t, dim3((t.nx() + 61) / 62, (t.ny() + 13) / 14), dim3(64, 4), st, flag, epoch);
-}
-template int launch_bcoef_fused(const OnMembers &, bool, unsigned *, unsigned, hipStream_t);
+    if (std::is_same<T, OnMembers>::value) { negflag = nullptr; epoch = 0u; smallflag = nullptr; }
+    d_bcoef_fused<BT_X, BT_Y, MASKED>(t.view(), t.fields(), ph, ph.use_mask_gradients, negflag, epoch, smallflag);
+}
+template <class T> int launch_bcoef_fused(const T &t, bool wide, unsigned *flag, unsigned epoch, hipStream_t st, unsigned *small, bool unmasked)
+{
+    if constexpr (std::is_same<T, OnLevel>::value) {
+        const dim3 gw((t.nx() + 125) / 126, (t.ny() + 13) / 14), gn((t.nx() + 61) / 62, (t.ny() + 13) / 14);
+        unsigned *const none = nullptr;
+        if (unmasked && wide) return launch_grid(k_bcoef_fused<T, 126, 14, false>, t, gw, dim3(128, 2), st, none, 0u, none);
+        if (unmasked) return launch_grid(k_bcoef_fused<T, 62, 14, false>, t, gn, dim3(64, 4), st, none, 0u, none);
+        if (wide) return launch_grid(k_bcoef_fused<T, 126, 14>, t, gw, dim3(128, 2), st, flag, epoch, small);
+    }
+    return launch_grid(k_bcoef_fused<T, 62, 14>, t, dim3((t.nx() + 61) / 62, (t.ny() + 13) / 14), dim3(64, 4), st, flag, epoch, small);
+}
+template int launch_bcoef_fused(const OnMembers &, bool, unsigned *, unsigned, hipStream_t, unsigned *, bool);
+void suhmo_mask_poll(suhmo_level *L)
+{
+    if (!L->mask_scan_pending) return;
+    const hipError_t e = hipEventQuery(L->mask_ev);
+    if (e == hipErrorNotReady) { (void)hipGetLastError(); return; }
+    L->mask_scan_pending = 0;
+    if (e != hipSuccess) { (void)hipGetLastError(); L->mask_scan_errors++; return; }
+    if (L->mask_scan_version == L->mask_version) L->mask_state = *(volatile unsigned *)L->mask_host ? SUHMO_MASK_DIRTY : SUHMO_MASK_CLEAN;
+}
+int suhmo_mask_scan_begin(suhmo_level *L, hipStream_t st)
+{
+    if (!L->mask_ev) HIPCHK(hipEventCreateWithFlags(&L->mask_ev, hipEventDisableTiming));
+    HIPCHK(hipMemsetAsync(suhmo_mask_scan_word(L), 0, sizeof(unsigned), st));
+    return 0;
+}
+int suhmo_mask_scan_end(suhmo_level *L, hipStream_t st)
+{
+    HIPCHK(hipMemcpyAsync(L->mask_host, suhmo_mask_scan_word(L), sizeof(unsigned), hipMemcpyDeviceToHost, st));
+    HIPCHK(hipEventRecord(L->mask_ev, st));
+    L->mask_scan_pending = 1; L->mask_scan_version = L->mask_version; L->mask_scans++;
+    return 0;
+}
 template <class T> int launch_re(const T &t, hipStream_t st) { return launch_over(k_re<T>, t, GHOSTED, st); }
 template <class T> int launch_bcoef_faces(const T &t, hipStream_t st) { return launch_over(k_bcoef_faces<T>, t, FACES, st); }
 template <class T> int launch_grad_cc(const T &t, hipStream_t st)
@@ -348,6 +387,17 @@
 template int launch_bcoef_faces(const OnMembers &, hipStream_t);
 template int launch_grad_cc(const OnMembers &, hipStream_t);
 
+static bool bcoef_is_fused(const suhmo_level *L, int depth)
+{
+    const Depth &D = L->d[depth];
+    return L->bcoef_fused && D.v.nx >= 4 && D.v.ny >= 4 && (!(D.v.ext[0] || D.v.ext[1]) || (D.v.gy >= 2 && D.v.ny >= 2))
+           && L->desc.nx_global == 0;
+}
+bool suhmo_mask_would_scan(const suhmo_level *L)
+{
+    return L->mask_known && !L->mask_view && L->mask_scan_errors < 3 && L->mask_state == SUHMO_MASK_UNKNOWN && !L->mask_scan_pending && L->mask_host
+           && !L->mask_capturing && bcoef_is_fused(L, 0);
+}
 extern "C" int suhmo_level_update_operator(suhmo_level_t *L, int depth, suhmo_stream_t s)
 {
     SUHMO_TIME("VCAMRNonLinearPoissonOp::UpdateOperator");
@@ -355,20 +405,26 @@
     HIPCHK(hipSetDevice(L->device));
     hipStream_t st = (hipStream_t)s;
     Depth &D = L->d[depth];
-    bool fused = L->bcoef_fused && D.v.nx >= 4 && D.v.ny >= 4 && (!(D.v.ext[0] || D.v.ext[1]) || (D.v.gy >= 2 && D.v.ny >= 2))
-                 && L->desc.nx_global == 0;
+    const bool fused = bcoef_is_fused(L, depth);
     int rc = suhmo_ensure_phi_halo(L, depth, fused ? 2 : 1, st); if (rc) return rc;
     if (fused) {
         const bool wide = L->bcoef_tile_x == 126 && D.v.nx >= 256;
         unsigned *flag = nullptr;
         if (depth == 0) { L->maskflag_epoch = 0; L->mask_reported = 0; }
-        if (depth == 0 && L->skip_mask) {
-            flag = (unsigned *)(L->scratch + L->scratch_elems - 1);
+        if (depth == 0 && !L->mask_capturing) suhmo_mask_poll(L);
+        const bool unmasked = depth == 0 && suhmo_mask_clean(L, 0);
+        unsigned *small = nullptr;
+        const bool scan = depth == 0 && suhmo_mask_would_scan(L);
+        if (scan) { small = suhmo_mask_scan_word(L); if ((rc = suhmo_mask_scan_begin(L, st))) return rc; }
+        if (depth == 0 && L->mask_capturing && L->mask_known && !L->mask_view && !unmasked && L->mask_host) { small = suhmo_mask_scan_word(L); L->mask_scan_captured = 1; }
+        if (depth == 0 && L->skip_mask && !unmasked) {
+            flag = suhmo_mask_report_word(L);
             if (++L->mask_epoch == 0) L->mask_epoch = 1;
             L->mask_reported = 1;
         }
-        if ((rc = launch_bcoef_fused(on_level(L, depth), wide, flag, L->mask_epoch, st))) return rc;
-        if (flag && (D.v.ext[0] || D.v.ext[1])) {
+        if ((rc = launch_bcoef_fused(on_level(L, depth), wide, flag, L->mask_epoch, st, small, unmasked))) return rc;
+        if (unmasked) L->bcoef_unmasked++;
+        if ((flag || small) && (D.v.ext[0] || D.v.ext[1])) {
             MaskHalo h;
             h.nd = 0; h.lo = D.v.ext[0]; h.hi = D.v.ext[1];
             const int last = L->coarse_mask_ok ? (L->agg ? L->agg_depth : L->ndepth) : 1;
@@ -379,8 +435,9 @@
                 if (Dk.v.gy > gmax) gmax = Dk.v.gy;
                 h.nd = k + 1;
             }
-            hipLaunchKernelGGL(k_mask_halo_report, dim3((D.v.nx + 255) / 256, 2 * gmax, h.nd), dim3(256), 0, st, h, flag, L->mask_epoch);
-        }
+            hipLaunchKernelGGL(k_mask_halo_report, dim3((D.v.nx + 255) / 256, 2 * gmax, h.nd), dim3(256), 0, st, h, flag, L->mask_epoch, small);
+        }
+        if (scan && (rc = suhmo_mask_scan_end(L, st))) return rc;
     } else {
         if (depth == 0) { L->maskflag_epoch = 0; L->mask_reported = 0; }
         if (!suhmo_field(L, depth, SUHMO_F_GRADX) || !suhmo_field(L, depth, SUHMO_F_GRADY) || !suhmo_field(L, depth, SUHMO_F_RE)) return -2;
@@ -707,6 +764,7 @@
         if (L->agg && dep >= L->agg_depth) continue;
         rc = suhmo_exchange_fields(L, dep, {SUHMO_F_ACOEF, SUHMO_F_B, SUHMO_F_PI, SUHMO_F_ZB, SUHMO_F_MASK}, st); if (rc) return rc;
     }
+    if (!L->coarse_mask_ok && (L->d[0].v.ext[0] || L->d[0].v.ext[1])) suhmo_mask_halo_written(L);
     L->coarse_mask_ok = 1;
     return suhmo_agg_gather_static(L, with_faces, st);
 }
diff --git a/suhmo_amd/csrc/suhmo_common.h b/suhmo_amd/csrc/suhmo_common.h
--- a/suhmo_amd/csrc/suhmo_common.h
+++ b/suhmo_amd/csrc/suhmo_common.h
@@ -120,6 +120,8 @@
     double *p1[SUHMO_MAXDEPTH], *a1[SUHMO_MAXDEPTH];
     double *rhs;
     int rout_req, rout_done, rout_np; const double *rout_rhs;
+    int mask_clean; long n_bcoef_unmasked, n_relax_unmasked;
+    int has_scan;
 };
 struct ProfEv { hipEvent_t a, b; long cells; int restricts; };
 
@@ -176,6 +178,14 @@
     int mask_reported;
     int coarse_mask_ok;
     unsigned mask_epoch, maskflag_epoch;
+    int mask_known, mask_state;
+    unsigned mask_version, mask_scan_version;
+    int mask_scan_pending, mask_capturing;
+    int mask_scan_captured;
+    int mask_view;
+    int mask_scan_errors;
+    unsigned *mask_host; hipEvent_t mask_ev;
+    long mask_scans, bcoef_unmasked, relax_unmasked;
     int overlap_halo;
     hipStream_t xstream; hipEvent_t xev[2]; long overlapped;
     int tile_strips;
@@ -190,6 +200,25 @@
     int gsrb_tile, tile_t, tile_s;
 };
 
+enum { SUHMO_MASK_UNKNOWN = 0, SUHMO_MASK_CLEAN = 1, SUHMO_MASK_DIRTY = 2 };
+static inline void suhmo_mask_written(suhmo_level *L)
+{
+    L->coarse_mask_ok = 0; L->maskflag_epoch = 0;
+    L->mask_version++; L->mask_state = SUHMO_MASK_UNKNOWN;
+}
+static inline void suhmo_mask_halo_written(suhmo_level *L) { L->mask_version++; L->mask_state = SUHMO_MASK_UNKNOWN; }
+bool suhmo_mask_would_scan(const suhmo_level *L);
+#define SUHMO_HSCRATCH_DOUBLES 64
+#define SUHMO_HSCRATCH_MASK 60
+static inline unsigned *suhmo_mask_report_word(const suhmo_level *L) { return (unsigned *)(L->scratch + L->scratch_elems - 1); }
+static inline unsigned *suhmo_mask_scan_word(const suhmo_level *L) { return suhmo_mask_report_word(L) + 1; }
+int suhmo_mask_scan_begin(suhmo_level *L, hipStream_t st);
+int suhmo_mask_scan_end(suhmo_level *L, hipStream_t st);
+void suhmo_mask_poll(suhmo_level *L);
+static inline bool suhmo_mask_clean(const suhmo_level *L, int depth)
+{
+    return L->mask_known && !L->mask_view && L->mask_state == SUHMO_MASK_CLEAN && (depth == 0 || L->coarse_mask_ok) && L->desc.nx_global == 0;
+}
 void suhmo_set_error(const char *fmt, ...);
 struct SuhmoTimer { const char *name; double t0; int mode; explicit SuhmoTimer(const char *n); ~SuhmoTimer(); };
 #define SUHMO_TIME(label) SuhmoTimer suhmo_tm_(label)
diff --git a/suhmo_amd/csrc/suhmo_fas.hip b/suhmo_amd/csrc/suhmo_fas.hip
--- a/suhmo_amd/csrc/suhmo_fas.hip
+++ b/suhmo_amd/csrc/suhmo_fas.hip
@@ -108,38 +108,56 @@
 {
     done = false;
     const int key[4] = {sp->num_smooth, sp->num_bottom, sp->bcoeff_otf, nd};
+    const int mask_clean = (suhmo_mask_clean(L, 0) ? 1 : 0) | (L->ndepth > 1 && suhmo_mask_clean(L, 1) ? 2 : 0);
+    const bool scanning = sp->bcoeff_otf && suhmo_mask_would_scan(L);
+    auto launch = [&](const VGraph &g) {
+        int rc = 0;
+        if (scanning && (rc = suhmo_mask_scan_begin(L, (hipStream_t)s))) return rc;
+        HIPCHK(hipGraphLaunch(g.exec, (hipStream_t)s)); L->vgraph_replays++;
+        if (scanning && (rc = suhmo_mask_scan_end(L, (hipStream_t)s))) return rc;
+        return 0;
+    };
+    auto replayed = [&](const VGraph &g) {
+        L->bcoef_unmasked += g.n_bcoef_unmasked; L->relax_unmasked += g.n_relax_unmasked;
+        if (g.rout_done) { L->resout_done = 1; L->resout_count++; L->resout_np = g.rout_np; }
+    };
     auto at_start = [&](const VGraph &g) {
-        if (memcmp(g.key, key, sizeof(key))) return false;
+        if (memcmp(g.key, key, sizeof(key)) || g.mask_clean != mask_clean) return false;
         for (int d = 0; d < L->ndepth; d++) if (L->d[d].fp.f[SUHMO_F_PHI] != g.p0[d] || L->d[d].phi_alt != g.a0[d]) return false;
         if (g.rout_req != (L->resid_in_relax ? L->resout_req : 0) || g.rout_rhs != L->resout_rhs) return false;
         return L->d[0].fp.f[SUHMO_F_RHS] == g.rhs;
     };
     for (const VGraph &g : L->vgraphs)
         if (at_start(g)) {
-            if (!g.exec) return 0;
-            HIPCHK(hipGraphLaunch(g.exec, (hipStream_t)s)); L->vgraph_replays++;
+            if (!g.exec || (scanning && !g.has_scan)) return 0;
+            { int rc = launch(g); if (rc) return rc; }
             for (int d = 0; d < L->ndepth; d++) { L->d[d].fp.f[SUHMO_F_PHI] = g.p1[d]; L->d[d].phi_alt = g.a1[d]; } suhmo_fp_changed();
-            if (g.rout_done) { L->resout_done = 1; L->resout_count++; L->resout_np = g.rout_np; }
+            replayed(g);
             done = true;
             return 0;
         }
     for (int k = 0; k < 4; k++) if (L->vgraph_seen[k] != key[k]) { memcpy(L->vgraph_seen, key, sizeof(key)); return 0; }
     if (L->vgraphs.size() >= 16) return 0;
     if (!L->gstream) HIPCHK(hipStreamCreateWithFlags(&L->gstream, hipStreamNonBlocking));
-    VGraph g; memcpy(g.key, key, sizeof(key)); g.exec = nullptr;
+    VGraph g; memcpy(g.key, key, sizeof(key)); g.exec = nullptr; g.mask_clean = mask_clean; g.has_scan = 0;
     for (int d = 0; d < SUHMO_MAXDEPTH; d++) { g.p0[d] = g.a0[d] = g.p1[d] = g.a1[d] = nullptr; }
     for (int d = 0; d < L->ndepth; d++) { g.p0[d] = L->d[d].fp.f[SUHMO_F_PHI]; g.a0[d] = L->d[d].phi_alt; }
     g.rhs = L->d[0].fp.f[SUHMO_F_RHS];
     g.rout_req = L->resid_in_relax ? L->resout_req : 0; g.rout_rhs = L->resout_rhs; g.rout_done = 0;
     const int rout_before = L->resout_done; const long rout_count = L->resout_count;
+    const long bcoef_unmasked = L->bcoef_unmasked, relax_unmasked = L->relax_unmasked;
     HIPCHK(hipStreamSynchronize((hipStream_t)s));
     hipGraph_t graph = nullptr;
     hipError_t e = hipStreamBeginCapture(L->gstream, hipStreamCaptureModeThreadLocal);
     int rc = 0;
     if (e == hipSuccess) {
+        L->mask_capturing = 1; L->mask_scan_captured = 0;
         rc = vcycle_body(L, sp, nd, (suhmo_stream_t)L->gstream);
+        L->mask_capturing = 0; g.has_scan = L->mask_scan_captured;
         e = hipStreamEndCapture(L->gstream, &graph);
     }
+    g.n_bcoef_unmasked = L->bcoef_unmasked - bcoef_unmasked; g.n_relax_unmasked = L->relax_unmasked - relax_unmasked;
+    L->bcoef_unmasked = bcoef_unmasked; L->relax_unmasked = relax_unmasked;
     g.rout_done = L->resout_count != rout_count;
     g.rout_np = L->resout_np;
     L->resout_done = rout_before; L->resout_count = rout_count;
@@ -155,10 +173,10 @@
     if (graph) (void)hipGraphDestroy(graph);
     (void)hipGetLastError();
     L->vgraphs.push_back(g);
-    if (!g.exec) return 0;
-    HIPCHK(hipGraphLaunch(g.exec, (hipStream_t)s)); L->vgraph_replays++;
+    if (!g.exec || (scanning && !g.has_scan)) return 0;
+    if ((rc = launch(g))) return rc;
     for (int d = 0; d < L->ndepth; d++) { L->d[d].fp.f[SUHMO_F_PHI] = g.p1[d]; L->d[d].phi_alt = g.a1[d]; } suhmo_fp_changed();
-    if (g.rout_done) { L->resout_done = 1; L->resout_count++; L->resout_np = g.rout_np; }
+    replayed(g);
     done = true;
     return 0;
 }
@@ -172,6 +190,7 @@
     const Depth &D = L->d[0];
     const bool ext = D.v.ext[0] || D.v.ext[1];
     const bool host_bottom = L->bottom_solver && !suhmo_bottom_one_launch(L, nd - 1);
+    suhmo_mask_poll(L);
     if (L->graph_max_cells > 0 && !L->ex && !ext && !L->prof_on && !host_bottom && (long)D.v.nx * D.v.ny <= L->graph_max_cells) {
         bool done = false;
         int rc = vcycle_graph(L, sp, nd, s, done);
diff --git a/suhmo_amd/csrc/suhmo_gsrb.hip b/suhmo_amd/csrc/suhmo_gsrb.hip
--- a/suhmo_amd/csrc/suhmo_gsrb.hip
+++ b/suhmo_amd/csrc/suhmo_gsrb.hip
@@ -243,21 +243,29 @@
     double *onorm;
 };
 
-struct RowCoef {
-    double rhs[2], B[2], Pi[2], zb[2], mask[2], a[2], byS[2], byN[2];
+template <bool MASKED> struct RowMask { double mask[2]; };
+template <> struct RowMask<false> {};
+template <bool MASKED>
+struct RowCoef : RowMask<MASKED> {
+    double rhs[2], B[2], Pi[2], zb[2], a[2], byS[2], byN[2];
     double bx0, bx1, bx2;
 };
+template <bool MASKED> __device__ __forceinline__ double row_mask(const RowCoef<MASKED> &q, int a)
+{
+    if constexpr (MASKED) return q.mask[a]; else return 1.0;
+}
 #define CP2(d, s, f) d.f[0] = s.f[0]; d.f[1] = s.f[1]
-template <bool HAS_ALPHA>
-__device__ __forceinline__ void copy_coef(RowCoef &d, const RowCoef &s)
-{
-    CP2(d, s, rhs); CP2(d, s, B); CP2(d, s, Pi); CP2(d, s, zb); CP2(d, s, mask);
+template <bool HAS_ALPHA, bool MASKED>
+__device__ __forceinline__ void copy_coef(RowCoef<MASKED> &d, const RowCoef<MASKED> &s)
+{
+    CP2(d, s, rhs); CP2(d, s, B); CP2(d, s, Pi); CP2(d, s, zb);
+    if constexpr (MASKED) { CP2(d, s, mask); }
     if (HAS_ALPHA) { CP2(d, s, a); }
     CP2(d, s, byS); CP2(d, s, byN);
     d.bx0 = s.bx0; d.bx1 = s.bx1; d.bx2 = s.bx2;
 }
 
-template <int K, bool HAS_ALPHA, int NT, int RM = 0, bool FRHS = false>
+template <int K, bool HAS_ALPHA, int NT, int RM = 0, bool FRHS = false, bool MASKED = true>
 __global__ __launch_bounds__(NT) void k_gsrb_fused(DV v, FP fp, const double *__restrict__ pin,
                                                    double *__restrict__ pout, suhmo_phys_t ph, FusedGeom g)
 {
@@ -296,14 +304,15 @@
     auto wrapj = [&](int j) { if (g.wrap_y) { if (j < 0) j += v.ny; else if (j >= v.ny) j -= v.ny; } return j; };
     auto ld2 = [&](const double *__restrict__ p, int idx) { return *reinterpret_cast<const double2 *>(p + idx); };
 
-    RowCoef cf0, cf1, cf2, cf3, cf4, cf5;
+    RowCoef<MASKED> cf0, cf1, cf2, cf3, cf4, cf5;
     double racc = 0.0, raccp = 0.0;
     double nmax = 0.0;
     const bool xbc = !v.per[0] && (c0 - HX <= 0 || c0 + g.W + HX >= v.nx);
     const bool ybc = !v.per[1] && (jmin <= 0 || jmax >= v.ny - 1);
     double2 pnext = make_double2(0.0, 0.0);
     double2 pprev = make_double2(0.0, 0.0);
-    const bool usemask = !g.negflag || *g.negflag == g.mask_epoch;
+    bool usemask = false;
+    if constexpr (MASKED) usemask = !g.negflag || *g.negflag == g.mask_epoch;
 
     int sr = 0;
     auto ring = [](int x) { return x < 0 ? x + R : x; };
@@ -324,7 +333,7 @@
 #define LD2(dst, p, ix) { double2 t_ = ld2(p, ix); dst[0] = t_.x; dst[1] = t_.y; }
             LD2(cf0.rhs, (FRHS ? g.fres : f_rhs), idx); LD2(cf0.B, f_B, idx); LD2(cf0.Pi, f_Pi, idx);
             LD2(cf0.zb, f_zb, idx);
-            if (usemask) { LD2(cf0.mask, f_mask, idx); } else { cf0.mask[0] = 1.0; cf0.mask[1] = 1.0; }
+            if constexpr (MASKED) { if (usemask) { LD2(cf0.mask, f_mask, idx); } else { cf0.mask[0] = 1.0; cf0.mask[1] = 1.0; } }
             if (HAS_ALPHA) LD2(cf0.a, f_a, idx);
             LD2(cf0.byS, f_by, idx); LD2(cf0.byN, f_by, idx + v.P);
             double2 bxp = ld2(f_bx, idx);
@@ -353,7 +362,7 @@
                         if (jf == v.ny - 1 && !v.ext[1]) n = (v.bct[1][1] == 0) ? v.two_v[1][1] - c : c + v.neu[1][1];
                     }
                     double nl, dnl;
-                    nl_terms(ph, c, cf1.B[a], cf1.Pi[a], cf1.zb[a], cf1.mask[a], nl, dnl);
+                    nl_terms(ph, c, cf1.B[a], cf1.Pi[a], cf1.zb[a], row_mask(cf1, a), nl, dnl);
                     const double bxW = a ? cf1.bx1 : cf1.bx0, bxE = a ? cf1.bx2 : cf1.bx1;
                     lo[a] = lofphi_cell(v, v.alpha, c, e, w, n, s, bxE, bxW, cf1.byN[a], cf1.byS[a], nl);
                     cc[a] = c;
@@ -375,7 +384,7 @@
             __syncthreads();
         }
 
-        auto advance_a = [&](const int m, const RowCoef &q, auto a_tag) {
+        auto advance_a = [&](const int m, const RowCoef<MASKED> &q, auto a_tag) {
             constexpr int a = decltype(a_tag)::value;
             const int j = r - m;
             const int x = xl + a, i = im + a;
@@ -393,7 +402,7 @@
                 if (j == v.ny - 1 && !v.ext[1]) n = (v.bct[1][1] == 0) ? v.two_v[1][1] - c : c + v.neu[1][1];
             }
             double nl, dnl;
-            nl_terms(ph, c, q.B[a], q.Pi[a], q.zb[a], q.mask[a], nl, dnl);
+            nl_terms(ph, c, q.B[a], q.Pi[a], q.zb[a], row_mask(q, a), nl, dnl);
             const double bxW = a ? q.bx1 : q.bx0, bxE = a ? q.bx2 : q.bx1;
             double aterm = HAS_ALPHA ? v.alpha * q.a[a] : v.alpha;
             double lofphi = lofphi_cell(v, aterm, c, e, w, n, s, bxE, bxW, q.byN[a], q.byS[a], nl);
@@ -401,7 +410,7 @@
             double denom = 1.0e-16 + lam + dnl;
             lds[s0 * LW + x] = c + (q.rhs[a] - lofphi) / denom;
         };
-        auto advance = [&](const int m, const RowCoef &q) {
+        auto advance = [&](const int m, const RowCoef<MASKED> &q) {
             const int j = r - m;
             if (j >= jmin && j <= jmax) {
                 const int a = (j + v.j0 + ((m - 1) & 1)) & 1;
@@ -422,7 +431,7 @@
         if constexpr (RR) {
             const int jr = r - 2 * K - 1;
             if (own && jr >= jA && jr < jB && jr >= 0 && jr < v.ny) {
-                const RowCoef &q = (K >= 2) ? cf5 : cf3;
+                const RowCoef<MASKED> &q = (K >= 2) ? cf5 : cf3;
                 const int s0 = ring(sr - (2 * K + 1)), sN = ring(sr - 2 * K), sS = ring(sr - (2 * K + 2));
                 const double *row = lds + s0 * LW;
                 double acc = (jr & 1) ? racc : 0.0, accp = (jr & 1) ? raccp : 0.0;
@@ -441,7 +450,7 @@
                         if (jr == v.ny - 1 && !v.ext[1]) n = (v.bct[1][1] == 0) ? v.two_v[1][1] - c : c + v.neu[1][1];
                     }
                     double nl, dnl;
-                    nl_terms(ph, c, q.B[a], q.Pi[a], q.zb[a], q.mask[a], nl, dnl);
+                    nl_terms(ph, c, q.B[a], q.Pi[a], q.zb[a], row_mask(q, a), nl, dnl);
                     const double bxW = a ? q.bx1 : q.bx0, bxE = a ? q.bx2 : q.bx1;
                     double aterm = HAS_ALPHA ? v.alpha * q.a[a] : v.alpha;
                     double lofphi = lofphi_cell(v, aterm, c, e, w, n, s, bxE, bxW, q.byN[a], q.byS[a], nl);
@@ -474,11 +483,11 @@
         }
         sr = sr + 1 == R ? 0 : sr + 1;
         if (in_row) { lds[sr * LW + xl] = pnext.x; lds[sr * LW + xl + 1] = pnext.y; }
-        if constexpr (RR && K >= 2) copy_coef<HAS_ALPHA>(cf5, cf4);
-        if constexpr (K >= 2) { copy_coef<HAS_ALPHA>(cf4, cf3); copy_coef<HAS_ALPHA>(cf3, cf2); }
-        else if constexpr (RR) copy_coef<HAS_ALPHA>(cf3, cf2);
-        copy_coef<HAS_ALPHA>(cf2, cf1);
-        copy_coef<HAS_ALPHA>(cf1, cf0);
+        if constexpr (RR && K >= 2) copy_coef<HAS_ALPHA, MASKED>(cf5, cf4);
+        if constexpr (K >= 2) { copy_coef<HAS_ALPHA, MASKED>(cf4, cf3); copy_coef<HAS_ALPHA, MASKED>(cf3, cf2); }
+        else if constexpr (RR) copy_coef<HAS_ALPHA, MASKED>(cf3, cf2);
+        copy_coef<HAS_ALPHA, MASKED>(cf2, cf1);
+        copy_coef<HAS_ALPHA, MASKED>(cf1, cf0);
     }
     if constexpr (ROUT) {
         if (g.onorm) {
@@ -516,19 +525,21 @@
     g.nstrips = (v.nx + maxW - 1) / maxW;
     g.W = 2 * ((v.nx + 2 * g.nstrips - 1) / (2 * g.nstrips));
     g.nstrips = (v.nx + g.W - 1) / g.W;
+    const bool unmasked = suhmo_mask_clean(L, depth) && v.alpha == 0.0;
     {
-        static int slots_k[3] = {0, 0, 0};
-        if (!slots_k[K]) {
+        static int slots_k[3][2] = {{0, 0}, {0, 0}, {0, 0}};
+        if (!slots_k[K][unmasked]) {
             int nb = 0, ncu = 0, dev = 0;
             HIPCHK(hipGetDevice(&dev));
             HIPCHK(hipDeviceGetAttribute(&ncu, hipDeviceAttributeMultiprocessorCount, dev));
-            HIPCHK(hipOccupancyMaxActiveBlocksPerMultiprocessor(&nb, (k_gsrb_fused<K, false, NT, RM>), NT, 0));
-            slots_k[K] = (nb > 0 ? nb : 1) * (ncu > 0 ? ncu : 256);
+            if (unmasked) HIPCHK(hipOccupancyMaxActiveBlocksPerMultiprocessor(&nb, (k_gsrb_fused<K, false, NT, RM, false, false>), NT, 0));
+            else HIPCHK(hipOccupancyMaxActiveBlocksPerMultiprocessor(&nb, (k_gsrb_fused<K, false, NT, RM>), NT, 0));
+            slots_k[K][unmasked] = (nb > 0 ? nb : 1) * (ncu > 0 ? ncu : 256);
         }
         g.jbeg = v.ext[0] ? -ext_rows : 0;
         g.jend = v.ny + (v.ext[1] ? ext_rows : 0);
         const int nrows = g.jend - g.jbeg;
-        int nch = slots_k[K] / g.nstrips;
+        int nch = slots_k[K][unmasked] / g.nstrips;
         if (nch < 1) nch = 1;
         g.Hc = (nrows + nch - 1) / nch;
         if (g.Hc < 8 * K) g.Hc = 8 * K;
@@ -561,9 +572,9 @@
         if (part != 1) D.prolong_pending = 0;
     }
     g.negflag = nullptr; g.mask_epoch = 0;
-    if (L->skip_mask && L->maskflag_epoch && L->maskflag_epoch == L->mask_epoch && (depth == 0 || L->coarse_mask_ok)
+    if (!unmasked && L->skip_mask && L->maskflag_epoch && L->maskflag_epoch == L->mask_epoch && (depth == 0 || L->coarse_mask_ok)
         && (L->desc.nx_global == 0)) {
-        g.negflag = (const unsigned *)(L->scratch + L->scratch_elems - 1); g.mask_epoch = L->mask_epoch;
+        g.negflag = suhmo_mask_report_word(L); g.mask_epoch = L->mask_epoch;
     }
     g.rres = g.rphi = nullptr; g.rP = g.rgy = 0;
     if (RST) {
@@ -588,14 +599,18 @@
             g.fres = D.fp.f[SUHMO_F_RES]; g.frhs = D.fp.f[SUHMO_F_RHS]; g.flphi = suhmo_field(L, depth, SUHMO_F_LPHI); g.fphiold = suhmo_field(L, depth, SUHMO_F_PHIOLD);
             if (!g.flphi || !g.fphiold) return -2;
             D.rhs_pending = 0; L->frhs_stream++;
-            hipLaunchKernelGGL((k_gsrb_fused<2, false, 64, false, true>), dim3(g.ntiles), dim3(NT), 0, st, v, D.fp, pin, D.phi_alt, L->ph, g);
+            if (unmasked) { hipLaunchKernelGGL((k_gsrb_fused<2, false, 64, 0, true, false>), dim3(g.ntiles), dim3(NT), 0, st, v, D.fp, pin, D.phi_alt, L->ph, g); L->relax_unmasked++; }
+            else hipLaunchKernelGGL((k_gsrb_fused<2, false, 64, 0, true>), dim3(g.ntiles), dim3(NT), 0, st, v, D.fp, pin, D.phi_alt, L->ph, g);
             { std::swap(D.fp.f[SUHMO_F_PHI], D.phi_alt); suhmo_fp_changed(); }
             return 0;
         } else { suhmo_set_error("internal: rhs_pending on a launch that cannot form it"); return -4; }
     }
     if (v.alpha != 0.0)
-        hipLaunchKernelGGL((k_gsrb_fused<K, true, NT, false>), dim3(g.ntiles), dim3(NT), 0, st, v, D.fp, pin, D.phi_alt, L->ph, g);
-    else
+        hipLaunchKernelGGL((k_gsrb_fused<K, true, NT, 0>), dim3(g.ntiles), dim3(NT), 0, st, v, D.fp, pin, D.phi_alt, L->ph, g);
+    else if (unmasked) {
+        hipLaunchKernelGGL((k_gsrb_fused<K, false, NT, RM, false, false>), dim3(g.ntiles), dim3(NT), 0, st, v, D.fp, pin, D.phi_alt, L->ph, g);
+        L->relax_unmasked++;
+    } else
         hipLaunchKernelGGL((k_gsrb_fused<K, false, NT, RM>), dim3(g.ntiles), dim3(NT), 0, st, v, D.fp, pin, D.phi_alt, L->ph, g);
     if (part != 1) { std::swap(D.fp.f[SUHMO_F_PHI], D.phi_alt); suhmo_fp_changed(); }
     return 0;
diff --git a/suhmo_amd/csrc/suhmo_hier.h b/suhmo_amd/csrc/suhmo_hier.h
--- a/suhmo_amd/csrc/suhmo_hier.h
+++ b/suhmo_amd/csrc/suhmo_hier.h
@@ -23,7 +23,7 @@
 template <class T> int launch_re(const T &t, hipStream_t st);
 template <class T> int launch_bcoef_faces(const T &t, hipStream_t st);
 template <class T> int launch_coef_ghosts(const T &t, int field, hipStream_t st);
-template <class T> int launch_bcoef_fused(const T &t, bool wide, unsigned *flag, unsigned epoch, hipStream_t st);
+template <class T> int launch_bcoef_fused(const T &t, bool wide, unsigned *flag, unsigned epoch, hipStream_t st, unsigned *small = nullptr, bool unmasked = false);
 int suhmo_multi_grad_cc(const suhmo_multi &m, hipStream_t st);
 int suhmo_multi_re_bcoef(const suhmo_multi &m, hipStream_t st);
 int suhmo_multi_norm_max(const suhmo_multi &m, suhmo_level *slot, int field, double *out, hipStream_t st);
diff --git a/suhmo_amd/csrc/suhmo_hier.hip b/suhmo_amd/csrc/suhmo_hier.hip
--- a/suhmo_amd/csrc/suhmo_hier.hip
+++ b/suhmo_amd/csrc/suhmo_hier.hip
@@ -75,6 +75,7 @@
     if ((rc = ensure_field(H, l, dst)) || (rc = ensure_field(H, l, src))) return rc;
     if (dst == SUHMO_F_PHI) { for (suhmo_level *L : H->lev[l].box) L->d[0].phi_fresh = 0; H->phi_ver[l]++; }
     if (dst == SUHMO_F_PHI && l == 0) H->phi_shadow_fresh = false;
+    if (dst == SUHMO_F_MASK) for (suhmo_level *L : H->lev[l].box) suhmo_mask_written(L);
     if (l == 0) H->base_full_ver++;
     if (l == 0) {
         suhmo_level *L = base_of(H);
@@ -583,6 +584,7 @@
     int rc = check_hier(H); if (rc) return rc;
     ARG(l >= 0 && l < H->nlev && field >= 0 && field < SUHMO_F_COUNT);
     HIPCHK(hipSetDevice(H->device));
+    if (field == SUHMO_F_MASK) for (suhmo_level *L : H->lev[l].box) suhmo_mask_written(L);
     return hier_ff(H, l, field, -1, corners != 0, HST(s));
 }
 extern "C" int suhmo_hier_cf_interp(suhmo_hier_t *H, int l, int field_f, int field_c, suhmo_stream_t s)
diff --git a/suhmo_amd/csrc/suhmo_hier_fill.hip b/suhmo_amd/csrc/suhmo_hier_fill.hip
--- a/suhmo_amd/csrc/suhmo_hier_fill.hip
+++ b/suhmo_amd/csrc/suhmo_hier_fill.hip
@@ -572,6 +572,7 @@
     if ((rc = ensure_field(H, l, ff)) || (rc = ensure_field(H, l - 1, fc)) || (rc = refresh_tables(H, l, st)) || (rc = coarse_args(H, l - 1, st, ca))) return rc;
     if (fc == SUHMO_F_PHI) { for (suhmo_level *L : H->lev[l - 1].box) L->d[0].phi_fresh = 0; H->phi_ver[l - 1]++; }
     if (fc == SUHMO_F_PHI && l == 1) H->phi_shadow_fresh = false;
+    if (fc == SUHMO_F_MASK) for (suhmo_level *L : H->lev[l - 1].box) suhmo_mask_written(L);
     if (mode == 1) {
         if (V.avg_cov.n) {
             dim3 grd((V.cov_w + 63) / 64, (V.cov_h + 3) / 4, (unsigned)V.avg_cov.n);
@@ -678,6 +679,7 @@
     int rc;
     CoarseArgs ca;
     if ((rc = ensure_field(H, l - 1, field_c)) || (rc = refresh_tables(H, l, st))) return rc;
+    if (field_c == SUHMO_F_MASK) for (suhmo_level *L : H->lev[l - 1].box) suhmo_mask_written(L);
     { const int fl[3] = {SUHMO_F_PHI, SUHMO_F_BX, SUHMO_F_BY};
       if (l == 1) { if ((rc = refresh_base(H, fl, 3, st))) return rc; }
       else if (V.part && (rc = sync_run(H, l - 1, V.sy_cread, fl, 3, st))) return rc;
diff --git a/suhmo_amd/csrc/suhmo_level.hip b/suhmo_amd/csrc/suhmo_level.hip
--- a/suhmo_amd/csrc/suhmo_level.hip
+++ b/suhmo_amd/csrc/suhmo_level.hip
@@ -168,7 +168,7 @@
     L->resout_req = L->resout_armed = L->resout_done = 0; L->resout_rhs = nullptr; L->resout_count = 0; L->resid_in_relax = 1;
     L->graph_max_cells = 1500000; L->gstream = nullptr; L->vgraph_replays = 0; memset(L->vgraph_seen, 0, sizeof(L->vgraph_seen));
     L->fused_min_cells = 1000000;
-    L->skip_mask = 1; L->poll_readback = 1;
+    L->skip_mask = 1; L->mask_known = 1; L->poll_readback = 1;
     L->bottom_solver = 0; L->bottom_one_launch_max_cells = 16384;
     L->bottom_ctr = nullptr; L->bottom_host_iters = L->bottom_host_solves = 0;
     {
@@ -181,7 +181,8 @@
             {"SUHMO_RESID_IN_RELAX", &suhmo_level::resid_in_relax}, {"SUHMO_TILE_STRIPS", &suhmo_level::tile_strips}, {"SUHMO_TILE_CHUNKS", &suhmo_level::tile_chunks},
             {"SUHMO_TILE_RESTRICT", &suhmo_level::tile_restrict}, {"SUHMO_TILE_ORDER", &suhmo_level::tile_order}, {"SUHMO_FAS_RHS_IN_RELAX", &suhmo_level::fas_rhs_in_relax},
             {"SUHMO_TILE_S", &suhmo_level::tile_s}, {"SUHMO_GSRB_TILE", &suhmo_level::gsrb_tile}, {"SUHMO_TILE_T", &suhmo_level::tile_t},
-            {"SUHMO_FUSED_RESTRICT", &suhmo_level::fused_restrict}, {"SUHMO_SKIP_MASK", &suhmo_level::skip_mask}, {"SUHMO_POLL_READBACK", &suhmo_level::poll_readback}};
+            {"SUHMO_FUSED_RESTRICT", &suhmo_level::fused_restrict}, {"SUHMO_SKIP_MASK", &suhmo_level::skip_mask}, {"SUHMO_MASK_KNOWN", &suhmo_level::mask_known},
+            {"SUHMO_POLL_READBACK", &suhmo_level::poll_readback}};
         static const LongKnob longs[] = {
             {"SUHMO_AGG_MIN_CELLS", &suhmo_level::agg_min_cells}, {"SUHMO_TILE_MAX_CELLS", &suhmo_level::tile_max_cells},
             {"SUHMO_GRAPH_MAX_CELLS", &suhmo_level::graph_max_cells}, {"SUHMO_FUSED_MIN_CELLS", &suhmo_level::fused_min_cells},
@@ -234,6 +235,9 @@
     }
     L->scratch = nullptr; L->scratch_elems = 0; L->hscratch = nullptr; L->hscratch_dev = nullptr; L->hseq = 0;
     L->mask_epoch = 0; L->maskflag_epoch = 0; L->mask_reported = 0; L->coarse_mask_ok = 0;
+    L->mask_state = SUHMO_MASK_UNKNOWN; L->mask_version = 1; L->mask_scan_version = 0; L->mask_scan_pending = 0; L->mask_capturing = 0;
+    L->mask_scan_captured = 0; L->mask_view = 0; L->mask_scan_errors = 0;
+    L->mask_host = nullptr; L->mask_ev = nullptr; L->mask_scans = L->bcoef_unmasked = L->relax_unmasked = 0;
     L->stub = 1;
     if (!stub) { int rc = level_storage(L); if (rc) { suhmo_level_destroy(L); return rc; } }
     *out = L;
@@ -255,8 +259,9 @@
     L->scratch_elems = 16384;
     HIPCHK(hipMalloc(&L->scratch, L->scratch_elems * sizeof(double)));
     HIPCHK(hipMemset(L->scratch, 0, L->scratch_elems * sizeof(double)));
-    HIPCHK(hipHostMalloc(&L->hscratch, 64 * sizeof(double), hipHostMallocMapped | hipHostMallocCoherent));
-    memset(L->hscratch, 0, 64 * sizeof(double));
+    HIPCHK(hipHostMalloc(&L->hscratch, SUHMO_HSCRATCH_DOUBLES * sizeof(double), hipHostMallocMapped | hipHostMallocCoherent));
+    memset(L->hscratch, 0, SUHMO_HSCRATCH_DOUBLES * sizeof(double));
+    L->mask_host = (unsigned *)(L->hscratch + SUHMO_HSCRATCH_MASK);
     if (L->poll_readback && hipHostGetDevicePointer((void **)&L->hscratch_dev, L->hscratch, 0) != hipSuccess) { L->hscratch_dev = nullptr; L->poll_readback = 0; (void)hipGetLastError(); }
     return 0;
 }
@@ -281,6 +286,7 @@
     if (L->xstream) { (void)hipStreamDestroy(L->xstream); (void)hipEventDestroy(L->xev[0]); (void)hipEventDestroy(L->xev[1]); }
     if (L->scratch) (void)hipFree(L->scratch);
     if (L->bottom_ctr) (void)hipFree(L->bottom_ctr);
+    if (L->mask_ev) (void)hipEventDestroy(L->mask_ev);
     if (L->hscratch) (void)hipHostFree(L->hscratch);
     delete L;
     return 0;
@@ -323,7 +329,7 @@
     static const struct { const char *k; int suhmo_level::*m; } tab[] = {
         {"gsrb_variant", &suhmo_level::gsrb_variant}, {"fused_hc", &suhmo_level::fused_hc}, {"bcoef_fused", &suhmo_level::bcoef_fused}, {"bcoef_tile_x", &suhmo_level::bcoef_tile_x},
         {"fused_nt", &suhmo_level::fused_nt}, {"fused_restrict", &suhmo_level::fused_restrict}, {"strips_rhs_local", &suhmo_level::strips_rhs_local},
-        {"tile_strips", &suhmo_level::tile_strips}, {"overlap_halo", &suhmo_level::overlap_halo}, {"skip_mask", &suhmo_level::skip_mask}, {"tile_chunks",
+        {"tile_strips", &suhmo_level::tile_strips}, {"overlap_halo", &suhmo_level::overlap_halo}, {"skip_mask", &suhmo_level::skip_mask}, {"mask_known", &suhmo_level::mask_known}, {"tile_chunks",
             &suhmo_level::tile_chunks}, {"tile_order", &suhmo_level::tile_order}, {"tile_restrict", &suhmo_level::tile_restrict}, {"fas_rhs_in_relax",
             &suhmo_level::fas_rhs_in_relax}, {"resid_in_relax", &suhmo_level::resid_in_relax}, {"fas_rhs_fused", &suhmo_level::fas_rhs_fused},
         {"tile_s", &suhmo_level::tile_s}, {"gsrb_tile", &suhmo_level::gsrb_tile}, {"tile_t", &suhmo_level::tile_t}, {"poll_readback", &suhmo_level::poll_readback}};
@@ -365,6 +371,10 @@
     if (!strcmp(key, "rhs_in_streaming_launches")) { *value = L->frhs_stream; return 0; }
     if (!strcmp(key, "rhs_in_tile_launches")) { *value = L->frhs_tile; return 0; }
     if (!strcmp(key, "residual_in_relax_launches")) { *value = L->resout_count; return 0; }
+    if (!strcmp(key, "mask_scans")) { *value = L->mask_scans; return 0; }
+    if (!strcmp(key, "mask_state")) { *value = L->mask_state; return 0; }
+    if (!strcmp(key, "bcoef_unmasked_launches")) { *value = L->bcoef_unmasked; return 0; }
+    if (!strcmp(key, "relax_unmasked_launches")) { *value = L->relax_unmasked; return 0; }
     if (!strcmp(key, "vcycle_graph_replays")) { *value = L->vgraph_replays; return 0; }
     if (!strcmp(key, "bottom_solver")) { *value = L->bottom_solver; return 0; }
     if (!strcmp(key, "bottom_one_launch_max_cells")) { *value = L->bottom_one_launch_max_cells; return 0; }
@@ -416,6 +426,7 @@
         if (!suhmo_field(L, depth, field)) return -2;
         int rc = L->ex(L->user, L, depth, &field, 1, s);
         if (!rc && field == SUHMO_F_PHI) L->d[depth].phi_fresh = suhmo_halo_rows(v);
+        if (field == SUHMO_F_MASK) suhmo_mask_halo_written(L);
         return rc;
     }
     return 0;
@@ -438,6 +449,7 @@
     CHECK_DF(L, depth, field);
     double *p = suhmo_field(L, depth, field);
     if (!p) { suhmo_set_error("field allocation failed"); return -2; }
+    if (field == SUHMO_F_MASK) { L->mask_view = 1; suhmo_mask_written(L); suhmo_level_drop_graphs(L); }
     if (base) *base = p;
     if (pitch) *pitch = L->d[depth].v.P;
     if (origin) *origin = cidx(L->d[depth].v, 0, 0);
@@ -480,7 +492,7 @@
     CHECK_DF(L, depth, field); ARG(src);
     HIPCHK(hipSetDevice(L->device));
     if (field == SUHMO_F_PHI) phi_changed(L, depth);
-    if (field == SUHMO_F_MASK) { L->coarse_mask_ok = 0; L->maskflag_epoch = 0; }
+    if (field == SUHMO_F_MASK) suhmo_mask_written(L);
     return field_io(L, depth, field, (double *)src, ghosted, on_device, true, (hipStream_t)s);
 }
 extern "C" int suhmo_level_get_field(suhmo_level_t *L, int depth, int field, double *dst, int ghosted,
@@ -509,7 +521,7 @@
     hipStream_t st = (hipStream_t)s;
     const DV &v = L->d[depth].v;
     if (field == SUHMO_F_PHI) phi_changed(L, depth);
-    if (field == SUHMO_F_MASK) { L->coarse_mask_ok = 0; L->maskflag_epoch = 0; }
+    if (field == SUHMO_F_MASK) suhmo_mask_written(L);
     int r[4]; box_region(L, depth, field, ibox, r);
     int j0 = v.j0;
     flo0 -= v.i0; fhi0 -= v.i0;
@@ -588,6 +600,7 @@
     const DV &v = L->d[depth].v;
     ARG(rows >= 1 && rows <= v.gy);
     HIPCHK(hipSetDevice(L->device));
+    if (field == SUHMO_F_MASK) suhmo_mask_halo_written(L);
     int jstart = side == 0 ? -rows : v.ny;
     if (field == SUHMO_F_BY && side == 1) jstart = v.ny + 1;
     hipLaunchKernelGGL(k_unpack_rows, grid2d(v.nx + 1, rows), BLK2D, 0, (hipStream_t)s, v, suhmo_field(L, depth, field), jstart, rows, dev_buf);
diff --git a/suhmo_amd/csrc/suhmo_ops.hip b/suhmo_amd/csrc/suhmo_ops.hip
--- a/suhmo_amd/csrc/suhmo_ops.hip
+++ b/suhmo_amd/csrc/suhmo_ops.hip
@@ -37,6 +37,7 @@
     CHECK_DF(L, depth, field); ARG(!is_face(field));
     HIPCHK(hipSetDevice(L->device));
     if (!suhmo_field(L, depth, field)) return -2;
+    if (field == SUHMO_F_MASK) suhmo_mask_written(L);
     return launch_fill_ghosts(on_level(L, depth), field, homogeneous, (hipStream_t)s);
 }
 
@@ -158,6 +159,7 @@
     for (int f : fields) if (!suhmo_field(L, depth, f)) return -2;
     int rc = L->ex(L->user, L, depth, fields.begin(), (int)fields.size(), (suhmo_stream_t)st);
     if (!rc) for (int f : fields) if (f == SUHMO_F_PHI) L->d[depth].phi_fresh = suhmo_halo_rows(v);
+    for (int f : fields) if (f == SUHMO_F_MASK) suhmo_mask_halo_written(L);
     return rc;
 }
 int suhmo_exchange_list(suhmo_level *L, int depth, const int *fields, int n, hipStream_t st)
@@ -167,6 +169,7 @@
     for (int k = 0; k < n; k++) if (!suhmo_field(L, depth, fields[k])) return -2;
     int rc = L->ex(L->user, L, depth, fields, n, (suhmo_stream_t)st);
     if (!rc) for (int k = 0; k < n; k++) if (fields[k] == SUHMO_F_PHI) L->d[depth].phi_fresh = suhmo_halo_rows(v);
+    for (int k = 0; k < n; k++) if (fields[k] == SUHMO_F_MASK) suhmo_mask_halo_written(L);
     return rc;
 }
 int suhmo_ensure_phi_halo(suhmo_level *L, int depth, int need, hipStream_t st)
@@ -480,6 +483,7 @@
     HIPCHK(hipSetDevice(L->device));
     Depth &D = L->d[depth];
     double *dst = suhmo_field(L, depth, dst_field);
+    if (dst_field == SUHMO_F_MASK) suhmo_mask_written(L);
     hipLaunchKernelGGL(k_divergence, grid2d(D.v.nx, D.v.ny), BLK2D, 0, (hipStream_t)s, D.v, D.fp.f[SUHMO_F_BX], D.fp.f[SUHMO_F_BY], dst);
     HIPCHK(hipGetLastError());
     return 0;
@@ -539,7 +543,7 @@
     HIPCHK(hipSetDevice(L->device));
     if (!suhmo_field(L, depth, dst) || !suhmo_field(L, depth, x) || !suhmo_field(L, depth, y)) return -2;
     if (dst == SUHMO_F_PHI) phi_changed(L, depth);
-    if (dst == SUHMO_F_MASK) { L->coarse_mask_ok = 0; L->maskflag_epoch = 0; }
+    if (dst == SUHMO_F_MASK) suhmo_mask_written(L);
     return launch_axby(on_level(L, depth), dst, x, y, a, b, (hipStream_t)s);
 }
 extern "C" int suhmo_level_set_value(suhmo_level_t *L, int depth, int field, double val, suhmo_stream_t s)
@@ -548,7 +552,7 @@
     HIPCHK(hipSetDevice(L->device));
     Depth &D = L->d[depth];
     if (field == SUHMO_F_PHI) phi_changed(L, depth);
-    if (field == SUHMO_F_MASK) { L->coarse_mask_ok = 0; L->maskflag_epoch = 0; }
+    if (field == SUHMO_F_MASK) suhmo_mask_written(L);
     hipLaunchKernelGGL(k_setval, grid2d(D.v.nx, D.v.ny), BLK2D, 0, (hipStream_t)s, D.v, suhmo_field(L, depth, field), val);
     HIPCHK(hipGetLastError());
     return 0;
```

New measurement: 492.0 V-cycles/s (median of 6 runs). 1.02x the previous value.
